# awslabs/crowd-coachable-recommendations

Hardware: AMD Instinct MI355X
Metric: queries/sec, exhaustive inner-product top-100 retrieval (NQ-shaped 2,681,468 x 768 bf16 corpus) (higher is better)
Workload: dtype bf16

## Files before the change

### crowd-coachable-recommendations_amd/ccrec_amd/_lib.py

```python
import ctypes
import os

_HERE = os.path.dirname(os.path.abspath(__file__))
LIB_PATH = os.path.join(os.path.dirname(_HERE), "lib", "libccr_hip.so")

CCR_OK = 0
CCR_ERR_INVALID, CCR_ERR_HIP, CCR_ERR_WORKSPACE, CCR_ERR_BLOCK_ID = -1, -2, -3, -4
DTYPE_F32, DTYPE_F16, DTYPE_BF16 = 0, 1, 2
SEARCH_DEFAULT, SEARCH_FORCE_DENSE, SEARCH_FORCE_FUSED, SEARCH_ASYNC = 0, 1, 2, 4
SCORES_CANONICAL, SCORES_MFMA = 0, 1

EXPORTS = [
    "ccr_last_error", "ccr_version", "ccr_pack_bf16", "ccr_pack_bf16_ex", "ccr_meanpool_pack_bf16", "ccr_meanpool_pack_bf16_ex", "ccr_index_create",
    "ccr_index_create_with_norms", "ccr_index_destroy",
    "ccr_index_rows", "ccr_index_dim", "ccr_search_workspace_bytes", "ccr_search", "ccr_search_last_stats",
    "ccr_merge_topk", "ccr_merge_topk_strided", "ccr_apply_block", "ccr_inbatch_ce_workspace_bytes", "ccr_inbatch_ce_fwd", "ccr_inbatch_ce_bwd", "ccr_inbatch_ce_bwd_dev", "ccr_rank_metrics",
    "ccr_search_finish", "ccr_scores", "ccr_search_blocked_workspace_bytes", "ccr_search_blocked",
    "ccr_search_sparse_prior_workspace_bytes", "ccr_search_sparse_prior", "ccr_colsum_bf16", "ccr_meanpool_bwd", "ccr_bm25_index_create", "ccr_bm25_index_destroy", "ccr_bm25_search_workspace_bytes",
    "ccr_bm25_search", "ccr_pack_bf16_padded", "ccr_shard_message_bytes", "ccr_search_shard", "ccr_shard_message_fill", "ccr_merge_shard_messages",
    "ccr_attention_bf16", "ccr_add_layernorm", "ccr_meanpool_pack_bf16_packed", "ccr_embed_layernorm", "ccr_gelu_bf16",
    "ccr_attention_half", "ccr_add_layernorm_half", "ccr_embed_layernorm_half", "ccr_gelu_half", "ccr_merge_short_lists",
    "ccr_bm25_search_workspace_bytes_k", "ccr_bm25_search_last_stats", "ccr_bm25_index_set_idf", "ccr_inbatch_pack3_bf16", "ccr_inbatch_ce_fwd_f32",
    "ccr_search_stream_wait_main_pass", "ccr_pool_ce_workspace_bytes", "ccr_pool_ce_fwd", "ccr_pool_ce_fwd_f32", "ccr_pool_ce_bwd_dev",
    "ccr_bpr_sample", "ccr_bpr_frozen_workspace_bytes", "ccr_bpr_frozen_fwd", "ccr_bpr_frozen_bwd_dev",
    "ccr_attention_fwd_train_half", "ccr_attention_bwd_workspace_bytes", "ccr_attention_bwd_half", "ccr_add_layernorm_bwd_half", "ccr_gelu_bwd_half",
    "ccr_dropout_bits_rows", "ccr_dropout_bits_attention", "ccr_dropout_apply", "ccr_attention_fwd_train_drop_half", "ccr_attention_bwd_drop_half",
    "ccr_add_layernorm_drop_half", "ccr_add_layernorm_bwd_drop_half",
]

MIN_VERSION = 101
BPR_VERSION = 102
ENCODER_TRAIN_VERSION = 103
ENCODER_DROPOUT_VERSION = 104

SHARD_HEADER_BYTES = 32
SHARD_MAGIC = 0x4D524343


class ShardHeader(ctypes.Structure):
    _fields_ = [("magic", ctypes.c_uint32), ("n_flagged", ctypes.c_uint32), ("k_valid", ctypes.c_uint32),
                ("n_covered", ctypes.c_uint32), ("row_offset", ctypes.c_int64), ("n_rows", ctypes.c_int64)]


class SearchStats(ctypes.Structure):
    _fields_ = [("path", ctypes.c_int32), ("n_fallback", ctypes.c_int32), ("sample_tiles", ctypes.c_int32),
                ("ranges", ctypes.c_int32), ("cap", ctypes.c_int32), ("sublists", ctypes.c_int32),
                ("n_candidates", ctypes.c_int64), ("ms_sample", ctypes.c_float), ("ms_threshold", ctypes.c_float),
                ("ms_main", ctypes.c_float), ("ms_select", ctypes.c_float), ("ms_fallback", ctypes.c_float),
                ("ms_total", ctypes.c_float), ("n_retried", ctypes.c_int32), ("n_dense", ctypes.c_int32),
                ("main_launches", ctypes.c_int32), ("opt_rank", ctypes.c_int32), ("main_tile_queries", ctypes.c_int32),
                ("reserved0", ctypes.c_int32)]


class CcrError(RuntimeError):
    pass


_lib = None


def load():
    global _lib
    if _lib is not None:
        return _lib
    if not os.path.isfile(LIB_PATH):
        raise CcrError(f"{LIB_PATH} not built: run `python -c 'import __graft_entry__ as g; g.build()'` "
                       f"(or make -C crowd-coachable-recommendations_amd/csrc)")
    lib = ctypes.CDLL(LIB_PATH)
    lib.ccr_version.restype = ctypes.c_int
    have = int(lib.ccr_version())
    if have < MIN_VERSION:
        raise CcrError(f"{LIB_PATH} is version {have}, this binding needs {MIN_VERSION}: rebuild it "
                       f"(python -c 'import __graft_entry__ as g; g.build()')")
    missing = [name for name in EXPORTS if not hasattr(lib, name)]
    if missing:
        raise CcrError(f"{LIB_PATH} lacks {', '.join(missing)}: rebuild it (python -c 'import __graft_entry__ as g; g.build()')")
    vp, i32, i64, f32, sz = ctypes.c_void_p, ctypes.c_int, ctypes.c_int64, ctypes.c_float, ctypes.c_size_t
    lib.ccr_last_error.restype = ctypes.c_char_p
    lib.ccr_last_error.argtypes = []
    lib.ccr_version.restype = i32
    lib.ccr_pack_bf16.argtypes = [vp, vp, vp, i64, i32, i32, vp]
    lib.ccr_pack_bf16_ex.argtypes = [vp, vp, vp, vp, i64, i32, i32, vp]
    lib.ccr_index_create_with_norms.argtypes = [vp, i64, i32, i64, vp, vp, ctypes.POINTER(vp)]
    lib.ccr_meanpool_pack_bf16.argtypes = [vp, i32, vp, vp, vp, i32, i32, i32, i32, vp]
    lib.ccr_meanpool_pack_bf16_ex.argtypes = [vp, i32, vp, vp, vp, vp, vp, i32, i32, i32, i32, vp]
    lib.ccr_index_create.argtypes = [vp, i64, i32, i64, vp, ctypes.POINTER(vp)]
    lib.ccr_index_destroy.argtypes = [vp]
    lib.ccr_index_rows.argtypes = [vp]
    lib.ccr_index_rows.restype = i64
    lib.ccr_index_dim.argtypes = [vp]
    lib.ccr_search_workspace_bytes.argtypes = [vp, i32, i32]
    lib.ccr_search_workspace_bytes.restype = sz
    lib.ccr_search.argtypes = [vp, vp, i32, i32, vp, vp, vp, sz, i32, vp]
    lib.ccr_search_last_stats.argtypes = [vp, ctypes.POINTER(SearchStats)]
    lib.ccr_merge_topk.argtypes = [vp, vp, i32, i32, i32, vp, vp, vp]
    lib.ccr_merge_topk_strided.argtypes = [vp, vp, i64, i64, i32, i32, i32, vp, vp, vp]
    lib.ccr_apply_block.argtypes = [vp, vp, i32, i32, vp, vp, i64, vp, vp, i32, vp]
    lib.ccr_inbatch_ce_workspace_bytes.argtypes = [i32, i32]
    lib.ccr_inbatch_ce_workspace_bytes.restype = sz
    lib.ccr_inbatch_ce_fwd.argtypes = [vp, vp, vp, i32, i32, f32, vp, vp, vp, sz, vp]
    lib.ccr_inbatch_ce_bwd.argtypes = [vp, vp, vp, vp, i32, i32, f32, f32, vp, vp, vp, vp, sz, vp]
    lib.ccr_inbatch_ce_bwd_dev.argtypes = [vp, vp, vp, vp, i32, i32, f32, vp, vp, vp, vp, vp, sz, vp]
    lib.ccr_inbatch_pack3_bf16.argtypes = [vp, vp, vp, i32, i32, vp, vp]
    lib.ccr_inbatch_ce_fwd_f32.argtypes = [vp, vp, vp, i32, i32, f32, vp, vp, vp, vp, sz, vp]
    lib.ccr_pool_ce_workspace_bytes.argtypes = [i32, i32, i32]
    lib.ccr_pool_ce_workspace_bytes.restype = sz
    lib.ccr_pool_ce_fwd.argtypes = [vp, vp, vp, vp, i32, i32, i32, f32, vp, vp, vp, sz, vp]
    lib.ccr_pool_ce_fwd_f32.argtypes = [vp, vp, vp, vp, i32, i32, i32, f32, vp, vp, vp, vp, sz, vp]
    lib.ccr_pool_ce_bwd_dev.argtypes = [vp, vp, vp, vp, vp, i32, i32, i32, f32, vp, vp, vp, vp, vp, sz, vp]
    lib.ccr_bpr_sample.argtypes = [vp, i32, i32, i64, vp, vp, vp, f32, vp, vp, i32, vp, i32, vp, vp]
    lib.ccr_bpr_frozen_workspace_bytes.argtypes = [i32, i32, i32]
    lib.ccr_bpr_frozen_workspace_bytes.restype = sz
    lib.ccr_bpr_frozen_fwd.argtypes = [vp, i64, i32, vp, vp, f32, vp, vp, vp, vp, i32, i32, vp, vp, sz, vp]
    lib.ccr_bpr_frozen_bwd_dev.argtypes = [vp, i64, i32, vp, vp, f32, vp, vp, vp, vp, i32, i32, vp, vp, vp, vp, vp, sz, vp]
    lib.ccr_rank_metrics.argtypes = [vp, i32, i32, vp, vp, vp, i32, vp, vp, vp]
    lib.ccr_search_finish.argtypes = [vp]
    lib.ccr_search_stream_wait_main_pass.argtypes = [vp, vp]
    lib.ccr_scores.argtypes = [vp, vp, i32, i32, vp, vp]
    lib.ccr_search_blocked_workspace_bytes.argtypes = [vp, i32, i32, vp]
    lib.ccr_search_blocked_workspace_bytes.restype = sz
    lib.ccr_search_blocked.argtypes = [vp, vp, i32, i32, vp, vp, vp, vp, vp, sz, i32, vp]
    lib.ccr_search_sparse_prior_workspace_bytes.argtypes = [vp, i32, i32, vp]
    lib.ccr_search_sparse_prior_workspace_bytes.restype = sz
    lib.ccr_search_sparse_prior.argtypes = [vp, vp, i32, i32, vp, vp, vp, vp, vp, vp, sz, i32, vp]
    lib.ccr_colsum_bf16.argtypes = [vp, i64, i32, vp, vp]
    lib.ccr_meanpool_bwd.argtypes = [vp, vp, vp, i32, i32, i32, i32, vp]
    lib.ccr_bm25_index_create.argtypes = [vp, vp, vp, vp, i64, i64, ctypes.c_double, ctypes.POINTER(vp)]
    lib.ccr_bm25_index_destroy.argtypes = [vp]
    lib.ccr_bm25_search_workspace_bytes.argtypes = [vp, i32, i32]
    lib.ccr_bm25_search_workspace_bytes.restype = sz
    lib.ccr_bm25_search_workspace_bytes_k.argtypes = [vp, i32, i32, i32]
    lib.ccr_bm25_search_workspace_bytes_k.restype = sz
    lib.ccr_bm25_search_last_stats.argtypes = [vp, vp]
    lib.ccr_bm25_index_set_idf.argtypes = [vp, vp, vp, vp]
    lib.ccr_bm25_search.argtypes = [vp, vp, vp, vp, i32, i32, vp, vp, vp, sz, vp]
    lib.ccr_pack_bf16_padded.argtypes = [vp, i64, i32, vp, i32, vp, vp, i32, vp]
    lib.ccr_attention_bf16.argtypes = [vp, vp, vp, vp, i32, i32, i32, i32, ctypes.c_float, vp]
    lib.ccr_add_layernorm.argtypes = [vp, vp, vp, vp, ctypes.c_float, vp, vp, i64, i32, vp]
    lib.ccr_embed_layernorm.argtypes = [vp, i64, vp, i64, vp, i64, vp, vp, vp, vp, vp, ctypes.c_float, vp, vp, i64, i32, vp]
    lib.ccr_gelu_bf16.argtypes = [vp, vp, i64, vp]
    lib.ccr_attention_half.argtypes = [vp, vp, vp, vp, i32, i32, i32, i32, ctypes.c_float, i32, vp]
    lib.ccr_add_layernorm_half.argtypes = [vp, vp, vp, vp, ctypes.c_float, vp, vp, i64, i32, i32, vp]
    lib.ccr_embed_layernorm_half.argtypes = [vp, i64, vp, i64, vp, i64, vp, vp, vp, vp, vp, ctypes.c_float, vp, vp, i64, i32, i32, vp]
    lib.ccr_gelu_half.argtypes = [vp, vp, i64, i32, vp]
    lib.ccr_attention_fwd_train_half.argtypes = [vp, vp, vp, vp, vp, i32, i32, i32, i32, ctypes.c_float, i32, vp]
    lib.ccr_attention_bwd_workspace_bytes.argtypes = [i32, i32, i32]
    lib.ccr_attention_bwd_workspace_bytes.restype = sz
    lib.ccr_attention_bwd_half.argtypes = [vp, vp, vp, vp, vp, vp, vp, i32, i32, i32, i32, ctypes.c_float, i32, vp, sz, vp]
    lib.ccr_add_layernorm_bwd_half.argtypes = [vp, vp, vp, ctypes.c_float, vp, vp, vp, vp, vp, i64, i32, i32, vp, sz, vp]
    lib.ccr_gelu_bwd_half.argtypes = [vp, vp, vp, i64, i32, vp]
    u64, u32, f64 = ctypes.c_uint64, ctypes.c_uint32, ctypes.c_double
    lib.ccr_dropout_bits_rows.argtypes = [vp, i64, i32, u64, u32, f64, vp]
    lib.ccr_dropout_bits_attention.argtypes = [vp, vp, vp, vp, i64, i32, i32, i32, u64, u32, f64, vp]
    lib.ccr_dropout_apply.argtypes = [vp, vp, f32, vp, vp, i64, i32, i32, vp]
    lib.ccr_attention_fwd_train_drop_half.argtypes = [vp, vp, vp, vp, vp, vp, f32, i32, i32, i32, i32, f32, i32, vp]
    lib.ccr_attention_bwd_drop_half.argtypes = [vp, vp, vp, vp, vp, vp, vp, vp, f32, vp, i32, i32, i32, i32, f32, i32, vp, sz, vp]
    lib.ccr_add_layernorm_drop_half.argtypes = [vp, vp, f32, vp, vp, vp, f32, vp, vp, i64, i32, i32, vp]
    lib.ccr_add_layernorm_bwd_drop_half.argtypes = [vp, vp, f32, vp, vp, f32, vp, vp, vp, vp, vp, i64, i32, i32, vp, sz, vp]
    lib.ccr_meanpool_pack_bf16_packed.argtypes = [vp, i32, vp, vp, vp, vp, vp, vp, i32, i32, i32, vp]
    lib.ccr_shard_message_bytes.argtypes = [i32, i32]
    lib.ccr_shard_message_bytes.restype = sz
    lib.ccr_search_shard.argtypes = [vp, vp, i32, i32, vp, vp, sz, i32, vp]
    lib.ccr_shard_message_fill.argtypes = [vp, i32, i32, i32, vp, vp, i64, i64, vp]
    lib.ccr_merge_shard_messages.argtypes = [vp, i64, i32, i32, i32, vp, vp, vp]
    lib.ccr_merge_short_lists.argtypes = [vp, i64, i32, i32, i32, i32, vp, vp, vp, vp, vp]
    for name in EXPORTS:
        fn = getattr(lib, name)
        if fn.restype is ctypes.c_int and name not in ("ccr_version", "ccr_index_dim"):
            fn.restype = i32
    _lib = lib
    return lib


def check(rc, what=""):
    if rc != CCR_OK:
        msg = load().ccr_last_error().decode("utf-8", "replace")
        if rc == CCR_ERR_BLOCK_ID:
            raise AssertionError("block id not found")
        raise CcrError(f"{what} failed ({rc}): {msg}")
```

### crowd-coachable-recommendations_amd/csrc/ccr_api.hip

```cpp
#include <stdarg.h>
#include <stdlib.h>
#include <string.h>

#include <math.h>

#include <algorithm>
#include <mutex>
#include <vector>

#include "ccr_index.h"
#include "ccr_narrow.h"
#include "ccr_topk_device.h"

namespace ccr {

static thread_local char g_err[512] = "";
void set_error(const char *fmt, ...) {
    va_list ap;
    va_start(ap, fmt);
    vsnprintf(g_err, sizeof(g_err), fmt, ap);
    va_end(ap);
}

static int env_int(const char *name, int dflt) {
    const char *e = getenv(name);
    return e ? atoi(e) : dflt;
}

Knobs read_knobs() {
    Knobs kn;
    kn.qgroups = env_int("CCR_QGROUPS", 0);
    kn.progressive = env_int("CCR_PROGRESSIVE", 1);
    kn.max_phases = env_int("CCR_PHASES", 3);
    kn.mfma16 = env_int("CCR_MFMA16", -1);
    kn.sample_div = env_int("CCR_SAMPLE_DIV", 0);
    kn.max_lists = env_int("CCR_MAX_LISTS", 0);
    kn.ranges = env_int("CCR_RANGES", 0);
    kn.optimistic = env_int("CCR_OPTIMISTIC", -1);
    kn.opt_rank = env_int("CCR_OPT_RANK", 0);
    kn.narrow = env_int("CCR_NARROW", -1);
    kn.wide = env_int("CCR_WIDE", -1);
    kn.narrow_grid = env_int("CCR_NARROW_GRID", 0);
    kn.narrow_groups = env_int("CCR_NARROW_GROUPS", NARROW_MAX_GROUPS);
    return kn;
}

static int pick_qgroups(int qblocks, int dim, const Knobs &kn, int tile_q = TILE_Q) {
    {
        const int v = kn.qgroups;
        if ((v == 1 || v == 2 || v == 4 || v == 8) && qblocks % v == 0) return v;
    }
    const size_t block_bytes = (size_t)tile_q * dim * 2;
    int best = 1;
    for (int gq = 1; gq <= NUM_XCD; gq *= 2) {
        if (qblocks % gq) continue;
        best = gq;
        if ((size_t)(qblocks / gq) * block_bytes <= (size_t)3 << 20) break;
    }
    return best;
}

static inline int64_t round_up(int64_t v, int64_t m) { return (v + m - 1) / m * m; }

static int best_sample_ranges(int64_t n_vt, int qblocks, int qgroups, int grid) {
    const int nrc = NUM_XCD / qgroups, qb_per = qblocks / qgroups, per_x = std::max(1, grid / NUM_XCD);
    int best_r = NUM_XCD;
    double best = 1e300;
    const int64_t r_max = round_up(std::min<int64_t>(n_vt, 1024), NUM_XCD);
    std::vector<double> load((size_t)per_x);
    for (int64_t R = NUM_XCD; R <= r_max; R += NUM_XCD) {
        double worst = 0.0;
        for (int rc = 0; rc < nrc; ++rc) {
            std::fill(load.begin(), load.end(), 0.0);
            const int64_t items = R / nrc * qb_per;
            for (int64_t item = 0; item < items; ++item) {
                const int64_t r = rc + nrc * (item / qb_per);
                const int64_t ntile = (n_vt - r + R - 1) / R;
                if (ntile > 0) load[(size_t)(item % per_x)] += (double)ntile + 0.15;
            }
            worst = std::max(worst, *std::max_element(load.begin(), load.end()));
        }
        if (worst < best - 1e-9) {
            best = worst;
            best_r = (int)R;
        }
    }
    return best_r;
}

constexpr size_t DENSE_SCRATCH_TARGET = (size_t)1 << 30;

struct MainPassChoice {
    int64_t sample, ranges;
    int item_a, item_b;
    int opt_rank;
};

static int optimistic_rank(int k, int64_t sample, int64_t tiles, const Knobs &kn) {
    if (kn.opt_rank > 0) return kn.opt_rank;
    const double need = (double)k * (double)sample / (double)tiles;
    int r = 40;
    for (; r < 1 << 20; ++r) {
        const double a = 1.0 / (9.0 * r), t = 1.0 - a - 5.2 * sqrt(a);
        if (t > 0.0 && (double)r * t * t * t >= need) break;
    }
    return r;
}

static MainPassChoice choose_main_pass(const Plan &p, int k, int64_t sample_a, int64_t sample_b, int64_t sample_c, const Knobs &kn,
                                       bool single_only = false) {
    const int nrc = NUM_XCD / p.main_qgroups, qb_per = p.main_qblocks / p.main_qgroups, per_x = p.grid / NUM_XCD;
    const double tile_cost = p.tile_q == WIDE_Q ? 1.37 : 1.0;
    int64_t max_lists = p.rescore_cap > 512 ? 2048 : 1024;
    if ((max_lists / p.sublists) * p.main_qblocks < p.grid) max_lists = 2048;
    if (kn.max_lists >= 64 && kn.max_lists < max_lists) max_lists = kn.max_lists;
    const int64_t r_hi = std::min<int64_t>(max_lists / p.sublists, round_up(std::max<int64_t>(1, p.tiles / 8), NUM_XCD));
    const int64_t target = std::min<int64_t>(r_hi, round_up(std::max<int64_t>(NUM_XCD, (int64_t)p.grid * 6 / p.main_qblocks), NUM_XCD));
    const bool prog_on = kn.progressive != 0 && !single_only;
    const int max_phases = kn.max_phases;
    const double qscale = (double)p.nq_pad / 3584.0;
    const double select_per_range = 0.1 * qscale, hit_w = 0.014 * qscale, phase_w = 3.0;
    auto sample_cost = [&](int64_t smp) -> double {
        return (double)((smp * p.qblocks + p.grid - 1) / p.grid) + 0.015 * (double)smp * std::max(1.0, qscale);
    };

    MainPassChoice best_choice = {sample_a, target, 0, 0, 0};
    double best = 1e300;
    for (int pass = 0; pass < 3; ++pass) {
        const int64_t smp = pass == 0 ? sample_a : (pass == 1 ? sample_b : sample_c);
        if ((pass >= 1 && smp == sample_a) || (pass == 2 && smp == sample_b)) continue;
        const double fs = (double)smp / (double)p.tiles;
        const double smp_cost = sample_cost(smp);
        auto survivors = [&](double fa, double fb) -> double {
            if (fa <= 0.0) return (double)k / fs;
            if (fb <= 0.0) return (double)k * (fa / fs + (1.0 - fa) / fa);
            return (double)k * (fa / fs + fb / fa + (1.0 - fa - fb) / (fa + fb));
        };
        const int64_t r_lo = std::max<int64_t>(NUM_XCD, target / 2 / NUM_XCD * NUM_XCD);
        for (int64_t R = r_lo; R <= std::min(r_hi, target * 2); R += NUM_XCD) {
            if (kn.ranges > 0 && R != std::min<int64_t>(r_hi, std::max<int64_t>(r_lo, round_up(kn.ranges, NUM_XCD)))) continue;
            const int64_t items = R / nrc * qb_per;
            const double item_cost = ((double)((p.tiles + R - 1) / R) + 0.15) * tile_cost;
            auto rounds = [&](int64_t n) { return (double)((n + per_x - 1) / per_x); };
            const double common = smp_cost + select_per_range * (double)R + 1e-3 * std::abs((double)(R - target));
            const double single = rounds(items) * item_cost + hit_w * survivors(0.0, 0.0) + common;
            if (single < best && kn.optimistic != 1) {
                best = single;
                best_choice = {smp, R, 0, 0, 0};
            }
            if (kn.optimistic != 0 && smp * GROUPS_PER_TILE >= 4 * 40) {
                const int rank = optimistic_rank(k, smp, p.tiles, kn);
                if ((int64_t)rank * 4 <= smp * GROUPS_PER_TILE) {
                    const double pass = std::max((double)rank / fs, (double)k);
                    const double opt = rounds(items) * item_cost + hit_w * pass + common - (kn.optimistic == 1 ? 1e9 : 0.0);
                    if (opt < best) {
                        best = opt;
                        best_choice = {smp, R, 0, 0, rank};
                    }
                }
            }
            if (!(prog_on && items > per_x && (double)p.tiles / (double)R >= 8.0)) continue;
            const double fa = (double)per_x / (double)items;
            const double two = (1.0 + rounds(items - per_x)) * item_cost + phase_w + hit_w * survivors(fa, 0.0) + common;
            if (two < best) {
                best = two;
                best_choice = {smp, R, per_x, 0, 0};
            }
            if (max_phases < 3) continue;
            for (int m = 1; m <= 3; ++m) {
                const int64_t ib = (int64_t)per_x * (1 + m);
                if (ib >= items) break;
                const double fb = (double)m * per_x / (double)items;
                const double three = (1.0 + m + rounds(items - ib)) * item_cost + 2.0 * phase_w + hit_w * survivors(fa, fb) + common;
                if (three < best) {
                    best = three;
                    best_choice = {smp, R, per_x, (int)ib, 0};
                }
            }
        }
    }
    return best_choice;
}

static CandLayout one_segment(int cap) {
    CandLayout L;
    memset(&L, 0, sizeof(L));
    L.nseg = 1;
    L.seg_end[0] = L.seg_end[1] = L.seg_end[2] = INT32_MAX;
    L.cap[0] = L.cap[1] = L.cap[2] = cap;
    return L;
}

static Plan make_plan_for(int64_t n_rows, int dim, int n_q, int k, int flags, int num_cu, const Knobs &kn, int mfma16) {
    Plan p;
    memset(&p, 0, sizeof(p));
    p.nq_pad = (int)round_up(n_q, TILE_Q);
    p.qblocks = p.nq_pad / TILE_Q;
    p.tile_q = TILE_Q;
    p.main_qblocks = p.qblocks;
    p.main_qgroups = 1;
    p.tiles = (n_rows + TILE_DOCS - 1) / TILE_DOCS;
    p.full_tiles = n_rows / TILE_DOCS;
    p.grid = std::max(NUM_XCD, num_cu / NUM_XCD * NUM_XCD);
    {
        p.mfma16 = mfma16;
        p.sublists = p.mfma16 ? 8 : 4;
    }
    p.rescore_cap = std::min(8192, std::max(256, 2 * pow2_ceil(k)));

    const int64_t min_sample = (2 * (int64_t)k + GROUPS_PER_TILE - 1) / GROUPS_PER_TILE;
    int64_t sample_div = 32;
    bool sample_div_forced = false;
    {
        if (kn.sample_div >= 4 && kn.sample_div <= 256) {
            sample_div = kn.sample_div;
            sample_div_forced = true;
        }
    }
    auto sample_for = [&](int64_t div) { return std::max<int64_t>({(p.tiles + div - 1) / div, min_sample, 4}); };
    int64_t sample = sample_for(sample_div);
    bool fused = (dim % 8 == 0) && dim >= 8 && (sample * 4 <= p.full_tiles) && k <= MAX_K;
    if ((flags & CCR_SEARCH_FORCE_FUSED) && (dim % 8 == 0) && p.full_tiles >= 1) {
        if (!fused) sample = std::min<int64_t>(std::max<int64_t>(sample, 1), p.full_tiles);
        fused = sample * GROUPS_PER_TILE >= k;
    }
    if (flags & CCR_SEARCH_FORCE_DENSE) fused = false;
    p.fused = fused ? 1 : 0;

    if (p.fused) {
        p.qgroups = pick_qgroups(p.qblocks, dim, kn);
        const bool pinned = sample_div_forced || (flags & CCR_SEARCH_FORCE_FUSED);
        const int64_t sample_alt = pinned ? sample : sample_for(2 * sample_div);
        int64_t sample_big = pinned ? sample : sample_for(sample_div / 2);
        if (sample_big * 4 > p.full_tiles) sample_big = sample;
        int nqt = n_q <= 16 ? 1 : (n_q <= 32 ? 2 : 4);
        int ngroups = n_q <= NARROW_MAX_Q ? 1 : 2;
        if (n_q > NARROW_MAX_Q && n_q <= 96 && kn.narrow_groups >= 2 && dim % TILE_K == 0 && narrow_lds_bytes(6, dim) <= (size_t)160 * 1024)
            nqt = 6, ngroups = 1;
        const bool narrow = kn.narrow != 0 && n_q <= NARROW_MAX_Q * std::min(std::max(kn.narrow_groups, 1), NARROW_MAX_GROUPS) && dim % TILE_K == 0 &&
                            narrow_lds_bytes(nqt, dim) <= (size_t)160 * 1024 && (ngroups == 1 || num_cu >= 16);
        p.narrow = narrow ? nqt : 0;
        p.narrow_groups = narrow ? ngroups : 1;
        p.tile_q = TILE_Q;
        p.main_qblocks = p.qblocks;
        if (!narrow && p.mfma16 && dim % 32 == 0 && kn.wide != 0) {
            const int wb = (n_q + WIDE_Q - 1) / WIDE_Q;
            const double per_xcd = (double)(wb / pick_qgroups(wb, dim, kn, WIDE_Q)) * WIDE_Q * dim * 2.0;
            const double per_flop = per_xcd <= 3.2 * 1048576.0 ? 0.95 : (per_xcd <= 5.5 * 1048576.0 ? 0.97 : 1.04);
            if (kn.wide == 1 || (double)wb * WIDE_Q * per_flop < (double)p.qblocks * TILE_Q) {
                p.tile_q = WIDE_Q;
                p.main_qblocks = wb;
                p.nq_pad = (int)round_up(std::max<int64_t>(n_q, (int64_t)wb * WIDE_Q), TILE_Q);
                p.qblocks = p.nq_pad / TILE_Q;
                p.qgroups = pick_qgroups(p.qblocks, dim, kn);
            }
        }
        p.main_qgroups = pick_qgroups(p.main_qblocks, dim, kn, p.tile_q);
        const MainPassChoice choice = choose_main_pass(p, k, sample, sample_alt, sample_big, kn, narrow);
        sample = choice.sample;
        const int64_t R = choice.ranges;
        p.sample_tiles = (int)sample;
        p.sample_stride = std::max<int64_t>(1, p.full_tiles / sample);
        p.sample_ranges = best_sample_ranges(sample, p.qblocks, p.qgroups, p.grid);
        p.ranges = (int)R;
        p.item_a = choice.item_a;
        p.item_b = choice.item_b;
        p.opt_rank = choice.opt_rank;
        const int nrc_p = NUM_XCD / p.main_qgroups, qb_per_p = p.main_qblocks / p.main_qgroups;
        const int64_t RA = p.item_a ? std::min<int64_t>(R, (int64_t)nrc_p * ((p.item_a + qb_per_p - 1) / qb_per_p)) : 0;
        const int64_t RB = p.item_b ? std::min<int64_t>(R, (int64_t)nrc_p * ((p.item_b + qb_per_p - 1) / qb_per_p)) : 0;
        const double ratio = (double)p.tiles / (double)sample;
        const double expect = (double)k * ratio * 1.3 + 64.0;
        const double fs = 1.0 / ratio, nlists = (double)R * p.sublists;
        const double xk = 1.25 * ((double)k + 4.75 * sqrt((double)k) + 8.0) / (double)k;
        const int64_t tile_rows = TILE_DOCS / p.sublists;
        const double xr = p.opt_rank ? 1.25 * ((double)p.opt_rank + 4.75 * sqrt((double)p.opt_rank) + 8.0) / (double)p.opt_rank : 0.0;
        auto cap_for = [&](double g) -> int {
            const double mean = p.opt_rank ? xr * std::max((double)p.opt_rank / fs, (double)k) / nlists : xk * (double)k / (g * nlists);
            const int64_t c = (int64_t)(mean + 6.0 * sqrt(mean)) + 16 + tile_rows;
            return (int)round_up(std::min<int64_t>(std::max<int64_t>(c, 16), 8192), 4);
        };
        const double fa = p.item_a ? (double)(p.item_a / qb_per_p) * nrc_p / (double)R : 0.0;
        const double fb = p.item_b ? std::max(0.0, (double)(p.item_b / qb_per_p) * nrc_p / (double)R - fa) : 0.0;
        const double upd_compact = std::min(32768.0, std::max(4096.0, 8.0 * pow2_ceil(k)));
        auto seen = [&](double g, double found) { return found > upd_compact ? g * upd_compact / found : g; };
        const double found_a = (double)k * fa / fs;
        CandLayout &L = p.cand;
        memset(&L, 0, sizeof(L));
        const int seg_end_v[3] = {RA ? (int)RA : (int)R, RB > RA ? (int)RB : (int)R, (int)R};
        int64_t recs = 0;
        L.nseg = 0;
        int prev_end = 0;
        for (int g = 0; g < 3; ++g) {
            L.seg_end[g] = INT32_MAX;
            L.cap[g] = 16;
            L.base[g] = recs;
        }
        for (int g = 0; g < 3; ++g) {
            if (seg_end_v[g] <= prev_end) continue;
            const int sg = L.nseg++;
            double frac_seen = fs;
            if (sg == 1) frac_seen = fa >= 2.0 * fs ? seen(fa, found_a) : fs;
            if (sg == 2) frac_seen = fa >= 2.0 * fs ? seen(fa + fb, found_a + (double)k * fb / fa) : fs;
            L.seg_end[sg] = seg_end_v[g];
            L.cap[sg] = cap_for(std::min(1.0, std::max(frac_seen, fs)));
            L.base[sg] = recs;
            recs += (int64_t)(seg_end_v[g] - prev_end) * p.nq_pad * p.sublists * L.cap[sg];
            recs = round_up(recs, 32);
            prev_end = seg_end_v[g];
        }
        L.seg_end[L.nseg - 1] = INT32_MAX;
        p.cap = L.cap[0];
        const double want_opt = std::max(xr * std::max((double)p.opt_rank / fs, (double)k) + 512.0, k > 256 ? 18.0 * k : 0.0);
        p.select_compact = select_compact_entries(dim, p.ranges * p.sublists, p.rescore_cap,
                                                  (int64_t)((p.opt_rank ? want_opt : (RA ? 16.0 * k + 512.0 : expect)) * 1.25));
        p.first_nsub = p.ranges * p.sublists;
        p.first_sp = p.sublists;
        p.first_lay = p.cand;
        if (p.narrow) {
            const double pass = p.opt_rank ? xr * std::max((double)p.opt_rank / fs, (double)k) : expect;
            int64_t capn = std::max<int64_t>(recs / ((int64_t)NARROW_SUBLISTS * std::max(1, n_q)), (int64_t)(8.0 * pass) + 4096);
            capn = std::min<int64_t>(capn, (int64_t)1 << 22) / 4 * 4;
            recs = std::max<int64_t>(recs, capn * NARROW_SUBLISTS * n_q);
            p.first_lay = one_segment((int)capn);
            p.first_nsub = NARROW_SUBLISTS;
            p.first_sp = NARROW_SUBLISTS;
        }
        p.cand_recs = recs;
        p.dense_rows_per_chunk = FALLBACK_ROWS;
    } else {
        int64_t rows = (int64_t)(DENSE_SCRATCH_TARGET / ((size_t)n_rows * 4));
        rows = std::min<int64_t>(std::max<int64_t>(rows, 1), n_q);
        if (rows >= 64) rows = rows / 64 * 64;
        p.dense_rows_per_chunk = rows;
    }
    const SearchWs w = search_ws(p, n_rows, dim, n_q, k, nullptr);
    p.off_qnorm = (size_t)w.qnorm, p.off_thr = (size_t)w.thr, p.off_gmax = (size_t)w.gmax, p.off_cnt = (size_t)w.cnt, p.off_cand = (size_t)w.cand;
    p.off_flag = (size_t)w.flag_count, p.off_dense = (size_t)w.dense, p.off_retry = (size_t)w.Q2, p.off_top = (size_t)w.top, p.off_safe = (size_t)w.thr_safe;
    p.total = w.total;
    return p;
}

SearchWs search_ws(const Plan &p, int64_t n_rows, int dim, int n_q, int k, char *base) {
    SearchWs w;
    memset(&w, 0, sizeof(w));
    Bump b = {0};
    auto at = [&](size_t off) { return (char *)((uintptr_t)base + off); };
    auto take = [&](size_t bytes) { return at(b.take(bytes)); };
    if (!p.fused) {
        w.flag_count = (uint32_t *)take(64 + (size_t)n_q * 4);
        w.flag_list = w.flag_count + 16;
        w.dense_bytes = (size_t)p.dense_rows_per_chunk * (n_rows + 3) * 4;
        w.dense = (float *)take(w.dense_bytes);
        w.total = b.off;
        return w;
    }
    const size_t nq_pad = p.nq_pad;
    w.qnorm = (float *)take(nq_pad * 4);
    w.thr = (float *)take(nq_pad * 8);
    w.cq = w.thr + nq_pad;
    w.gmax = (float *)take((size_t)p.sample_tiles * GROUPS_PER_TILE * nq_pad * 4);
    w.cnt = (uint32_t *)take((size_t)p.ranges * nq_pad * p.sublists * 4);
    w.cand = (uint2 *)take((size_t)p.cand_recs * 8);
    w.flag_count = (uint32_t *)take(64 + (size_t)n_q * 4);
    w.stat_cand = (unsigned long long *)(w.flag_count + 2);
    w.flag_list = w.flag_count + 16;
    w.cand_bytes = (char *)w.flag_count - (char *)w.cand;
    w.top = (uint32_t *)take(p.item_b ? (nq_pad + (size_t)n_q * k) * 4 : 0);
    w.thr_safe = (float *)take(p.opt_rank ? nq_pad * 8 : 0);
    w.cq_safe = w.thr_safe + nq_pad;
    w.dense_bytes = (size_t)p.dense_rows_per_chunk * n_rows * 4;
    w.dense = (float *)take(w.dense_bytes);
    w.retry_bytes = nq_pad * dim * 2 + nq_pad * 8 + (size_t)n_q * 16 + 64 + 64 + (size_t)n_q * 4 + 256 * 10;
    Bump r = {b.take(w.retry_bytes)};
    w.Q2 = (uint16_t *)at(r.take(nq_pad * dim * 2));
    w.thr2 = (float *)at(r.take(nq_pad * 4));
    w.cq2 = (float *)at(r.take(nq_pad * 4));
    w.retry_list = (uint32_t *)at(r.take((size_t)n_q * 4));
    w.dense_list = (uint32_t *)at(r.take((size_t)n_q * 4));
    w.counts = (uint32_t *)at(r.take(64));
    w.flag2 = (uint32_t *)at(r.take(64 + (size_t)n_q * 4));
    w.list_b = (uint32_t *)at(r.take((size_t)n_q * 4));
    w.list_c = (uint32_t *)at(r.take((size_t)n_q * 4));
    w.total = b.off;
    return w;
}

Plan make_plan(int64_t n_rows, int dim, int n_q, int k, int flags, int num_cu, const Knobs &kn) {
    if (kn.mfma16 >= 0) return make_plan_for(n_rows, dim, n_q, k, flags, num_cu, kn, kn.mfma16 ? 1 : 0);
    if (k <= 512) return make_plan_for(n_rows, dim, n_q, k, flags, num_cu, kn, 1);
    const Plan p32 = make_plan_for(n_rows, dim, n_q, k, flags, num_cu, kn, 0);
    if (p32.fused && p32.ranges * 8 <= 2048) return make_plan_for(n_rows, dim, n_q, k, flags, num_cu, kn, 1);
    return p32;
}

}

using namespace ccr;

namespace {
constexpr int SLAB_SLOTS = 1024, SLAB_SLOT_BYTES = 256, MAX_DEVICES = 64;
struct Slab {
    char *base = nullptr;
    char *host = nullptr;
    std::vector<int> free_slots;
};
constexpr int SLAB_HOST_BYTES = 64;
std::mutex g_slab_mutex;
Slab g_slabs[MAX_DEVICES];

int slab_take(int device, uint32_t **out, volatile uint32_t **host_out) {
    std::lock_guard<std::mutex> lock(g_slab_mutex);
    CCR_REQUIRE(device >= 0 && device < MAX_DEVICES, "device ordinal %d out of range", device);
    Slab &sl = g_slabs[device];
    if (!sl.base) {
        CCR_HIP_CHECK(hipMalloc((void **)&sl.base, (size_t)SLAB_SLOTS * SLAB_SLOT_BYTES));
        if (hipHostMalloc((void **)&sl.host, (size_t)SLAB_SLOTS * SLAB_HOST_BYTES, hipHostMallocDefault) != hipSuccess) {
            (void)hipFree(sl.base);
            sl.base = nullptr;
            set_error("ccr_index_create: hipHostMalloc of the pinned flag lines failed");
            return CCR_ERR_HIP;
        }
        for (int i = SLAB_SLOTS - 1; i >= 0; --i) sl.free_slots.push_back(i);
    }
    if (sl.free_slots.empty()) {
        set_error("ccr_index_create: more than %d live indices on device %d", SLAB_SLOTS, device);
        return CCR_ERR_INVALID;
    }
    *out = reinterpret_cast<uint32_t *>(sl.base + (size_t)sl.free_slots.back() * SLAB_SLOT_BYTES);
    *host_out = reinterpret_cast<volatile uint32_t *>(sl.host + (size_t)sl.free_slots.back() * SLAB_HOST_BYTES);
    sl.free_slots.pop_back();
    return CCR_OK;
}

void slab_give(int device, uint32_t *p) {
    if (!p || device < 0 || device >= MAX_DEVICES) return;
    std::lock_guard<std::mutex> lock(g_slab_mutex);
    Slab &sl = g_slabs[device];
    sl.free_slots.push_back((int)((reinterpret_cast<char *>(p) - sl.base) / SLAB_SLOT_BYTES));
}
}

extern "C" const char *ccr_last_error(void) { return g_err; }
extern "C" int ccr_version(void) { return 104; }

extern "C" int ccr_index_destroy(ccr_index *ix);

namespace {
struct CachedBlock {
    void *p;
    size_t bytes;
};
std::vector<CachedBlock> g_blocks[MAX_DEVICES];
constexpr size_t BLOCK_CACHE_ENTRIES = 8;

int block_take(int device, size_t bytes, void **out, size_t *got) {
    CCR_REQUIRE(device >= 0 && device < MAX_DEVICES, "device ordinal %d out of range", device);
    bytes = (bytes + 4095) / 4096 * 4096;
    {
        std::lock_guard<std::mutex> lock(g_slab_mutex);
        auto &v = g_blocks[device];
        for (size_t i = 0; i < v.size(); ++i)
            if (v[i].bytes >= bytes && v[i].bytes <= 2 * bytes) {
                *out = v[i].p;
                *got = v[i].bytes;
                v.erase(v.begin() + i);
                return CCR_OK;
            }
    }
    CCR_HIP_CHECK(hipMalloc(out, bytes));
    *got = bytes;
    return CCR_OK;
}

void block_give(int device, void *p, size_t bytes) {
    if (!p) return;
    void *drop = nullptr;
    if (device >= 0 && device < MAX_DEVICES && bytes <= ((size_t)64 << 20)) {
        std::lock_guard<std::mutex> lock(g_slab_mutex);
        auto &v = g_blocks[device];
        v.push_back({p, bytes});
        if (v.size() > BLOCK_CACHE_ENTRIES) {
            drop = v.front().p;
            v.erase(v.begin());
        }
    } else {
        drop = p;
    }
    if (drop) (void)hipFree(drop);
}
}

static int index_create_impl(const uint16_t *D_bf16, int64_t n_rows, int dim, int64_t global_row_offset, const float *row_bounds,
                             void *stream, ccr_index **out) {
    CCR_REQUIRE(D_bf16 && out, "ccr_index_create: null pointer");
    CCR_REQUIRE(n_rows >= 1 && n_rows < ((int64_t)1 << 32), "ccr_index_create: n_rows=%lld out of range [1, 2^32)",
                (long long)n_rows);
    CCR_REQUIRE(dim >= 8 && dim % 8 == 0 && dim <= 4096, "ccr_index_create: dim=%d must be a multiple of 8 in [8, 4096]", dim);
    CCR_REQUIRE((uintptr_t)D_bf16 % 16 == 0, "ccr_index_create: corpus pointer must be 16-byte aligned");
    hipStream_t s = (hipStream_t)stream;
    ccr_index *ix = new ccr_index();
    memset(ix, 0, sizeof(*ix));
    ix->D = D_bf16;
    ix->n_rows = n_rows;
    ix->dim = dim;
    ix->offset = ix->id_out = global_row_offset;
    ix->knobs = read_knobs();
    auto build = [&]() -> int {
        CCR_HIP_CHECK(hipGetDevice(&ix->device));
        CCR_HIP_CHECK(hipDeviceGetAttribute(&ix->num_cu, hipDeviceAttributeMultiprocessorCount, ix->device));
        int rc = slab_take(ix->device, &ix->dmax_bits, &ix->host_flags);
        if (rc != CCR_OK) return rc;
        const int64_t tiles = (n_rows + TILE_DOCS - 1) / TILE_DOCS;
        void *tn = nullptr;
        rc = block_take(ix->device, (size_t)tiles * 4, &tn, &ix->tile_bytes);
        if (rc != CCR_OK) return rc;
        ix->tile_norm = (float *)tn;
        uint32_t *tile_bits = reinterpret_cast<uint32_t *>(ix->tile_norm);
        if (row_bounds) {
            ix->row_norm = row_bounds;
            rc = launch_tile_norms(row_bounds, n_rows, tile_bits, ix->dmax_bits, s);
            if (rc != CCR_OK) return rc;
        } else {
            void *rn = nullptr;
            rc = block_take(ix->device, (size_t)n_rows * 4, &rn, &ix->row_bytes);
            if (rc != CCR_OK) return rc;
            ix->row_norm = ix->row_norm_own = (float *)rn;
            CCR_HIP_CHECK(hipMemsetAsync(ix->dmax_bits, 0, 4, s));
            CCR_HIP_CHECK(hipMemsetAsync(tile_bits, 0, (size_t)tiles * 4, s));
            rc = launch_row_norms_bf16(D_bf16, n_rows, dim, ix->row_norm_own, ix->dmax_bits, tile_bits, s);
            if (rc != CCR_OK) return rc;
            CCR_HIP_CHECK(hipStreamSynchronize(s));
        }
        return CCR_OK;
    };
    const int rc = build();
    if (rc != CCR_OK) {
        ccr_index_destroy(ix);
        return rc;
    }
    *out = ix;
    return CCR_OK;
}

extern "C" int ccr_index_create(const uint16_t *D_bf16, int64_t n_rows, int dim, int64_t global_row_offset, void *stream,
                                ccr_index **out) {
    return index_create_impl(D_bf16, n_rows, dim, global_row_offset, nullptr, stream, out);
}

extern "C" int ccr_index_create_with_norms(const uint16_t *D_bf16, int64_t n_rows, int dim, int64_t global_row_offset,
                                           const float *row_norm_bounds, void *stream, ccr_index **out) {
    CCR_REQUIRE(row_norm_bounds, "ccr_index_create_with_norms: null row_norm_bounds");
    return index_create_impl(D_bf16, n_rows, dim, global_row_offset, row_norm_bounds, stream, out);
}

extern "C" int ccr_index_destroy(ccr_index *ix) {
    if (!ix) return CCR_OK;
    if (ix->pending.active && ix->have_events) (void)hipEventSynchronize(ix->ev[EV_ASYNC_END]);
    ix->pending.active = false;
    slab_give(ix->device, ix->dmax_bits);
    block_give(ix->device, ix->tile_norm, ix->tile_bytes);
    block_give(ix->device, ix->row_norm_own, ix->row_bytes);
    if (ix->have_events)
        for (int i = 0; i < EV_COUNT; ++i)
            if (ix->ev[i]) (void)hipEventDestroy(ix->ev[i]);
    delete ix;
    return CCR_OK;
}

extern "C" int64_t ccr_index_rows(const ccr_index *ix) { return ix ? ix->n_rows : -1; }
extern "C" int ccr_index_dim(const ccr_index *ix) { return ix ? ix->dim : -1; }

extern "C" size_t ccr_search_workspace_bytes(const ccr_index *ix, int n_q, int k) {
    if (!ix || n_q <= 0 || k <= 0) return 0;
    Plan a = make_plan(ix->n_rows, ix->dim, n_q, k, CCR_SEARCH_DEFAULT, ix->num_cu, ix->knobs);
    Plan b = make_plan(ix->n_rows, ix->dim, n_q, k, CCR_SEARCH_FORCE_DENSE, ix->num_cu, ix->knobs);
    Plan c = make_plan(ix->n_rows, ix->dim, n_q, k, CCR_SEARCH_FORCE_FUSED, ix->num_cu, ix->knobs);
    return std::max({a.total, b.total, c.total}) + 256;
}

extern "C" int ccr_search_stream_wait_main_pass(const ccr_index *ix, void *stream) {
    CCR_REQUIRE(ix, "ccr_search_stream_wait_main_pass: null index");
    if (!ix->main_pass_recorded) return CCR_OK;
    CCR_HIP_CHECK(hipStreamWaitEvent((hipStream_t)stream, ix->ev[EV_MAIN_END], 0));
    return CCR_OK;
}

extern "C" int ccr_search_last_stats(const ccr_index *ix, ccr_search_stats *stats) {
    CCR_REQUIRE(ix && stats, "ccr_search_last_stats: null pointer");
    CCR_REQUIRE(!ix->pending.active, "ccr_search_last_stats: an asynchronous search is pending (call ccr_search_finish first)");
    *stats = ix->stats;
    return CCR_OK;
}

static int dense_for_list(const ccr_index *ix, const uint16_t *Q, const uint32_t *d_qlist, int n, int k, float *scratch, int64_t rows_per_chunk,
                          float *out_scores, int64_t *out_ids, hipStream_t s) {
    for (int lo = 0; lo < n; lo += (int)rows_per_chunk) {
        const int m = std::min<int64_t>(rows_per_chunk, n - lo);
        int rc = launch_dense_scores(ix->D, ix->n_rows, ix->dim, Q, d_qlist ? d_qlist + lo : nullptr, lo, m, nullptr, scratch, s);
        if (rc != CCR_OK) return rc;
        rc = launch_dense_select(scratch, ix->n_rows, k, d_qlist ? d_qlist + lo : nullptr, lo, m, nullptr, ix->id_out, out_scores, out_ids, s);
        if (rc != CCR_OK) return rc;
    }
    return CCR_OK;
}

static bool margin_path_ok(const ccr_index *ix, int k) { return ix->dim % 8 == 0 && k <= MAX_K; }
static int64_t tiles_of(const ccr_index *ix) { return (ix->n_rows + TILE_DOCS - 1) / TILE_DOCS; }

static GemmArgs gemm_args(const ccr_index *ix, const uint16_t *Q, int n_q, int nq_pad) {
    GemmArgs g;
    memset(&g, 0, sizeof(g));
    g.D = ix->D;
    g.n_rows = ix->n_rows;
    g.dim = ix->dim;
    g.Q = Q;
    g.n_q = n_q;
    g.nq_pad = nq_pad;
    g.qblocks = nq_pad / TILE_Q;
    g.item_end = INT32_MAX;
    return g;
}

static GemmArgs filter_args(const ccr_index *ix, const Plan &p, const SearchWs &w, const uint16_t *Q, int n_q, int nq_pad, int qblocks,
                            int qgroups, const float *thr, const float *cq, const CandLayout &lay) {
    GemmArgs g = gemm_args(ix, Q, n_q, nq_pad);
    g.qblocks = qblocks;
    g.qgroups = qgroups;
    g.n_vt = p.tiles;
    g.tile_stride = 1;
    g.ranges = p.ranges;
    g.thr = thr;
    g.cq = cq;
    g.tile_norm = ix->tile_norm;
    g.cnt = w.cnt;
    g.cand = w.cand;
    g.lay = lay;
    return g;
}

static int store_scores(const ccr_index *ix, const uint16_t *Q, int n_q, int ranges, float *out, int64_t pitch, hipStream_t s) {
    GemmArgs g = gemm_args(ix, Q, n_q, (int)round_up(n_q, TILE_Q));
    g.n_vt = tiles_of(ix);
    g.tile_stride = 1;
    g.ranges = ranges;
    g.qgroups = 1;
    g.store = out;
    g.store_pitch = pitch;
    return launch_gemm(g, ix->knobs.mfma16 != 0 ? MAIN_16X16 : MAIN_32X32, EPI_STORE, std::max(NUM_XCD, ix->num_cu / NUM_XCD * NUM_XCD), s);
}

static int margin_for_rows(const ccr_index *ix, const uint16_t *Qc, const float *hint, const uint32_t *out_rows, int n, int k, float *scratch,
                           size_t scratch_bytes, float *out_scores, int64_t *out_ids, uint32_t *flag_count, uint32_t *flag_list, hipStream_t s) {
    const int64_t pitch = round_up(ix->n_rows, 4);
    int64_t chunk = (int64_t)(scratch_bytes / ((size_t)pitch * 4));
    CCR_REQUIRE(chunk >= 1, "margin path: no room for one score row");
    if (chunk > TILE_Q) chunk = chunk / TILE_Q * TILE_Q;
    const int ranges = (int)round_up(std::min<int64_t>(std::max<int64_t>(1, tiles_of(ix) / 4), 1024), NUM_XCD);
    for (int lo = 0; lo < n; lo += (int)chunk) {
        const int m = std::min<int64_t>(chunk, n - lo);
        const uint16_t *Q = Qc + (int64_t)lo * ix->dim;
        int rc = store_scores(ix, Q, m, ranges, scratch, pitch, s);
        if (rc != CCR_OK) return rc;
        rc = launch_margin_select(scratch, pitch, ix->n_rows, k, ix->dim, Q, ix->D, ix->tile_norm, ix->row_norm, ix->dmax_bits,
                                  hint ? hint + lo : nullptr, out_rows ? out_rows + lo : nullptr, lo, m, ix->id_out, out_scores, out_ids, flag_count, flag_list, s);
        if (rc != CCR_OK) return rc;
    }
    return CCR_OK;
}

static int run_main_pass(const ccr_index *ix, const Plan &p, const SearchWs &w, const uint16_t *Q, int n_q, int k, hipStream_t s) {
    GemmArgs gm = filter_args(ix, p, w, Q, n_q, p.nq_pad, p.main_qblocks, p.main_qgroups, w.thr, w.cq, p.cand);
    const int nrc = NUM_XCD / gm.qgroups, qb_per = gm.qblocks / gm.qgroups, items = p.ranges / nrc * qb_per;
    const int bounds[4] = {0, p.item_a, p.item_b, items};
    int done = 0, updates = 0, prev_full = 0, prev_part = 0, prev_blocks = 0;
    for (int ph = 1; ph < 4; ++ph) {
        if (bounds[ph] <= done) continue;
        if (done > 0) {
            const int rl_full = done / qb_per, part = done % qb_per;
            const int full = rl_full * nrc * p.sublists, partial = part ? (rl_full + 1) * nrc * p.sublists : 0;
            const bool more = bounds[ph] < items && ph < 3;
            const int rc = launch_threshold_update(w.cand, w.cnt, full, partial, part, prev_full, prev_part, prev_blocks, qb_per, p.sublists, n_q,
                                                   p.nq_pad, p.cand, k, w.cq, ix->tile_norm, p.item_b ? w.top : nullptr, updates > 0, more, w.thr, s, p.tile_q);
            if (rc != CCR_OK) return rc;
            prev_full = full;
            prev_part = partial;
            prev_blocks = part;
            ++updates;
        }
        gm.item_begin = done;
        gm.item_end = bounds[ph];
        const MainKernel kind = p.tile_q == WIDE_Q ? MAIN_WIDE : p.mfma16 ? MAIN_16X16 : MAIN_32X32;
        const int rc = launch_gemm(gm, kind, EPI_FILTER, p.grid, s);
        if (rc != CCR_OK) return rc;
        done = bounds[ph];
    }
    return CCR_OK;
}

static int run_narrow_pass(const ccr_index *ix, const Plan &p, const SearchWs &w, const uint16_t *Q, int n_q, hipStream_t s) {
    NarrowArgs na;
    memset(&na, 0, sizeof(na));
    na.D = ix->D;
    na.n_rows = ix->n_rows;
    na.dim = ix->dim;
    na.Q = Q;
    na.n_q = n_q;
    na.q_stride = narrow_query_stride(ix->dim);
    na.thr = w.thr;
    na.cq = w.cq;
    na.tile_norm = ix->tile_norm;
    na.cand = w.cand;
    na.cnt = w.cnt;
    na.cap = p.first_lay.cap[0];
    na.groups = p.narrow_groups;
    int ngrid = ix->knobs.narrow_grid > 0 ? ix->knobs.narrow_grid : ix->num_cu;
    const int64_t blocks = (ix->n_rows + 16 * NARROW_WAVES - 1) / (16 * NARROW_WAVES);
    if ((int64_t)ngrid > blocks) ngrid = (int)std::max<int64_t>(1, blocks);
    if (p.narrow_groups == 2) ngrid = std::max(16, ngrid / 16 * 16);
    return launch_narrow_filter(na, p.narrow, ngrid, s);
}

static int read_words(void *host, const void *dev, int n, hipStream_t s) {
    CCR_HIP_CHECK(hipMemcpyAsync(host, dev, (size_t)n * 4, hipMemcpyDeviceToHost, s));
    CCR_HIP_CHECK(hipStreamSynchronize(s));
    return CCR_OK;
}


static int fused_stats(ccr_index *ix, uint32_t nflag, unsigned long long ncand) {
    const Plan &p = ix->plan;
    ccr_search_stats &st = ix->stats;
    float a = 0, b = 0;
    CCR_HIP_CHECK(hipEventElapsedTime(&st.ms_sample, ix->ev[EV_SAMPLE_BEGIN], ix->ev[EV_SAMPLE_END]));
    CCR_HIP_CHECK(hipEventElapsedTime(&a, ix->ev[EV_BEGIN], ix->ev[EV_SAMPLE_BEGIN]));
    CCR_HIP_CHECK(hipEventElapsedTime(&b, ix->ev[EV_SAMPLE_END], ix->ev[EV_MAIN_BEGIN]));
    st.ms_threshold = a + b;
    CCR_HIP_CHECK(hipEventElapsedTime(&st.ms_main, ix->ev[EV_MAIN_BEGIN], ix->ev[EV_MAIN_END]));
    CCR_HIP_CHECK(hipEventElapsedTime(&st.ms_select, ix->ev[EV_MAIN_END], ix->ev[EV_SELECT_END]));
    CCR_HIP_CHECK(hipEventElapsedTime(&st.ms_total, ix->ev[EV_BEGIN], ix->ev[EV_SELECT_END]));
    st.path = 1;
    st.n_fallback = (int32_t)nflag;
    st.sample_tiles = p.sample_tiles;
    st.ranges = p.narrow ? 1 : p.ranges;
    st.cap = p.narrow ? p.first_lay.cap[0] : p.cap;
    st.sublists = p.narrow ? p.first_sp : p.sublists;
    st.main_launches = 1 + (p.item_a ? 1 : 0) + (p.item_b ? 1 : 0);
    st.opt_rank = p.opt_rank;
    st.main_tile_queries = p.narrow ? 0 : p.tile_q;
    st.n_candidates = (int64_t)ncand;
    return CCR_OK;
}

static int recover_thresholds(const ccr_index *ix, const SearchWs &w, int nflag) {
    const auto &pd = ix->pending;
    const int rc = launch_threshold(w.gmax, (int64_t)ix->plan.sample_tiles * GROUPS_PER_TILE, pd.n_q, ix->plan.nq_pad, pd.k, w.qnorm, ix->dmax_bits,
                                    ix->dim, ix->tile_norm, ix->plan.sample_stride, w.thr_safe, w.cq_safe, pd.stream);
    if (rc != CCR_OK) return rc;
    return launch_underfilled_to_retry(w.flag_list, 0, nflag, w.thr_safe, w.thr, pd.stream);
}

static int to_dense(const SearchWs &w, const uint32_t *list, int n, int &n_dense, hipStream_t s) {
    CCR_HIP_CHECK(hipMemcpyAsync(w.dense_list + n_dense, list, (size_t)n * 4, hipMemcpyDeviceToDevice, s));
    n_dense += n;
    return CCR_OK;
}

static int retry_group(ccr_index *ix, const SearchWs &w, const uint32_t *cur, int n_cur, int &n_dense) {
    const Plan &p = ix->plan;
    const auto &pd = ix->pending;
    hipStream_t s = pd.stream;
    const int nsub_all = p.ranges * p.sublists;
    for (int round = 0;; ++round) {
        int rc = launch_gather_queries(pd.Q, ix->dim, cur, n_cur, w.thr, w.cq, w.Q2, w.thr2, w.cq2, s);
        if (rc != CCR_OK) return rc;
        const int pad2 = (int)round_up(n_cur, TILE_Q);
        const int64_t cap2 = std::min<int64_t>(8192, (int64_t)(w.cand_bytes / 8) / ((int64_t)nsub_all * pad2) / 4 * 4);
        if (cap2 < 16) break;
        const CandLayout lay2 = one_segment((int)cap2);
        CCR_HIP_CHECK(hipMemsetAsync(w.cnt, 0, (size_t)nsub_all * pad2 * 4, s));
        CCR_HIP_CHECK(hipMemsetAsync(w.flag2, 0, 64, s));
        const GemmArgs g = filter_args(ix, p, w, w.Q2, n_cur, pad2, pad2 / TILE_Q, pick_qgroups(pad2 / TILE_Q, ix->dim, ix->knobs), w.thr2, w.cq2, lay2);
        rc = launch_gemm(g, p.mfma16 ? MAIN_16X16 : MAIN_32X32, EPI_FILTER, p.grid, s);
        if (rc != CCR_OK) return rc;
        rc = launch_select_rescore(w.cand, w.cnt, nsub_all, p.sublists, n_cur, pad2, lay2, pd.k, p.rescore_cap, p.select_compact, ix->n_rows,
                                   w.thr2, w.cq2, ix->tile_norm, ix->row_norm, ix->dmax_bits, w.Q2, ix->D, ix->dim, ix->id_out, pd.out_scores, pd.out_ids,
                                   w.flag2, w.flag2 + 16, nullptr, cur, s);
        if (rc != CCR_OK) return rc;
        ix->stats.n_retried += n_cur;
        uint32_t again = 0;
        rc = read_words(&again, w.flag2, 1, s);
        if (rc != CCR_OK || again == 0) return rc;
        uint32_t *next = (cur == w.list_b) ? w.list_c : w.list_b;
        rc = launch_partition_flags(w.flag2 + 16, 0, (int)again, next, w.dense_list + n_dense, w.counts, s);
        if (rc != CCR_OK) return rc;
        uint32_t hc[2] = {0, 0};
        rc = read_words(hc, w.counts, 2, s);
        if (rc != CCR_OK) return rc;
        n_dense += (int)hc[1];
        const uint32_t *list = cur;
        const int n = n_cur;
        cur = next;
        n_cur = (int)hc[0];
        if (n_cur == 0 || round == 2 || n_cur >= n) break;
        rc = launch_threshold_update(w.cand, w.cnt, nsub_all, 0, 0, 0, 0, 0, 1, p.sublists, n, pad2, lay2, pd.k, w.cq2, ix->tile_norm, nullptr,
                                     false, false, w.thr2, s);
        if (rc != CCR_OK) return rc;
        rc = launch_scatter_thresholds(list, n, w.thr2, w.thr, s);
        if (rc != CCR_OK) return rc;
    }
    return n_cur > 0 ? to_dense(w, cur, n_cur, n_dense, s) : CCR_OK;
}

static int retry_flagged(ccr_index *ix, const SearchWs &w, int n_retry, int &n_dense) {
    const Plan &p = ix->plan;
    const auto &pd = ix->pending;
    const int nsub_all = p.ranges * p.sublists;
    if (nsub_all > 2048) return to_dense(w, w.retry_list, n_retry, n_dense, pd.stream);
    int rc = launch_threshold_update(w.cand, w.cnt, p.first_nsub, 0, 0, 0, 0, 0, 1, p.first_sp, pd.n_q, p.nq_pad, p.first_lay, pd.k, w.cq,
                                     ix->tile_norm, nullptr, false, false, w.thr, pd.stream);
    if (rc != CCR_OK) return rc;
    const int64_t want_cap = std::min<int64_t>(8192, 4 * (int64_t)p.cap);
    int64_t group = (int64_t)(w.cand_bytes / 8) / ((int64_t)nsub_all * want_cap) / TILE_Q * TILE_Q;
    group = std::max<int64_t>(TILE_Q, std::min<int64_t>(group, round_up(n_retry, TILE_Q)));
    for (int g0 = 0; g0 < n_retry && rc == CCR_OK; g0 += (int)group)
        rc = retry_group(ix, w, w.retry_list + g0, std::min<int>((int)group, n_retry - g0), n_dense);
    return rc;
}

static int complete_dense(ccr_index *ix, const SearchWs &w, int n_dense) {
    const Plan &p = ix->plan;
    const auto &pd = ix->pending;
    hipStream_t s = pd.stream;
    const bool margin_in_cand = w.cand_bytes > w.dense_bytes;
    const int64_t fit = (int64_t)(w.cand_bytes / ((size_t)ix->n_rows * 4)) / 64 * 64;
    const bool fp64_in_cand = n_dense > p.dense_rows_per_chunk && fit >= 64;
    const int64_t chunk = fp64_in_cand ? std::min<int64_t>(fit, 256) : p.dense_rows_per_chunk;
    float *fp64_scr = fp64_in_cand ? (float *)w.cand : w.dense;
    if (!margin_path_ok(ix, pd.k))
        return dense_for_list(ix, pd.Q, w.dense_list, n_dense, pd.k, fp64_scr, chunk, pd.out_scores, pd.out_ids, s);
    CCR_HIP_CHECK(hipMemsetAsync(w.flag2, 0, 64, s));
    for (int lo = 0; lo < n_dense; lo += p.nq_pad) {
        const int m = std::min(p.nq_pad, n_dense - lo);
        int rc = launch_gather_queries(pd.Q, ix->dim, w.dense_list + lo, m, w.thr, w.cq, w.Q2, w.thr2, w.cq2, s);
        if (rc != CCR_OK) return rc;
        rc = margin_for_rows(ix, w.Q2, w.thr2, w.dense_list + lo, m, pd.k, margin_in_cand ? (float *)w.cand : w.dense,
                             margin_in_cand ? w.cand_bytes : w.dense_bytes, pd.out_scores, pd.out_ids, w.flag2, w.flag2 + 16, s);
        if (rc != CCR_OK) return rc;
    }
    uint32_t left = 0;
    const int rc = read_words(&left, w.flag2, 1, s);
    if (rc != CCR_OK || left == 0) return rc;
    return dense_for_list(ix, pd.Q, w.flag2 + 16, (int)left, pd.k, fp64_scr, chunk, pd.out_scores, pd.out_ids, s);
}

static int search_complete(ccr_index *ix) {
    auto &pd = ix->pending;
    hipStream_t s = pd.stream;
    const bool was_async = pd.active;
    pd.active = false;
    const SearchWs w = search_ws(ix->plan, ix->n_rows, ix->dim, pd.n_q, pd.k, pd.ws);
    struct { uint32_t nflag, pad; unsigned long long ncand; } host;
    int rc = CCR_OK;
    if (was_async) {
        CCR_HIP_CHECK(hipEventSynchronize(ix->ev[EV_ASYNC_END]));
        host.nflag = ix->host_flags[0];
        host.ncand = *reinterpret_cast<volatile unsigned long long *>(ix->host_flags + 2);
    } else {
        rc = read_words(&host, w.flag_count, 4, s);
        if (rc != CCR_OK) return rc;
    }
    rc = fused_stats(ix, host.nflag, host.ncand);
    if (rc != CCR_OK || host.nflag == 0) return rc;
    rc = ix->plan.opt_rank ? recover_thresholds(ix, w, (int)host.nflag) : CCR_OK;
    if (rc != CCR_OK) return rc;
    rc = launch_partition_flags(w.flag_list, 0, (int)host.nflag, w.retry_list, w.dense_list, w.counts, s);
    if (rc != CCR_OK) return rc;
    uint32_t hc[2] = {0, 0};
    rc = read_words(hc, w.counts, 2, s);
    if (rc != CCR_OK) return rc;
    int n_dense = (int)hc[1];
    if (hc[0] > 0) rc = retry_flagged(ix, w, (int)hc[0], n_dense);
    if (rc == CCR_OK && n_dense > 0) rc = complete_dense(ix, w, n_dense);
    if (rc != CCR_OK) return rc;
    ix->stats.n_dense += n_dense;
    CCR_HIP_CHECK(hipEventRecord(ix->ev[EV_DONE], s));
    CCR_HIP_CHECK(hipStreamSynchronize(s));
    CCR_HIP_CHECK(hipEventElapsedTime(&ix->stats.ms_fallback, ix->ev[EV_SELECT_END], ix->ev[EV_DONE]));
    ix->stats.ms_total += ix->stats.ms_fallback;
    return CCR_OK;
}

extern "C" int ccr_search_finish(ccr_index *ix) {
    CCR_REQUIRE(ix, "ccr_search_finish: null index");
    return ix->pending.active ? search_complete(ix) : CCR_OK;
}

static int search_dense(ccr_index *ix, const SearchWs &w, const uint16_t *Q, int n_q, int k, float *out_scores, int64_t *out_ids,
                        int flags, hipStream_t s) {
    const bool async = (flags & CCR_SEARCH_ASYNC) != 0;
    const int64_t chunk = ix->plan.dense_rows_per_chunk;
    int rc;
    if (!async && !(flags & CCR_SEARCH_FORCE_DENSE) && margin_path_ok(ix, k)) {
        CCR_HIP_CHECK(hipMemsetAsync(w.flag_count, 0, 64, s));
        rc = margin_for_rows(ix, Q, nullptr, nullptr, n_q, k, w.dense, w.dense_bytes, out_scores, out_ids, w.flag_count, w.flag_list, s);
        if (rc != CCR_OK) return rc;
        uint32_t nf = 0;
        rc = read_words(&nf, w.flag_count, 1, s);
        if (rc != CCR_OK) return rc;
        ix->stats.n_fallback = ix->stats.n_dense = (int32_t)nf;
        if (nf > 0) rc = dense_for_list(ix, Q, w.flag_list, (int)nf, k, w.dense, chunk, out_scores, out_ids, s);
    } else {
        rc = dense_for_list(ix, Q, nullptr, n_q, k, w.dense, chunk, out_scores, out_ids, s);
    }
    if (rc != CCR_OK) return rc;
    CCR_HIP_CHECK(hipEventRecord(ix->ev[EV_DONE], s));
    if (async) return CCR_OK;
    CCR_HIP_CHECK(hipStreamSynchronize(s));
    CCR_HIP_CHECK(hipEventElapsedTime(&ix->stats.ms_total, ix->ev[EV_BEGIN], ix->ev[EV_DONE]));
    ix->stats.ms_fallback = ix->stats.ms_total;
    return CCR_OK;
}

static int search_impl(ccr_index *ix, const uint16_t *Q_bf16, int n_q, int k, float *out_scores, int64_t *out_ids, int64_t id_out,
                       uint32_t *flagged_out, void *workspace, size_t ws_bytes, int flags, void *stream) {
    CCR_REQUIRE(ix && Q_bf16 && out_scores && out_ids, "ccr_search: null pointer");
    CCR_REQUIRE(n_q >= 0, "ccr_search: n_q=%d", n_q);
    CCR_REQUIRE(k >= 1 && k <= MAX_K && (int64_t)k <= ix->n_rows, "ccr_search: k=%d must be in [1, min(n_rows=%lld, %d)]", k,
                (long long)ix->n_rows, MAX_K);
    CCR_REQUIRE((uintptr_t)Q_bf16 % 16 == 0, "ccr_search: query pointer must be 16-byte aligned");
    CCR_REQUIRE(!ix->pending.active, "ccr_search: an asynchronous search is pending on this index (call ccr_search_finish first)");
    memset(&ix->stats, 0, sizeof(ix->stats));
    ix->main_pass_recorded = false;
    if (n_q == 0) return CCR_OK;
    hipStream_t s = (hipStream_t)stream;
    ix->id_out = id_out;
    const bool async = (flags & CCR_SEARCH_ASYNC) != 0;
    const int plan_flags = flags & ~CCR_SEARCH_ASYNC;
    if (!(ix->plan_nq == n_q && ix->plan_k == k && ix->plan_flags == plan_flags)) {
        ix->plan = make_plan(ix->n_rows, ix->dim, n_q, k, plan_flags, ix->num_cu, ix->knobs);
        ix->plan_nq = n_q;
        ix->plan_k = k;
        ix->plan_flags = plan_flags;
    }
    const Plan p = ix->plan;
    if (!workspace || ws_bytes < p.total || (uintptr_t)workspace % 256 != 0) {
        set_error("ccr_search: workspace %zu bytes (256-byte aligned) required, got %zu at %p", p.total, ws_bytes, workspace);
        return CCR_ERR_WORKSPACE;
    }
    const SearchWs w = search_ws(p, ix->n_rows, ix->dim, n_q, k, (char *)workspace);

    if (!ix->have_events) {
        for (int i = 0; i < EV_COUNT; ++i) CCR_HIP_CHECK(hipEventCreate(&ix->ev[i]));
        ix->have_events = true;
    }
    CCR_HIP_CHECK(hipEventRecord(ix->ev[EV_BEGIN], s));
    if (!p.fused) return search_dense(ix, w, Q_bf16, n_q, k, out_scores, out_ids, flags, s);

    CCR_HIP_CHECK(hipMemsetAsync(w.flag_count, 0, 64, s));
    if ((int64_t)p.ranges > p.tiles) CCR_HIP_CHECK(hipMemsetAsync(w.cnt, 0, (size_t)p.ranges * p.nq_pad * p.sublists * 4, s));
    int rc = launch_row_norms_bf16(Q_bf16, n_q, ix->dim, w.qnorm, nullptr, nullptr, s);
    if (rc != CCR_OK) return rc;

    GemmArgs gs = gemm_args(ix, Q_bf16, n_q, p.nq_pad);
    gs.qgroups = p.qgroups;
    gs.n_vt = p.sample_tiles;
    gs.tile_stride = p.sample_stride;
    gs.ranges = p.sample_ranges;
    gs.gmax = w.gmax;
    CCR_HIP_CHECK(hipEventRecord(ix->ev[EV_SAMPLE_BEGIN], s));
    rc = launch_gemm(gs, MAIN_32X32, EPI_GMAX, p.grid, s);
    if (rc != CCR_OK) return rc;
    CCR_HIP_CHECK(hipEventRecord(ix->ev[EV_SAMPLE_END], s));
    rc = launch_threshold(w.gmax, (int64_t)p.sample_tiles * GROUPS_PER_TILE, n_q, p.nq_pad, p.opt_rank ? p.opt_rank : k, w.qnorm, ix->dmax_bits,
                          ix->dim, ix->tile_norm, p.sample_stride, w.thr, w.cq, s, p.narrow ? w.cnt : nullptr, p.narrow ? NARROW_SUBLISTS : 0);
    if (rc != CCR_OK) return rc;

    CCR_HIP_CHECK(hipEventRecord(ix->ev[EV_MAIN_BEGIN], s));
    rc = p.narrow ? run_narrow_pass(ix, p, w, Q_bf16, n_q, s) : run_main_pass(ix, p, w, Q_bf16, n_q, k, s);
    if (rc != CCR_OK) return rc;
    CCR_HIP_CHECK(hipEventRecord(ix->ev[EV_MAIN_END], s));
    ix->main_pass_recorded = true;
    rc = launch_select_rescore(w.cand, w.cnt, p.first_nsub, p.first_sp, n_q, p.nq_pad, p.first_lay, k, p.rescore_cap, p.select_compact, ix->n_rows, w.thr,
                               w.cq, ix->tile_norm, ix->row_norm, ix->dmax_bits, Q_bf16, ix->D, ix->dim, ix->id_out, out_scores, out_ids,
                               w.flag_count, w.flag_list, w.stat_cand, nullptr, s);
    if (rc != CCR_OK) return rc;
    CCR_HIP_CHECK(hipEventRecord(ix->ev[EV_SELECT_END], s));

    ix->pending = {false, Q_bf16, n_q, k, out_scores, out_ids, (char *)workspace, s};
    if (!async) return search_complete(ix);
    if (flagged_out) CCR_HIP_CHECK(hipMemcpyAsync(flagged_out, w.flag_count, 4, hipMemcpyDeviceToDevice, s));
    CCR_HIP_CHECK(hipMemcpyAsync((void *)ix->host_flags, w.flag_count, 16, hipMemcpyDeviceToHost, s));
    CCR_HIP_CHECK(hipEventRecord(ix->ev[EV_ASYNC_END], s));
    ix->pending.active = true;
    return CCR_OK;
}

extern "C" int ccr_search(ccr_index *ix, const uint16_t *Q_bf16, int n_q, int k, float *out_scores, int64_t *out_ids,
                          void *workspace, size_t ws_bytes, int flags, void *stream) {
    CCR_REQUIRE(ix, "ccr_search: null index");
    return search_impl(ix, Q_bf16, n_q, k, out_scores, out_ids, ix->offset, nullptr, workspace, ws_bytes, flags, stream);
}

static inline size_t shard_rows_at(int n_q, int k) { return (sizeof(ccr_shard_header) + (size_t)n_q * k * 4 + 15) / 16 * 16; }

extern "C" size_t ccr_shard_message_bytes(int n_q, int k) {
    if (n_q < 0 || k < 1) return 0;
    return (shard_rows_at(n_q, k) + (size_t)n_q * k * 4 + 15) / 16 * 16;
}

extern "C" int ccr_search_shard(ccr_index *ix, const uint16_t *Q_bf16, int n_q, int k, void *message, void *workspace, size_t ws_bytes,
                                int flags, void *stream) {
    CCR_REQUIRE(ix && message, "ccr_search_shard: null pointer");
    CCR_REQUIRE((uintptr_t)message % 16 == 0, "ccr_search_shard: message must be 16-byte aligned");
    CCR_REQUIRE(n_q >= 0 && k >= 1, "ccr_search_shard: bad shape n_q=%d k=%d", n_q, k);
    hipStream_t s = (hipStream_t)stream;
    ccr_shard_header h;
    memset(&h, 0, sizeof(h));
    h.magic = CCR_SHARD_MAGIC;
    h.k_valid = (uint32_t)k;
    h.n_covered = 0u;
    h.row_offset = ix->offset;
    h.n_rows = ix->n_rows;
    int rc = launch_shard_header(h, message, s);
    if (rc != CCR_OK) return rc;
    if (n_q == 0) return CCR_OK;
    char *m = (char *)message;
    uint32_t *flagged = reinterpret_cast<uint32_t *>(m + offsetof(ccr_shard_header, n_flagged));
    return search_impl(ix, Q_bf16, n_q, k, reinterpret_cast<float *>(m + sizeof(ccr_shard_header)),
                       reinterpret_cast<int64_t *>(m + shard_rows_at(n_q, k)), ID_LOCAL_U32, flagged, workspace, ws_bytes, flags, stream);
}

extern "C" int ccr_scores(const ccr_index *ix, const uint16_t *Q_bf16, int n_q, int mode, float *out, void *stream) {
    CCR_REQUIRE(ix && Q_bf16 && out && n_q > 0, "ccr_scores: bad argument");
    CCR_REQUIRE((uintptr_t)Q_bf16 % 16 == 0, "ccr_scores: query pointer must be 16-byte aligned");
    if (mode == CCR_SCORES_CANONICAL)
        return launch_dense_scores(ix->D, ix->n_rows, ix->dim, Q_bf16, nullptr, 0, n_q, nullptr, out, (hipStream_t)stream);
    CCR_REQUIRE(mode == CCR_SCORES_MFMA, "ccr_scores: unknown mode %d", mode);
    CCR_REQUIRE(ix->dim % 8 == 0, "ccr_scores: CCR_SCORES_MFMA needs dim %% 8 == 0 (dim=%d)", ix->dim);
    return store_scores(ix, Q_bf16, n_q, (int)round_up(std::min<int64_t>(64, tiles_of(ix)), NUM_XCD), out, 0, (hipStream_t)stream);
}
```

### crowd-coachable-recommendations_amd/csrc/ccr_common.h

```cpp
#pragma once
#include <hip/hip_runtime.h>
#include <stdint.h>
#include <stdio.h>

#include "ccr_retrieval.h"

namespace ccr {

void set_error(const char *fmt, ...);

#define CCR_HIP_CHECK(expr)                                                                   \
    do {                                                                                      \
        hipError_t _e = (expr);                                                               \
        if (_e != hipSuccess) {                                                               \
            ccr::set_error("%s failed: %s (%s:%d)", #expr, hipGetErrorString(_e), __FILE__, __LINE__); \
            return CCR_ERR_HIP;                                                               \
        }                                                                                     \
    } while (0)

#define CCR_REQUIRE(cond, ...)            \
    do {                                  \
        if (!(cond)) {                    \
            ccr::set_error(__VA_ARGS__);  \
            return CCR_ERR_INVALID;       \
        }                                 \
    } while (0)

#define CCR_LAUNCH_CHECK()                                                              \
    do {                                                                                \
        hipError_t _e = hipGetLastError();                                              \
        if (_e != hipSuccess) {                                                         \
            ccr::set_error("kernel launch failed: %s (%s:%d)", hipGetErrorString(_e), __FILE__, __LINE__); \
            return CCR_ERR_HIP;                                                         \
        }                                                                               \
    } while (0)

constexpr int TILE_DOCS = 256;
constexpr int TILE_Q = 256;
constexpr int WIDE_Q = 384;
constexpr int TILE_K = 32;
constexpr int GEMM_THREADS = 512;
constexpr int GROUPS_PER_TILE = 16;
constexpr int MAX_K = 4096;
constexpr uint32_t FLAG_DENSE = 0x80000000u;
constexpr int NUM_XCD = 8;

struct CandLayout {
    int nseg;
    int seg_end[3];
    int cap[3];
    long long base[3];
};
__host__ __device__ __forceinline__ void cand_segment(const CandLayout &L, int r, int &cap, int &r0, long long &base) {
    const int g = (r >= L.seg_end[0] ? 1 : 0) + (r >= L.seg_end[1] ? 1 : 0);
    r0 = g ? L.seg_end[g - 1] : 0;
    cap = L.cap[g];
    base = L.base[g];
}
__host__ __device__ __forceinline__ long long cand_sublist(const CandLayout &L, int r, int q, int s, int nq_pad, int sp, int &cap) {
    const int g = (r >= L.seg_end[0] ? 1 : 0) + (r >= L.seg_end[1] ? 1 : 0);
    const int r0 = g ? L.seg_end[g - 1] : 0;
    cap = L.cap[g];
    return L.base[g] + (((long long)(r - r0) * nq_pad + q) * sp) * (long long)cap + s;
}

struct Plan {
    int fused;
    int nq_pad;
    int qblocks;
    int tile_q;
    int main_qblocks;
    int main_qgroups;
    int64_t tiles;
    int64_t full_tiles;
    int sample_tiles;
    int64_t sample_stride;
    int sample_ranges;
    int ranges;
    int item_a;
    int item_b;
    int opt_rank;
    int qgroups;
    int cap;
    CandLayout cand;
    int grid;
    int rescore_cap;
    int select_compact;
    int mfma16;
    int sublists;
    int narrow;
    int narrow_groups;
    int first_nsub;
    int first_sp;
    CandLayout first_lay;
    int64_t cand_recs;
    size_t off_qnorm, off_thr, off_gmax, off_cnt, off_cand, off_flag, off_dense, off_retry, off_top, off_safe, total;
    int64_t dense_rows_per_chunk;
};

enum { EPI_FILTER = 0, EPI_GMAX = 1, EPI_STORE = 2 };

struct GemmArgs {
    const uint16_t *D;
    int64_t n_rows;
    int dim;
    const uint16_t *Q;
    int n_q;
    int nq_pad;
    int qblocks;
    int64_t n_vt;
    int64_t tile_stride;
    int ranges;
    int qgroups;
    int item_begin, item_end;
    const float *thr;
    const float *cq;
    const float *tile_norm;
    uint2 *cand;
    uint32_t *cnt;
    CandLayout lay;
    float *gmax;
    float *store;
    int64_t store_pitch;
};


__device__ __forceinline__ float bf16_bits_to_f32(uint16_t h) { return __uint_as_float(((uint32_t)h) << 16); }

__device__ __forceinline__ uint32_t f32_orderable(float f) {
    uint32_t u = __float_as_uint(f);
    return (u & 0x80000000u) ? ~u : (u | 0x80000000u);
}
__device__ __forceinline__ float orderable_to_f32(uint32_t u) {
    return __uint_as_float((u & 0x80000000u) ? (u & 0x7fffffffu) : ~u);
}

constexpr int64_t ID_LOCAL_U32 = INT64_MIN;
__device__ __forceinline__ void store_id(int64_t *out_ids, int64_t pos, int64_t id_offset, uint32_t row) {
    if (id_offset == ID_LOCAL_U32)
        reinterpret_cast<uint32_t *>(out_ids)[pos] = row;
    else
        out_ids[pos] = id_offset + (int64_t)row;
}

__host__ __device__ __forceinline__ float mfma_gamma(int dim) { return (float)dim * 1.1920929e-7f * 1.02f; }

}
```

### crowd-coachable-recommendations_amd/csrc/ccr_fused.hip

```cpp
#include <stdlib.h>

#include <mutex>
#include <set>
#include <type_traits>
#include <utility>

#include "ccr_gemm_common.h"
#include "ccr_index.h"
#include "ccr_topk_device.h"

namespace ccr {

__device__ __attribute__((aligned(16))) uint32_t g_zero_chunk[4];

__device__ __forceinline__ float load_uniform_f32(const float *p) {
    float v;
    asm volatile("s_load_dword %0, %1, 0x0\n\ts_waitcnt lgkmcnt(0)" : "=s"(v) : "s"(p) : "memory");
    return v;
}

template <int N>
__device__ __forceinline__ void wait_vm() {
    asm volatile("s_waitcnt vmcnt(%0)" ::"n"(N) : "memory");
}

typedef float f32x4v __attribute__((ext_vector_type(4)));

__device__ __forceinline__ float max4_asm(const f32x4v &c) {
    float m;
    asm("v_max3_f32 %0, %1, %2, %3\n\tv_max_f32 %0, %0, %4" : "=&v"(m) : "v"(c[0]), "v"(c[1]), "v"(c[2]), "v"(c[3]));
    return m;
}
__device__ __forceinline__ float max3_asm(float a, float b, float c) {
    float m;
    asm("v_max3_f32 %0, %1, %2, %3" : "=v"(m) : "v"(a), "v"(b), "v"(c));
    return m;
}

struct ItemWalk {
    int jx, step, qg, rc, nrc, qb_per, end;
    __device__ __forceinline__ explicit ItemWalk(const GemmArgs &a) {
        const int xcd = blockIdx.x & (NUM_XCD - 1);
        jx = blockIdx.x >> 3;
        step = gridDim.x >> 3;
        qg = xcd % a.qgroups;
        rc = xcd / a.qgroups;
        nrc = NUM_XCD / a.qgroups;
        qb_per = a.qblocks / a.qgroups;
        const int count_x = (a.ranges / nrc) * qb_per;
        end = a.item_end < count_x ? a.item_end : count_x;
    }
    __device__ __forceinline__ int first(const GemmArgs &a) const { return a.item_begin + jx; }
    __device__ __forceinline__ int64_t item(const GemmArgs &a, int i, int &r, int &qb) const {
        const int rl = i / qb_per;
        const int b = qg * qb_per + i % qb_per;
        const int ri = rc + nrc * rl;
        const int64_t ntile = (a.n_vt - ri + a.ranges - 1) / a.ranges;
        r = ri;
        qb = b;
        return ntile;
    }
};


struct Mfma32 {
    typedef f32x16 Acc;
    static constexpr int TILE = 32, REGS = 16, DT = 4, QT = 2, SUBLISTS = 4;
    struct Frags { bf16x8 a[2][4], b[2][2]; };

    static __device__ __forceinline__ int src_swizzle(int row) { return (row >> 2) & 3; }

    int a_base, b_base, cofs[2];
    __device__ __forceinline__ Mfma32(int lane, int wd, int wq) {
        const int swz = (lane >> 2) & 3;
#pragma unroll
        for (int ks = 0; ks < 2; ++ks) cofs[ks] = (((2 * ks + (lane >> 5)) ^ swz) << 4);
        a_base = (wd * 128 + (lane & 31)) * 64;
        b_base = SUB_Q_REGION + (wq * 64 + (lane & 31)) * 64;
    }
    __device__ __forceinline__ void read(const char *buf, Frags &f) const {
#pragma unroll
        for (int ks = 0; ks < 2; ++ks) {
#pragma unroll
            for (int dt = 0; dt < 4; ++dt) f.a[ks][dt] = *reinterpret_cast<const bf16x8 *>(buf + a_base + dt * 2048 + cofs[ks]);
#pragma unroll
            for (int qt = 0; qt < 2; ++qt) f.b[ks][qt] = *reinterpret_cast<const bf16x8 *>(buf + b_base + qt * 2048 + cofs[ks]);
        }
    }
    static __device__ __forceinline__ void mma(Acc (&acc)[4][2], const Frags &f, bool first) {
        if (first) {
            const f32x16 z = {0.f, 0.f, 0.f, 0.f, 0.f, 0.f, 0.f, 0.f, 0.f, 0.f, 0.f, 0.f, 0.f, 0.f, 0.f, 0.f};
#pragma unroll
            for (int dt = 0; dt < 4; ++dt)
#pragma unroll
                for (int qt = 0; qt < 2; ++qt) acc[dt][qt] = __builtin_amdgcn_mfma_f32_32x32x16_bf16(f.a[0][dt], f.b[0][qt], z, 0, 0, 0);
        } else {
#pragma unroll
            for (int dt = 0; dt < 4; ++dt)
#pragma unroll
                for (int qt = 0; qt < 2; ++qt) acc[dt][qt] = __builtin_amdgcn_mfma_f32_32x32x16_bf16(f.a[0][dt], f.b[0][qt], acc[dt][qt], 0, 0, 0);
        }
#pragma unroll
        for (int dt = 0; dt < 4; ++dt)
#pragma unroll
            for (int qt = 0; qt < 2; ++qt) acc[dt][qt] = __builtin_amdgcn_mfma_f32_32x32x16_bf16(f.a[1][dt], f.b[1][qt], acc[dt][qt], 0, 0, 0);
    }

    static __device__ __forceinline__ void tile_max(const Acc (&acc)[4][2], int qt, float (&sub)[4][4], float (&mdt)[4]) {
#pragma unroll
        for (int dt = 0; dt < 4; ++dt) {
#pragma unroll
            for (int g = 0; g < 4; ++g)
                sub[dt][g] = fmaxf(fmaxf(acc[dt][qt][4 * g], acc[dt][qt][4 * g + 1]), fmaxf(acc[dt][qt][4 * g + 2], acc[dt][qt][4 * g + 3]));
            mdt[dt] = fmaxf(fmaxf(sub[dt][0], sub[dt][1]), fmaxf(sub[dt][2], sub[dt][3]));
        }
    }
    static __device__ __forceinline__ void gmax(const Acc (&acc)[4][2], const GemmArgs &a, int64_t vt, int q0, int wd, int wq, int lane) {
        const int h = lane >> 5;
#pragma unroll
        for (int qt = 0; qt < 2; ++qt) {
            float sub[4][4], mdt[4];
            tile_max(acc, qt, sub, mdt);
            const int ql = wq * 64 + qt * 32 + (lane & 31);
#pragma unroll
            for (int dt = 0; dt < 4; ++dt) a.gmax[(vt * GROUPS_PER_TILE + wd * 8 + dt * 2 + h) * a.nq_pad + q0 + ql] = mdt[dt];
        }
    }
    static __device__ __forceinline__ void filter(const Acc (&acc)[4][2], const float (&thr)[2], const float (&cqv)[2], float nt,
                                                  int64_t row_base, const GemmArgs &a, uint2 *const (&clist)[2], uint32_t (&ncand)[2],
                                                  int cap) {
        const uint32_t row32 = (uint32_t)row_base;
        const int64_t left = a.n_rows - row_base;
        const uint32_t rows_left = left <= 0 ? 0u : (left > 128 ? 128u : (uint32_t)left);
#pragma unroll
        for (int qt = 0; qt < 2; ++qt) {
            float sub[4][4], mdt[4];
            tile_max(acc, qt, sub, mdt);
            const float t = fmaf(-cqv[qt], nt, thr[qt]);
            const float mall = fmaxf(fmaxf(mdt[0], mdt[1]), fmaxf(mdt[2], mdt[3]));
            if (__ballot(mall >= t) == 0ull) continue;
#pragma unroll
            for (int dt = 0; dt < 4; ++dt) {
                if (__ballot(mdt[dt] >= t) == 0ull) continue;
#pragma unroll
                for (int g = 0; g < 4; ++g) {
                    if (sub[dt][g] >= t) {
#pragma unroll
                        for (int e2 = 0; e2 < 4; ++e2) {
                            const float v = acc[dt][qt][4 * g + e2];
                            const uint32_t off = (uint32_t)(dt * 32 + 8 * g + e2);
                            if (v >= t && off < rows_left) {
                                if (ncand[qt] < (uint32_t)cap) clist[qt][ncand[qt] * 4] = make_uint2(__float_as_uint(v), row32 + off);
                                ++ncand[qt];
                            }
                        }
                    }
                }
            }
        }
    }
};

struct Mfma16 {
    typedef f32x4v Acc;
    static constexpr int TILE = 16, REGS = 4, DT = 8, QT = 4, SUBLISTS = 8;
    struct Frags { bf16x8 a[8], b[4]; };

    static __device__ __forceinline__ int src_swizzle(int row) { return ((row >> 2) & 1) << 1; }

    int a_base, b_base;
    __device__ __forceinline__ Mfma16(int lane, int wd, int wq) {
        const int cofs = (((lane >> 4) ^ (((lane >> 2) & 1) << 1)) << 4);
        a_base = (wd * 128 + (lane & 15)) * 64 + cofs;
        b_base = SUB_Q_REGION + (wq * 64 + (lane & 15)) * 64 + cofs;
    }
    __device__ __forceinline__ void read(const char *buf, Frags &f) const {
#pragma unroll
        for (int dt = 0; dt < 8; ++dt) f.a[dt] = *reinterpret_cast<const bf16x8 *>(buf + a_base + dt * 1024);
#pragma unroll
        for (int qt = 0; qt < 4; ++qt) f.b[qt] = *reinterpret_cast<const bf16x8 *>(buf + b_base + qt * 1024);
    }
    static __device__ __forceinline__ void mma(Acc (&acc)[8][4], const Frags &f, bool first) {
        if (first) {
            const f32x4v z = {0.f, 0.f, 0.f, 0.f};
#pragma unroll
            for (int dt = 0; dt < 8; ++dt)
#pragma unroll
                for (int qt = 0; qt < 4; ++qt) acc[dt][qt] = __builtin_amdgcn_mfma_f32_16x16x32_bf16(f.a[dt], f.b[qt], z, 0, 0, 0);
            return;
        }
#pragma unroll
        for (int dt = 0; dt < 8; ++dt)
#pragma unroll
            for (int qt = 0; qt < 4; ++qt) acc[dt][qt] = __builtin_amdgcn_mfma_f32_16x16x32_bf16(f.a[dt], f.b[qt], acc[dt][qt], 0, 0, 0);
    }

    static __device__ __forceinline__ void filter(const Acc (&acc)[8][4], const float (&thr)[4], const float (&cqv)[4], float nt,
                                                  int64_t row_base, const GemmArgs &a, uint2 *const (&clist)[4], uint32_t (&ncand)[4],
                                                  int cap) {
#pragma unroll
        for (int qt = 0; qt < 4; ++qt) {
            float sub[8];
#pragma unroll
            for (int dt = 0; dt < 8; ++dt) sub[dt] = max4_asm(acc[dt][qt]);
            const float t = fmaf(-cqv[qt], nt, thr[qt]);
            float mall = max3_asm(sub[0], sub[1], sub[2]);
            mall = max3_asm(mall, sub[3], sub[4]);
            mall = max3_asm(mall, sub[5], sub[6]);
            mall = fmaxf(mall, sub[7]);
            if (__ballot(mall >= t) == 0ull) continue;
#pragma unroll
            for (int dt = 0; dt < 8; ++dt) {
                if (sub[dt] >= t) {
#pragma unroll
                    for (int e = 0; e < 4; ++e) {
                        const float v = acc[dt][qt][e];
                        const int64_t doc = row_base + dt * 16 + e;
                        if (v >= t && doc < a.n_rows) {
                            if (ncand[qt] < (uint32_t)cap) clist[qt][ncand[qt] * 8] = make_uint2(__float_as_uint(v), (uint32_t)doc);
                            ++ncand[qt];
                        }
                    }
                }
            }
        }
    }
};

template <class S, int EPI, bool TAIL>
__device__ __forceinline__ void main_pass_256(const GemmArgs &a) {
    static_assert(EPI != EPI_GMAX || std::is_same<S, Mfma32>::value, "EPI_GMAX exists on the 32x32 shape only");
    extern __shared__ __attribute__((aligned(16))) char smem[];

    const int tid = threadIdx.x & (GEMM_THREADS - 1);
    const int lane = tid & 63;
    const int wv = __builtin_amdgcn_readfirstlane(tid >> 6);
    const int wd = wv >> 2;
    const int wq = wv & 3;
    const int lc = lane & (S::TILE - 1);
    const int lh = lane / S::TILE;
    const int cell = wd * (S::SUBLISTS / 2) + lh;
    const bool g1 = (wv >= 4);
    const int KS2 = TAIL ? (a.dim + SUB_K - 1) / SUB_K : a.dim / SUB_K;

    const int srow = wv * 16 + (lane >> 2);
    const int schunk = (lane & 3) ^ S::src_swizzle(srow);
    const S mfma(lane, wd, wq);

    const ItemWalk walk(a);
    for (int item = walk.first(a); item < walk.end; item += walk.step) {
        int r, qb;
        const int64_t ntile = walk.item(a, item, r, qb);
        if (ntile <= 0) continue;
        const int q0 = qb * TILE_Q;

        float thr[S::QT] = {}, cqv[S::QT] = {};
        uint32_t ncand[S::QT] = {};
        uint2 *clist[S::QT] = {};
        int cap = 0;
        if (EPI == EPI_FILTER) {
            int seg_r0;
            long long seg_base;
            cand_segment(a.lay, r, cap, seg_r0, seg_base);
#pragma unroll
            for (int qt = 0; qt < S::QT; ++qt) {
                const int q = q0 + wq * 64 + qt * S::TILE + lc;
                thr[qt] = (q < a.n_q) ? a.thr[q] : __builtin_nanf("");
                cqv[qt] = (q < a.n_q) ? a.cq[q] : 0.f;
                clist[qt] = a.cand + seg_base + ((int64_t)(r - seg_r0) * a.nq_pad + q) * S::SUBLISTS * cap + cell;
            }
#pragma unroll
            for (int qt = 0; qt < S::QT; ++qt) asm volatile("" : "+v"(thr[qt]), "+v"(cqv[qt]));
        }
        float *dst[S::QT] = {};
        if (EPI == EPI_STORE) {
            const int64_t pitch = a.store_pitch ? a.store_pitch : a.n_rows;
#pragma unroll
            for (int qt = 0; qt < S::QT; ++qt) {
                const int q = q0 + wq * 64 + qt * S::TILE + lc;
                if (q < a.n_q) dst[qt] = a.store + (int64_t)q * pitch;
            }
        }
        const uint16_t *qsrc[2];
#pragma unroll
        for (int i = 0; i < 2; ++i) {
            int qrow = q0 + i * 128 + srow;
            if (qrow > a.n_q - 1) qrow = a.n_q - 1;
            qsrc[i] = a.Q + (int64_t)qrow * a.dim + schunk * 8;
        }

        typename S::Acc acc[S::DT][S::QT];
        const int64_t U = ntile * KS2;

        int64_t iu = 0, it = 0;
        int iks = 0;
        const uint16_t *dsrc[2];
        auto tile_ptrs = [&]() {
            const int64_t row0 = (r + it * a.ranges) * a.tile_stride * TILE_DOCS;
#pragma unroll
            for (int i = 0; i < 2; ++i) {
                int64_t drow = row0 + (i * 128 + srow);
                if (drow > a.n_rows - 1) drow = a.n_rows - 1;
                dsrc[i] = a.D + drow * a.dim + schunk * 8;
            }
        };
        tile_ptrs();
        auto issue = [&]() {
            char *buf = smem + (int)(iu & (RING - 1)) * SUB_BYTES;
            const int k0 = iks * SUB_K;
            if (TAIL && iks == KS2 - 1) {
                const bool in = k0 + schunk * 8 < a.dim;
#pragma unroll
                for (int i = 0; i < 2; ++i)
                    glds16(in ? (const void *)(dsrc[i] + k0) : (const void *)g_zero_chunk, buf + (i * 512 + wv * 64) * 16);
#pragma unroll
                for (int i = 0; i < 2; ++i)
                    glds16(in ? (const void *)(qsrc[i] + k0) : (const void *)g_zero_chunk, buf + SUB_Q_REGION + (i * 512 + wv * 64) * 16);
            } else {
#pragma unroll
                for (int i = 0; i < 2; ++i) glds16(dsrc[i] + k0, buf + (i * 512 + wv * 64) * 16);
#pragma unroll
                for (int i = 0; i < 2; ++i) glds16(qsrc[i] + k0, buf + SUB_Q_REGION + (i * 512 + wv * 64) * 16);
            }
            ++iu;
            if (++iks == KS2) {
                iks = 0;
                ++it;
                tile_ptrs();
            }
        };

        auto epilogue = [&](int64_t vt, float nt) {
            const int64_t row_base = vt * a.tile_stride * TILE_DOCS + wd * 128 + 4 * lh;
            if constexpr (EPI == EPI_GMAX) {
                S::gmax(acc, a, vt, q0, wd, wq, lane);
            } else if constexpr (EPI == EPI_FILTER) {
                S::filter(acc, thr, cqv, nt, row_base, a, clist, ncand, cap);
            } else {
                const int64_t pitch = a.store_pitch ? a.store_pitch : a.n_rows;
#pragma unroll
                for (int qt = 0; qt < S::QT; ++qt) {
                    if (!dst[qt]) continue;
#pragma unroll
                    for (int dt = 0; dt < S::DT; ++dt)
#pragma unroll
                        for (int g = 0; g < S::REGS / 4; ++g) {
                            const int64_t doc = row_base + dt * S::TILE + 8 * g;
                            if ((pitch & 3) == 0 && doc + 3 < a.n_rows) {
                                *reinterpret_cast<float4 *>(dst[qt] + doc) = make_float4(acc[dt][qt][4 * g], acc[dt][qt][4 * g + 1],
                                                                                             acc[dt][qt][4 * g + 2], acc[dt][qt][4 * g + 3]);
                            } else {
#pragma unroll
                                for (int e2 = 0; e2 < 4; ++e2)
                                    if (doc + e2 < a.n_rows) dst[qt][doc + e2] = acc[dt][qt][4 * g + e2];
                            }
                        }
                }
            }
        };

        const int npro = U < 3 ? (int)U : 3;
        for (int i = 0; i < npro; ++i) issue();
        if (npro == 3)
            CCR_WAIT_VM(8);
        else if (npro == 2)
            CCR_WAIT_VM(4);
        else
            CCR_WAIT_VM(0);
        CCR_BARRIER();
        if (g1) CCR_BARRIER();

        int cks = 0;
        int64_t ct = 0;
        bool pending = false;
        int64_t pending_vt = 0;
        float pending_nt = 0.f;
        for (int64_t u = 0; u < U; ++u) {
            if (pending) {
                epilogue(pending_vt, pending_nt);
                pending = false;
            }
            if (u + 1 < U) {
                if (u + 2 < U)
                    CCR_WAIT_VM(4);
                else
                    CCR_WAIT_VM(0);
            }
            typename S::Frags f;
            mfma.read(smem + (int)(u & (RING - 1)) * SUB_BYTES, f);
            if (u + 3 < U) issue();
            CCR_WAIT_LGKM0();
            CCR_BARRIER();
            S::mma(acc, f, cks == 0);
            if (++cks == KS2) {
                cks = 0;
                const int64_t vt_done = r + ct * a.ranges;
                const float nt_done = EPI == EPI_FILTER ? load_uniform_f32(a.tile_norm + vt_done * a.tile_stride) : 0.f;
                if (g1) {
                    epilogue(vt_done, nt_done);
                } else {
                    pending = true;
                    pending_vt = vt_done;
                    pending_nt = nt_done;
                }
                ++ct;
            }
            CCR_BARRIER();
        }
        if (pending) epilogue(pending_vt, pending_nt);
        if (!g1) CCR_BARRIER();

        if (EPI == EPI_FILTER) {
#pragma unroll
            for (int qt = 0; qt < S::QT; ++qt)
                a.cnt[((int64_t)r * a.nq_pad + q0 + wq * 64 + qt * S::TILE + lc) * S::SUBLISTS + cell] = ncand[qt];
        }
        __syncthreads();
    }
}

template <int EPI, bool TAIL = false>
__global__ __launch_bounds__(GEMM_THREADS, 2) void gemm_topk_kernel(const GemmArgs a) { main_pass_256<Mfma32, EPI, TAIL>(a); }
template <int EPI, bool TAIL = false>
__global__ __launch_bounds__(GEMM_THREADS, 2) void gemm_topk16_kernel(const GemmArgs a) { main_pass_256<Mfma16, EPI, TAIL>(a); }


__device__ __forceinline__ int fresh_lane() {
    int l;
    asm volatile("v_mbcnt_lo_u32_b32 %0, -1, 0\n\tv_mbcnt_hi_u32_b32 %0, -1, %0" : "=v"(l));
    return l;
}
__device__ __forceinline__ uint32_t lds_offset(const void *p) {
    return (uint32_t)(uintptr_t)(const __attribute__((address_space(3))) void *)p;
}
__device__ __forceinline__ float2 lds_read_f2(uint32_t addr) {
    uint64_t v;
    asm volatile("ds_read_b64 %0, %1\n\ts_waitcnt lgkmcnt(0)" : "=v"(v) : "v"(addr) : "memory");
    return make_float2(__uint_as_float((uint32_t)v), __uint_as_float((uint32_t)(v >> 32)));
}
__device__ __forceinline__ uint32_t lds_add_rtn(uint32_t addr, uint32_t x) {
    uint32_t r;
    asm volatile("ds_add_rtn_u32 %0, %1, %2\n\ts_waitcnt lgkmcnt(0)" : "=v"(r) : "v"(addr), "v"(x) : "memory");
    return r;
}
constexpr int WIDE_SUB_BYTES = (TILE_DOCS + WIDE_Q) * SUB_K * 2;
constexpr int WIDE_Q_REGION = TILE_DOCS * SUB_K * 2;
constexpr int WIDE_RING = 3;
constexpr int WIDE_PIECES = 5;
constexpr int WIDE_QT = 6;
#ifndef WIDE_BFR
#define WIDE_BFR 6
#endif
constexpr int WIDE_RING_BYTES = WIDE_RING * WIDE_SUB_BYTES;
constexpr size_t WIDE_LDS = (size_t)WIDE_RING_BYTES + WIDE_Q * 8 + (size_t)(GEMM_THREADS / 64) * WIDE_QT * 64 * 4;

__global__ __launch_bounds__(GEMM_THREADS, 2) void gemm_topk16w_kernel(const GemmArgs a) {
    extern __shared__ __attribute__((aligned(16))) char smem[];
    float2 *s_tc = reinterpret_cast<float2 *>(smem + WIDE_RING_BYTES);
    uint32_t *s_cnt = reinterpret_cast<uint32_t *>(smem + WIDE_RING_BYTES + WIDE_Q * 8);
    const int wv = __builtin_amdgcn_readfirstlane((int)threadIdx.x >> 6);
    const int wd = wv >> 2;
    const int wq = wv & 3;
    const bool g1 = (wv >= 4);
    const int KS2 = a.dim / SUB_K;
    const uint32_t pitch = (uint32_t)a.dim * 2u;
    uint32_t lane_src, lane_lds;
    {
        const int ln = fresh_lane();
        const int pr = ln >> 2;
        lane_src = (uint32_t)pr * pitch + (uint32_t)(((ln & 3) ^ (((pr >> 2) & 1) << 1)) << 4);
        lane_lds = (uint32_t)((ln & 15) * 64 + (((ln >> 4) ^ (((ln >> 2) & 1) << 1)) << 4));
    }

    const ItemWalk walk(a);
    for (int item = walk.first(a); item < walk.end; item += walk.step) {
        int r, qb;
        const int64_t ntile = walk.item(a, item, r, qb);
        if (ntile <= 0) continue;
        const int q0 = qb * WIDE_Q;

        int cap, seg_r0;
        long long seg_base;
        cand_segment(a.lay, r, cap, seg_r0, seg_base);
        {
            const int ln = fresh_lane();
            const int tid = wv * 64 + ln;
            if (tid < WIDE_Q) {
                const int q = q0 + tid;
                s_tc[tid] = make_float2((q < a.n_q) ? a.thr[q] : __builtin_nanf(""), (q < a.n_q) ? a.cq[q] : 0.f);
            }
#pragma unroll
            for (int qt = 0; qt < WIDE_QT; ++qt) s_cnt[(wv * WIDE_QT + qt) * 64 + ln] = 0u;
        }
        CCR_WAIT_VM(0);

        const int qlimit = (a.n_q - 1 - q0 < WIDE_Q - 1) ? a.n_q - 1 - q0 : WIDE_Q - 1;
        const char *qblk = reinterpret_cast<const char *>(a.Q) + (int64_t)q0 * pitch;

        f32x4v acc[8][WIDE_QT];
        const int U = (int)(ntile * KS2);
        int islot = 0, iks = 0;
        int64_t it = 0;
        const char *dtile = nullptr;
        int dlimit = 0;
        auto tile_base = [&]() __attribute__((always_inline)) {
            const int64_t row0 = (r + it * a.ranges) * a.tile_stride * TILE_DOCS;
            dlimit = (a.n_rows - 1 - row0 < TILE_DOCS - 1) ? (int)(a.n_rows - 1 - row0) : TILE_DOCS - 1;
            dtile = reinterpret_cast<const char *>(a.D) + row0 * pitch;
        };
        tile_base();
        const bool q_whole = g1 ? ((wv - 4) * 96 + 95 <= qlimit) : (wv * 96 + 15 <= qlimit);
        auto issue = [&]() __attribute__((always_inline)) {
            char *buf = smem + islot * WIDE_SUB_BYTES;
            const uint32_t kb = (uint32_t)iks * (SUB_K * 2);
            if (q_whole && (g1 || dlimit == TILE_DOCS - 1)) {
                const uint32_t voff = lane_src + kb;
                if (!g1) {
                    const char *rows = dtile + (size_t)(wv * 64) * pitch;
#pragma unroll
                    for (int i = 0; i < 4; ++i) glds16(rows + (size_t)(i * 16) * pitch + voff, buf + (wv * 4 + i) * 1024);
                    glds16(qblk + (size_t)(wv * 96) * pitch + voff, buf + WIDE_Q_REGION + wv * 96 * 64);
                } else {
                    const char *rows = qblk + (size_t)((wv - 4) * 96 + 16) * pitch;
                    char *dst = buf + WIDE_Q_REGION + ((wv - 4) * 96 + 16) * 64;
#pragma unroll
                    for (int i = 0; i < WIDE_PIECES; ++i) glds16(rows + (size_t)(i * 16) * pitch + voff, dst + i * 1024);
                }
            } else {
                const int iln = fresh_lane();
                const int pr = iln >> 2;
                const uint32_t co = (uint32_t)(((iln & 3) ^ (((pr >> 2) & 1) << 1)) << 4) + kb;
                auto piece = [&](const char *rows, int row0, int limit, char *dst) __attribute__((always_inline)) {
                    int row = row0 + pr;
                    row = row < limit ? row : limit;
                    glds16(rows + ((uint32_t)row * pitch + co), dst);
                };
                if (!g1) {
#pragma unroll
                    for (int i = 0; i < 4; ++i) piece(dtile, (wv * 4 + i) * 16, dlimit, buf + (wv * 4 + i) * 1024);
                    piece(qblk, wv * 96, qlimit, buf + WIDE_Q_REGION + wv * 96 * 64);
                } else {
#pragma unroll
                    for (int i = 0; i < WIDE_PIECES; ++i)
                        piece(qblk, (wv - 4) * 96 + 16 * (1 + i), qlimit, buf + WIDE_Q_REGION + ((wv - 4) * 96 + 16 * (1 + i)) * 64);
                }
            }
            islot = islot == WIDE_RING - 1 ? 0 : islot + 1;
            if (++iks == KS2) {
                iks = 0;
                ++it;
                if (!g1) tile_base();
            }
        };

        auto epilogue = [&](int64_t vt, float nt) __attribute__((always_inline)) {
            const int eln = fresh_lane();
            const int l15o = eln & 15, lqo = eln >> 4;
            char *const cbase = reinterpret_cast<char *>(a.cand + seg_base + ((int64_t)(r - seg_r0) * a.nq_pad + q0) * 8 * cap + wd * 4);
            const uint32_t row_lo = (uint32_t)(wd * 128 + 4 * lqo);
            const uint32_t tc_addr = lds_offset(s_tc) + (uint32_t)l15o * 8u;
            const uint32_t cnt_addr = lds_offset(s_cnt) + (uint32_t)(lqo * 16 + l15o) * 4u;
            const int64_t tile_row0 = vt * a.tile_stride * TILE_DOCS;
            const uint32_t rows_left = a.n_rows - tile_row0 < TILE_DOCS ? (uint32_t)(a.n_rows - tile_row0) : (uint32_t)TILE_DOCS;
#pragma unroll
            for (int qt = 0; qt < WIDE_QT; ++qt) {
                float sub[8];
#pragma unroll
                for (int dt = 0; dt < 8; ++dt) sub[dt] = max4_asm(acc[dt][qt]);
                const float2 tc = lds_read_f2(tc_addr + (uint32_t)(wq * 96 + qt * 16) * 8u);
                const float t = fmaf(-tc.y, nt, tc.x);
                float mall = max3_asm(sub[0], sub[1], sub[2]);
                mall = max3_asm(mall, sub[3], sub[4]);
                mall = max3_asm(mall, sub[5], sub[6]);
                mall = fmaxf(mall, sub[7]);
                if (__ballot(mall >= t) != 0ull) {
                    const uint32_t ql = (uint32_t)(wq * 96 + qt * 16 + l15o);
                    const uint32_t cell = (ql * 8u * (uint32_t)cap + (uint32_t)lqo) * 8u;
                    const uint32_t cn = cnt_addr + (uint32_t)((wv * WIDE_QT + qt) * 64) * 4u;
#pragma unroll
                    for (int dt = 0; dt < 8; ++dt) {
                        if (sub[dt] >= t) {
#pragma unroll
                            for (int e = 0; e < 4; ++e) {
                                const float v = acc[dt][qt][e];
                                const uint32_t row = row_lo + dt * 16 + e;
                                if (v >= t && row < rows_left) {
                                    const uint32_t n = lds_add_rtn(cn, 1u);
                                    if (n < (uint32_t)cap)
                                        *reinterpret_cast<uint2 *>(cbase + (cell + n * 64u)) = make_uint2(__float_as_uint(v), (uint32_t)tile_row0 + row);
                                }
                            }
                        }
                    }
                }
            }
        };

        const int npro = U < 2 ? U : 2;
        for (int i = 0; i < npro; ++i) issue();
        if (npro == 2)
            wait_vm<WIDE_PIECES>();
        else
            CCR_WAIT_VM(0);
        CCR_BARRIER();
        if (g1) CCR_BARRIER();

        int cks = 0;
        int64_t ct = 0;
        bool pending = false;
        int64_t pending_vt = 0;
        float pending_nt = 0.f;
        int uslot = 0;
        for (int u = 0; u < U; ++u) {
            if (u + 2 < U) issue();
            __builtin_amdgcn_sched_barrier(0);
            if (pending) {
                epilogue(pending_vt, pending_nt);
                pending = false;
            }
            const char *abuf = smem + uslot * WIDE_SUB_BYTES;
            const char *bbuf = abuf + WIDE_Q_REGION;
            uslot = uslot == WIDE_RING - 1 ? 0 : uslot + 1;
            const int a_base = wd * 128 * 64 + (int)lane_lds;
            const int b_base = wq * 96 * 64 + (int)lane_lds;
            bf16x8 af[8], bfr[WIDE_BFR];
#pragma unroll
            for (int dt = 0; dt < 8; ++dt) af[dt] = *reinterpret_cast<const bf16x8 *>(abuf + a_base + dt * 1024);
#pragma unroll
            for (int qt = 0; qt < WIDE_BFR; ++qt) bfr[qt] = *reinterpret_cast<const bf16x8 *>(bbuf + b_base + qt * 1024);
            if (u + 2 < U)
                wait_vm<WIDE_PIECES>();
            else
                CCR_WAIT_VM(0);
            CCR_WAIT_LGKM0();
            CCR_BARRIER();
            if (cks == 0) {
                const f32x4v z = {0.f, 0.f, 0.f, 0.f};
#pragma unroll
                for (int qt = 0; qt < WIDE_QT; ++qt) {
#pragma unroll
                    for (int dt = 0; dt < 8; ++dt) acc[dt][qt] = __builtin_amdgcn_mfma_f32_16x16x32_bf16(af[dt], bfr[qt % WIDE_BFR], z, 0, 0, 0);
                    if (WIDE_BFR == 3 && qt < 3) {
                        __builtin_amdgcn_sched_barrier(0);
                        bfr[qt] = *reinterpret_cast<const bf16x8 *>(bbuf + b_base + (qt + 3) * 1024);
                        __builtin_amdgcn_sched_barrier(0);
                    }
                }
            } else {
#pragma unroll
                for (int qt = 0; qt < WIDE_QT; ++qt) {
#pragma unroll
                    for (int dt = 0; dt < 8; ++dt)
                        acc[dt][qt] = __builtin_amdgcn_mfma_f32_16x16x32_bf16(af[dt], bfr[qt % WIDE_BFR], acc[dt][qt], 0, 0, 0);
                    if (WIDE_BFR == 3 && qt < 3) {
                        __builtin_amdgcn_sched_barrier(0);
                        bfr[qt] = *reinterpret_cast<const bf16x8 *>(bbuf + b_base + (qt + 3) * 1024);
                        __builtin_amdgcn_sched_barrier(0);
                    }
                }
            }
            if (++cks == KS2) {
                cks = 0;
                const int64_t vt_done = r + ct * a.ranges;
                const float nt_done = load_uniform_f32(a.tile_norm + vt_done * a.tile_stride);
                if (g1) {
                    epilogue(vt_done, nt_done);
                } else {
                    pending = true;
                    pending_vt = vt_done;
                    pending_nt = nt_done;
                }
                ++ct;
            }
            CCR_WAIT_LGKM0();
            CCR_BARRIER();
        }
        if (pending) epilogue(pending_vt, pending_nt);
        if (!g1) CCR_BARRIER();

        {
            const int ln = fresh_lane();
#pragma unroll
            for (int qt = 0; qt < WIDE_QT; ++qt)
                a.cnt[((int64_t)r * a.nq_pad + q0 + wq * 96 + qt * 16 + (ln & 15)) * 8 + wd * 4 + (ln >> 4)] = s_cnt[(wv * WIDE_QT + qt) * 64 + ln];
        }
        __syncthreads();
    }
}

__global__ __launch_bounds__(256) void row_norms_bf16_kernel(const uint16_t *__restrict__ X, int64_t rows, int dim,
                                                            float *__restrict__ norms, uint32_t *__restrict__ max_bits,
                                                            uint32_t *__restrict__ tile_bits) {
    const int lane = threadIdx.x & 63;
    const int64_t wave = ((int64_t)blockIdx.x * blockDim.x + threadIdx.x) >> 6;
    const int64_t nwaves = ((int64_t)gridDim.x * blockDim.x) >> 6;
    const int chunk = tile_bits ? 64 : 1;
    uint32_t wbits = 0u;
    for (int64_t r0 = wave * chunk; r0 < rows; r0 += nwaves * chunk) {
        uint32_t cbits = 0u;
        const int64_t r1 = r0 + chunk < rows ? r0 + chunk : rows;
        for (int64_t r = r0; r < r1; ++r) {
            const uint16_t *x = X + r * dim;
            float s = 0.f;
            for (int c = lane * 8; c < dim; c += 64 * 8) {
                const uint4 v = *reinterpret_cast<const uint4 *>(x + c);
                const uint32_t w[4] = {v.x, v.y, v.z, v.w};
#pragma unroll
                for (int e = 0; e < 4; ++e) {
                    const float lo = __uint_as_float(w[e] << 16), hi = __uint_as_float(w[e] & 0xffff0000u);
                    s = fmaf(lo, lo, s);
                    s = fmaf(hi, hi, s);
                }
            }
#pragma unroll
            for (int off = 32; off >= 1; off >>= 1) s += __shfl_xor(s, off, 64);
            const float n = sqrtf(s);
            if (norms && lane == 0) norms[r] = n;
            const uint32_t nb = __float_as_uint(n) & 0x7fffffffu;
            cbits = nb > cbits ? nb : cbits;
        }
        if (tile_bits && lane == 0) atomicMax(tile_bits + r0 / TILE_DOCS, cbits);
        wbits = cbits > wbits ? cbits : wbits;
    }
    if (max_bits && lane == 0 && wbits > __hip_atomic_load(max_bits, __ATOMIC_RELAXED, __HIP_MEMORY_SCOPE_AGENT)) atomicMax(max_bits, wbits);
}

__global__ __launch_bounds__(256) void tile_norms_kernel(const float *__restrict__ row_bounds, int64_t rows,
                                                        uint32_t *__restrict__ tile_bits) {
    __shared__ uint32_t s_w[4];
    const int64_t r = (int64_t)blockIdx.x * TILE_DOCS + threadIdx.x;
    uint32_t b = r < rows ? (__float_as_uint(row_bounds[r]) & 0x7fffffffu) : 0u;
#pragma unroll
    for (int off = 32; off >= 1; off >>= 1) {
        const uint32_t o = __shfl_xor(b, off, 64);
        b = o > b ? o : b;
    }
    if ((threadIdx.x & 63) == 0) s_w[threadIdx.x >> 6] = b;
    __syncthreads();
    if (threadIdx.x == 0) {
        const uint32_t m01 = s_w[0] > s_w[1] ? s_w[0] : s_w[1], m23 = s_w[2] > s_w[3] ? s_w[2] : s_w[3];
        tile_bits[blockIdx.x] = m01 > m23 ? m01 : m23;
    }
}

__global__ __launch_bounds__(1024) void max_tile_norm_kernel(const uint32_t *__restrict__ tile_bits, int64_t tiles,
                                                            uint32_t *__restrict__ max_bits) {
    __shared__ uint32_t s_w[16];
    uint32_t b = 0u;
    for (int64_t t = threadIdx.x; t < tiles; t += 1024) {
        const uint32_t v = tile_bits[t];
        b = v > b ? v : b;
    }
#pragma unroll
    for (int off = 32; off >= 1; off >>= 1) {
        const uint32_t o = __shfl_xor(b, off, 64);
        b = o > b ? o : b;
    }
    if ((threadIdx.x & 63) == 0) s_w[threadIdx.x >> 6] = b;
    __syncthreads();
    if (threadIdx.x == 0) {
        uint32_t m = 0u;
        for (int w = 0; w < 16; ++w) m = s_w[w] > m ? s_w[w] : m;
        *max_bits = m;
    }
}

__global__ __launch_bounds__(256) void threshold_kernel(const float *__restrict__ gmax, int64_t n_groups, int n_q, int nq_pad,
                                                       int k, const float *__restrict__ qnorm,
                                                       const uint32_t *__restrict__ dmax_bits, float gamma,
                                                       const float *__restrict__ tile_norm, int64_t sample_stride,
                                                       float *__restrict__ thr, float *__restrict__ cq) {
    __shared__ uint32_t s_hist[16][256];
    __shared__ uint32_t s_prefix[16], s_remaining[16];
    const int tid = threadIdx.x;
    const int ql = tid & 15, ph = tid >> 4;
    const int q = blockIdx.x * 16 + ql;
    if (tid < 16) {
        s_prefix[tid] = 0;
        s_remaining[tid] = (uint32_t)k;
    }
    const float dmax = __uint_as_float(*dmax_bits);
    const float c = (q < n_q) ? ((dmax < INFINITY) ? gamma * (qnorm[q] * 1.001f) * 1.001f : __builtin_nanf("")) : 0.f;
    auto tile_of = [&](int64_t g) { return tile_norm[(g / GROUPS_PER_TILE) * sample_stride]; };
    uint32_t mask = 0;
    for (int shift = 24; shift >= 0; shift -= 8) {
        for (int b = tid; b < 16 * 256; b += 256) (&s_hist[0][0])[b] = 0;
        __syncthreads();
        const uint32_t prefix = s_prefix[ql];
        int64_t i = ph;
        for (; i + 240 < n_groups; i += 256) {
            float v[16], tn[16];
#pragma unroll
            for (int j = 0; j < 16; ++j) {
                v[j] = gmax[(i + 16 * j) * nq_pad + q];
                tn[j] = tile_of(i + 16 * j);
            }
#pragma unroll
            for (int j = 0; j < 16; ++j) {
                const uint32_t o = f32_orderable(fmaf(-c, tn[j], v[j]));
                if ((o & mask) == prefix) atomicAdd(&s_hist[ql][(o >> shift) & 255u], 1u);
            }
        }
        for (; i < n_groups; i += 16) {
            const uint32_t o = f32_orderable(fmaf(-c, tile_of(i), gmax[i * nq_pad + q]));
            if ((o & mask) == prefix) atomicAdd(&s_hist[ql][(o >> shift) & 255u], 1u);
        }
        __syncthreads();
        {
            const int qi = tid >> 4, part = tid & 15;
            const uint32_t remaining = s_remaining[qi];
            uint32_t hb[16];
            uint32_t own = 0;
#pragma unroll
            for (int j = 0; j < 16; ++j) {
                hb[j] = s_hist[qi][16 * part + j];
                own += hb[j];
            }
            uint32_t incl = own;
#pragma unroll
            for (int off = 1; off < 16; off <<= 1) {
                const uint32_t t = __shfl_down(incl, off, 16);
                if (part + off < 16) incl += t;
            }
            const uint32_t above = incl - own;
            const uint32_t total = __shfl(incl, 0, 16);
            __syncthreads();
            if (above < remaining && remaining <= incl) {
                uint32_t cum = above;
                int d = 16 * part;
#pragma unroll
                for (int j = 15; j >= 1; --j) {
                    if (cum + hb[j] >= remaining) {
                        d = 16 * part + j;
                        break;
                    }
                    cum += hb[j];
                }
                s_prefix[qi] |= (uint32_t)d << shift;
                s_remaining[qi] = remaining - cum;
            } else if (part == 0 && total < remaining) {
                s_remaining[qi] = remaining - (total - hb[0]);
            }
        }
        mask |= 0xffu << shift;
        __syncthreads();
    }
    if (tid < 16) {
        const int qq = blockIdx.x * 16 + tid;
        if (qq < n_q) {
            const float tau = orderable_to_f32(s_prefix[tid]);
            cq[qq] = c;
            thr[qq] = (c < INFINITY) ? tau : __builtin_nanf("");
        }
    }
}


template <int THREADS, int BATCH, class At, class Want, class Put>
__device__ __forceinline__ void sweep_sublists(int tid, int n_lists, int first, int longest, const uint32_t *s_cnt, At at,
                                               Want want, Put put) {
    if (longest <= first) return;
    int lw = 0;
    while ((1 << lw) < longest - first) ++lw;
    const int sweep = n_lists << lw;
    for (int i0 = tid; i0 < sweep; i0 += THREADS * BATCH) {
        uint2 e[BATCH];
        int jj[BATCH], ss[BATCH];
#pragma unroll
        for (int u = 0; u < BATCH; ++u) {
            const int i = i0 + u * THREADS;
            const int j = i >> lw, sl = first + (i & ((1 << lw) - 1));
            jj[u] = -1;
            ss[u] = sl;
            if (i < sweep && (uint32_t)sl < s_cnt[j] && want(j, sl)) {
                jj[u] = j;
                e[u] = at(j, sl);
            }
        }
#pragma unroll
        for (int u = 0; u < BATCH; ++u)
            if (jj[u] >= 0) put(jj[u], ss[u], e[u]);
    }
}

__global__ __launch_bounds__(256) void threshold_update_kernel(const uint2 *__restrict__ cand, const uint32_t *__restrict__ cnt,
                                                              int nsub_full, int nsub_part, int part_blocks, int prev_full,
                                                              int prev_part, int prev_blocks, int qb_per, int sp, int nq_pad,
                                                              const CandLayout lay, int k, int compact,
                                                              const float *__restrict__ cq, const float *__restrict__ tile_norm,
                                                              uint32_t *__restrict__ top, int top_in, int top_out,
                                                              float *__restrict__ thr, int tile_q) {
    extern __shared__ __attribute__((aligned(16))) uint32_t s_val[];
    __shared__ uint32_t s_hist[256];
    __shared__ uint32_t s_ctl[4];
    __shared__ uint32_t s_cnt[2048];
    __shared__ uint32_t s_total, s_maxc, s_fill, s_eq;
    const int tid = threadIdx.x;
    const int q = blockIdx.x;
    const int qpos = (q / tile_q) % qb_per;
    const int nsub = qpos < part_blocks ? nsub_part : nsub_full;
    uint32_t *top_n = top;
    uint32_t *top_v = top ? top + nq_pad + (int64_t)q * k : nullptr;
    const bool have_prev = top_in && top_n[q] == (uint32_t)k;
    const int j0 = have_prev ? (qpos < prev_blocks ? prev_part : prev_full) : 0;
    if (tid == 0) {
        s_total = have_prev ? (uint32_t)k : 0u;
        s_maxc = 0;
        s_fill = 0;
    }
    __syncthreads();
    uint32_t my = 0, mymax = 0;
    for (int j = j0 + tid; j < nsub; j += blockDim.x) {
        uint32_t c = cnt[((int64_t)(j / sp) * nq_pad + q) * sp + (j % sp)];
        int cap;
        (void)cand_sublist(lay, j / sp, q, j % sp, nq_pad, sp, cap);
        if (c > (uint32_t)cap) c = (uint32_t)cap;
        s_cnt[j - j0] = c;
        my += c;
        mymax = c > mymax ? c : mymax;
    }
    if (my) {
        atomicAdd(&s_total, my);
        atomicMax(&s_maxc, mymax);
    }
    __syncthreads();
    if (s_total < (uint32_t)k) {
        if (top_out && tid == 0) top_n[q] = 0u;
        return;
    }
    auto sub_base = [&](int j) -> int64_t {
        int cap;
        return cand_sublist(lay, (j0 + j) / sp, q, (j0 + j) % sp, nq_pad, sp, cap);
    };
    uint32_t kth = 0;
    int need_eq = 0, M = 0;
    bool selected = false;
    {
        const int maxc = (int)s_maxc;
        const float c = cq[q];
        uint32_t keep = 0u;
        auto append = [&](uint32_t o) {
            if (o >= keep) {
                const uint32_t p = atomicAdd(&s_fill, 1u);
                if (p < (uint32_t)compact) s_val[p] = o;
            }
        };
        for (int round = 0; round < 4; ++round) {
            __syncthreads();
            if (tid == 0) s_fill = 0;
            __syncthreads();
            selected = false;
            if (have_prev)
                for (int i = tid; i < k; i += blockDim.x) append(top_v[i]);
            sweep_sublists<256, 8>(
                tid, nsub - j0, 0, maxc, s_cnt, [&](int j, int sl) -> uint2 { return cand[sub_base(j) + (int64_t)sl * sp]; },
                [](int, int) { return true; },
                [&](int, int, uint2 e) { append(f32_orderable(fmaf(-c, tile_norm[e.y / TILE_DOCS], __uint_as_float(e.x)))); });
            __syncthreads();
            const uint32_t filled = s_fill;
            M = (int)(filled < (uint32_t)compact ? filled : (uint32_t)compact);
            if (M < k) break;
            block_radix_select(
                [&](int64_t i, bool &skip) -> uint32_t {
                    (void)skip;
                    return s_val[i];
                },
                (int64_t)M, k, s_hist, s_ctl, kth, need_eq);
            selected = true;
            if (filled <= (uint32_t)compact || kth <= keep) break;
            keep = kth;
        }
    }
    if (top_out) {
        if (!selected) {
            if (tid == 0) top_n[q] = 0u;
        } else {
            __syncthreads();
            if (tid == 0) s_fill = s_eq = 0u;
            __syncthreads();
            for (int i = tid; i < M; i += blockDim.x) {
                const uint32_t v = s_val[i];
                bool take = v > kth;
                if (v == kth) take = atomicAdd(&s_eq, 1u) < (uint32_t)need_eq;
                if (take) top_v[atomicAdd(&s_fill, 1u)] = v;
            }
            if (tid == 0) top_n[q] = (uint32_t)k;
        }
    }
    if (tid == 0) {
        const float t1 = orderable_to_f32(kth);
        if (t1 > thr[q]) thr[q] = t1;
    }
}

template <int THREADS>
__global__ __launch_bounds__(THREADS) void select_rescore_kernel(const uint2 *__restrict__ cand, const uint32_t *__restrict__ cnt,
                                                            int ranges, int sp, int nq_pad, const CandLayout lay, int k, int rescore_cap, int compact,
                                                            int64_t n_rows, float *__restrict__ thr, const float *__restrict__ cq,
                                                            const float *__restrict__ tile_norm, const float *__restrict__ row_norm,
                                                            const uint32_t *__restrict__ dmax_bits,
                                                            const uint16_t *__restrict__ Q, const uint16_t *__restrict__ D,
                                                            int dim, int64_t id_offset, float *__restrict__ out_scores,
                                                            int64_t *__restrict__ out_ids, uint32_t *__restrict__ flag_count,
                                                            uint32_t *__restrict__ flag_list,
                                                            unsigned long long *__restrict__ stat_cand,
                                                            const uint32_t *__restrict__ out_rows) {
    extern __shared__ __attribute__((aligned(16))) char sm[];
    const size_t cnt_bytes = ((size_t)(ranges + 1) * 4 + 15) & ~(size_t)15;
    uint16_t *s_q = reinterpret_cast<uint16_t *>(sm);
    uint32_t *s_cnt = reinterpret_cast<uint32_t *>(sm + (((size_t)dim * 2 + 15) & ~(size_t)15));
    uint32_t *s_off = reinterpret_cast<uint32_t *>(reinterpret_cast<char *>(s_cnt) + cnt_bytes);
    unsigned long long *s_keys = reinterpret_cast<unsigned long long *>(reinterpret_cast<char *>(s_off) + cnt_bytes);
    uint2 *s_comp = reinterpret_cast<uint2 *>(s_keys + rescore_cap);
    __shared__ uint32_t s_hist[256];
    __shared__ uint32_t s_ctl[4];
    __shared__ uint32_t s_wsum[THREADS / 64];
    __shared__ int s_flag;
    __shared__ uint32_t s_total, s_maxc, s_fill;
    __shared__ uint32_t s_ncoll;

    const int tid = threadIdx.x;
    const int q = blockIdx.x;
    if (tid == 0) {
        s_flag = 0;
        s_total = 0;
        s_ncoll = 0;
        s_maxc = 0;
        s_fill = 0;
    }
    __syncthreads();
    const int per = (ranges + THREADS - 1) / THREADS;
    uint32_t my = 0, mymax = 0;
    for (int j = tid * per; j < min(ranges, tid * per + per); ++j) {
        uint32_t c = cnt[((int64_t)(j / sp) * nq_pad + q) * sp + (j % sp)];
        int cap;
        (void)cand_sublist(lay, j / sp, q, j % sp, nq_pad, sp, cap);
        if (c > (uint32_t)cap) {
            s_flag = 1;
            c = (uint32_t)cap;
        }
        s_cnt[j] = c;
        my += c;
        mymax = c > mymax ? c : mymax;
    }
    {
        const int lane = tid & 63, wid = tid >> 6;
        uint32_t incl = my;
#pragma unroll
        for (int off = 1; off < 64; off <<= 1) {
            const uint32_t t = __shfl_up(incl, off, 64);
            if (lane >= off) incl += t;
        }
        if (lane == 63) s_wsum[wid] = incl;
        if (my) atomicMax(&s_maxc, mymax);
        for (int c = tid; c < dim / 8; c += THREADS)
            reinterpret_cast<uint4 *>(s_q)[c] = reinterpret_cast<const uint4 *>(Q + (int64_t)q * dim)[c];
        __syncthreads();
        uint32_t base = incl - my;
        for (int w = 0; w < wid; ++w) base += s_wsum[w];
        for (int j = tid * per; j < min(ranges, tid * per + per); ++j) {
            s_off[j] = base;
            base += s_cnt[j];
        }
        if (tid == THREADS - 1) s_total = base;
        __syncthreads();
    }
    if (tid == 0 && stat_cand) atomicAdd(stat_cand, (unsigned long long)s_total);
    bool bad = (s_flag != 0) || (s_total < (uint32_t)k);
    bool dense_only = (s_flag == 0) && bad;
    if (dense_only && thr && tid == 0) thr[q] = -INFINITY;

    auto sub_base = [&](int j) -> int64_t {
        int cap;
        return cand_sublist(lay, j / sp, q, j % sp, nq_pad, sp, cap);
    };
    auto at = [&](int j, int sl) -> uint2 { return cand[sub_base(j) + (int64_t)sl * sp]; };
    const int coll_cap = rescore_cap;
    uint32_t kth = 0;
    int need_eq = 0;
    int n_lds = 0;
    const float c = cq[q];
    bool row_lb = false;

    if (!bad && s_total <= (uint32_t)compact) {
        constexpr int FIRST = THREADS >= 1024 ? 8 : 4, MAXL = 8;
        {
            const int per_cell = FIRST * sp / 2;
            const int nload = (ranges / sp) * per_cell;
            uint4 v[MAXL];
#pragma unroll
            for (int t = 0; t < MAXL; ++t) {
                const int x = tid + t * THREADS;
                if (x < nload) {
                    const int cell = x / per_cell, w = x - cell * per_cell;
                    int cap;
                    v[t] = *reinterpret_cast<const uint4 *>(cand + cand_sublist(lay, cell, q, 0, nq_pad, sp, cap) + 2 * w);
                }
            }
#pragma unroll
            for (int t = 0; t < MAXL; ++t) {
                const int x = tid + t * THREADS;
                if (x < nload) {
                    const int cell = x / per_cell, w = x - cell * per_cell;
                    const int slot = (2 * w) / sp, part = (2 * w) % sp;
                    const int j = cell * sp + part;
                    if ((uint32_t)slot < s_cnt[j]) s_comp[s_off[j] + slot] = make_uint2(v[t].x, v[t].y);
                    if ((uint32_t)slot < s_cnt[j + 1]) s_comp[s_off[j + 1] + slot] = make_uint2(v[t].z, v[t].w);
                }
            }
        }
        sweep_sublists<THREADS, 8>(tid, ranges, FIRST, (int)s_maxc, s_cnt, at, [](int, int) { return true; },
                                   [&](int j, int sl, uint2 e) { s_comp[s_off[j] + sl] = e; });
        __syncthreads();
        n_lds = (int)s_total;
        for (int i0 = tid; i0 < n_lds; i0 += 4 * THREADS) {
            uint2 e[4];
            float rn[4];
#pragma unroll
            for (int u = 0; u < 4; ++u) {
                const int i = i0 + u * THREADS;
                e[u] = s_comp[i < n_lds ? i : i0];
                rn[u] = tile_norm[e[u].y / TILE_DOCS];
            }
#pragma unroll
            for (int u = 0; u < 4; ++u) {
                const int i = i0 + u * THREADS;
                if (i < n_lds) s_comp[i] = make_uint2(__float_as_uint(fmaf(-c, rn[u], __uint_as_float(e[u].x))), e[u].y);
            }
        }
        __syncthreads();
    } else if (!bad && compact < k) {
        bad = dense_only = true;
    } else if (!bad) {
        float keep = -INFINITY;
        bool fits = false;
        row_lb = true;
        for (int round = 0; round < 4 && !fits; ++round) {
            __syncthreads();
            if (tid == 0) s_fill = 0u;
            __syncthreads();
            sweep_sublists<THREADS, 8>(tid, ranges, 0, (int)s_maxc, s_cnt, at, [](int, int) { return true; },
                                       [&](int, int, uint2 e) {
                                           const float cn = c * row_norm[e.y];
                                           if (__uint_as_float(e.x) + cn >= keep) {
                                               const uint32_t p = atomicAdd(&s_fill, 1u);
                                               if (p < (uint32_t)compact) s_comp[p] = make_uint2(__float_as_uint(__uint_as_float(e.x) - cn), e.y);
                                           }
                                       });
            __syncthreads();
            if (s_fill <= (uint32_t)compact) {
                fits = true;
            } else {
                uint32_t kth0 = 0;
                int eq0 = 0;
                block_radix_select(
                    [&](int64_t i, bool &skip) -> uint32_t {
                        (void)skip;
                        return f32_orderable(__uint_as_float(s_comp[i].x));
                    },
                    compact, k, s_hist, s_ctl, kth0, eq0);
                keep = orderable_to_f32(kth0);
            }
        }
        if (fits)
            n_lds = (int)s_fill;
        else
            bad = dense_only = true;
    }
    if (!bad) {
        const int M = n_lds;
        block_radix_select(
            [&](int64_t i, bool &skip) -> uint32_t {
                (void)skip;
                return f32_orderable(__uint_as_float(s_comp[i].x));
            },
            M, k, s_hist, s_ctl, kth, need_eq);
        const float low = orderable_to_f32(kth);
        if (thr && low < thr[q]) {
            __syncthreads();
            if (tid == 0) {
                thr[q] = low;
                const uint32_t p = atomicAdd(flag_count, 1u);
                flag_list[p] = (out_rows ? out_rows[q] : (uint32_t)q);
            }
            return;
        }
        const float loose = fmaf(-2.f * c, __uint_as_float(*dmax_bits), low);
        for (int i = tid; i < M; i += THREADS) {
            const uint2 e = s_comp[i];
            const float lb = __uint_as_float(e.x);
            if (lb >= loose && fmaf(c, row_norm[e.y], fmaf(c, row_lb ? row_norm[e.y] : tile_norm[e.y / TILE_DOCS], lb)) >= low) {
                const uint32_t p = atomicAdd(&s_ncoll, 1u);
                if (p < (uint32_t)coll_cap) s_keys[p] = (unsigned long long)e.y;
            }
        }
        __syncthreads();
        if (s_ncoll > (uint32_t)coll_cap) bad = dense_only = true;
    }
    if (bad) {
        if (tid == 0) {
            const uint32_t p = atomicAdd(flag_count, 1u);
            flag_list[p] = (out_rows ? out_rows[q] : (uint32_t)q) | (dense_only ? FLAG_DENSE : 0u);
        }
        return;
    }
    const int ncoll = (int)s_ncoll;
    const int np2 = pow2_ceil(ncoll);
    const size_t stage_bytes = (size_t)compact * 8;
    int SB = (size_t)ncoll * 144 <= stage_bytes ? 128 : ((size_t)ncoll * 80 <= stage_bytes ? 64 : 0);
    constexpr int PRE = 8;
    if (SB == 128 && ncoll * 8 > PRE * THREADS) SB = 64;
    if (SB != 0 && ncoll <= 2 * THREADS && ncoll * (SB / 16) <= PRE * THREADS) {
        char *stage = reinterpret_cast<char *>(s_comp);
        const int stride = SB + 16;
        const int lpr = SB / 16;
        const int row_bytes = dim * 2;
        const char *Dbytes = reinterpret_cast<const char *>(D);
        const int col = (tid % lpr) * 16;
#define CCR_PIECES(X) X(0) X(1) X(2) X(3) X(4) X(5) X(6) X(7)
        const int acol = col < row_bytes ? col : 0;
        const char *Dcol = Dbytes + acol;
        const int npiece = ncoll * lpr;
#define CCR_DECL(j)                                                                                              \
    const int idx##j = tid + j * THREADS;                                                                        \
    const char *src##j = Dcol + (int64_t)(uint32_t)s_keys[idx##j < npiece ? idx##j / lpr : 0] * row_bytes;      \
    uint4 pre##j = *reinterpret_cast<const uint4 *>(src##j);
        CCR_PIECES(CCR_DECL)
#undef CCR_DECL
        double acc[2] = {0.0, 0.0};
        for (int k0 = 0; k0 < row_bytes; k0 += SB) {
            __syncthreads();
            const bool col_in = k0 + col < row_bytes;
#define CCR_PUT(j) \
    if (col_in && idx##j < npiece) *reinterpret_cast<uint4 *>(stage + (idx##j / lpr) * stride + col) = pre##j;
            CCR_PIECES(CCR_PUT)
#undef CCR_PUT
            __syncthreads();
            {
                const int kn = (k0 + SB + col < row_bytes) ? k0 + SB : -acol;
#define CCR_GET(j) pre##j = *reinterpret_cast<const uint4 *>(src##j + kn);
                CCR_PIECES(CCR_GET)
#undef CCR_GET
            }
#undef CCR_PIECES
#pragma unroll
            for (int j = 0; j < 2; ++j) {
                const int i = tid + j * THREADS;
                if (i < ncoll) {
                    double a = acc[j];
                    for (int c = 0; c < lpr && k0 + c * 16 < row_bytes; ++c) {
                        const uint4 dv = *reinterpret_cast<const uint4 *>(stage + (size_t)i * stride + c * 16);
                        const uint4 qv = *reinterpret_cast<const uint4 *>(reinterpret_cast<const char *>(s_q) + k0 + c * 16);
                        const uint32_t dw[4] = {dv.x, dv.y, dv.z, dv.w};
                        const uint32_t qw[4] = {qv.x, qv.y, qv.z, qv.w};
#pragma unroll
                        for (int e = 0; e < 4; ++e) {
                            a = fma((double)__uint_as_float(qw[e] << 16), (double)__uint_as_float(dw[e] << 16), a);
                            a = fma((double)__uint_as_float(qw[e] & 0xffff0000u), (double)__uint_as_float(dw[e] & 0xffff0000u), a);
                        }
                    }
                    acc[j] = a;
                }
            }
        }
        __syncthreads();
#pragma unroll
        for (int j = 0; j < 2; ++j) {
            const int i = tid + j * THREADS;
            if (i < np2) s_keys[i] = i < ncoll ? make_key((float)acc[j], (uint32_t)s_keys[i]) : 0ull;
        }
    } else {
        for (int i = tid; i < np2; i += blockDim.x) {
            unsigned long long key = 0ull;
            if (i < ncoll) {
                const uint32_t row = (uint32_t)s_keys[i];
                key = make_key(canonical_dot(s_q, D + (int64_t)row * dim, dim), row);
            }
            s_keys[i] = key;
        }
    }
    block_bitonic_sort_desc(s_keys, np2);
    const int64_t orow = out_rows ? (int64_t)out_rows[q] : (int64_t)q;
    for (int i = tid; i < k; i += blockDim.x) {
        const unsigned long long key = s_keys[i];
        out_scores[orow * k + i] = key_score(key);
        store_id(out_ids, orow * k + i, id_offset, key_idx(key));
    }
}

__global__ __launch_bounds__(256) void partition_flags_kernel(const uint32_t *__restrict__ flags, int begin, int n,
                                                             uint32_t *__restrict__ retry_list, uint32_t *__restrict__ dense_list,
                                                             uint32_t *__restrict__ counts) {
    __shared__ uint32_t s_n[2];
    if (threadIdx.x == 0) s_n[0] = s_n[1] = 0;
    __syncthreads();
    for (int i = begin + threadIdx.x; i < n; i += blockDim.x) {
        const uint32_t f = flags[i];
        if (f & FLAG_DENSE)
            dense_list[atomicAdd(&s_n[1], 1u)] = f & ~FLAG_DENSE;
        else
            retry_list[atomicAdd(&s_n[0], 1u)] = f;
    }
    __syncthreads();
    if (threadIdx.x < 2) counts[threadIdx.x] = s_n[threadIdx.x];
}

__global__ __launch_bounds__(256) void underfilled_to_retry_kernel(uint32_t *__restrict__ flags, int begin, int n,
                                                                  const float *__restrict__ thr_safe, float *__restrict__ thr) {
    const int i = begin + blockIdx.x * blockDim.x + threadIdx.x;
    if (i >= n) return;
    const uint32_t f = flags[i];
    const uint32_t q = f & ~FLAG_DENSE;
    if ((f & FLAG_DENSE) && thr[q] == -INFINITY && thr_safe[q] > -INFINITY) {
        thr[q] = thr_safe[q];
        flags[i] = q;
    }
}

__global__ __launch_bounds__(256) void scatter_thresholds_kernel(const uint32_t *__restrict__ list, int n, const float *__restrict__ thr2,
                                                                float *__restrict__ thr) {
    const int i = blockIdx.x * blockDim.x + threadIdx.x;
    if (i < n) thr[list[i]] = thr2[i];
}

__global__ __launch_bounds__(256) void gather_queries_kernel(const uint16_t *__restrict__ Q, int dim, const uint32_t *__restrict__ list,
                                                            int n, const float *__restrict__ thr, const float *__restrict__ delta,
                                                            uint16_t *__restrict__ Q2, float *__restrict__ thr2,
                                                            float *__restrict__ delta2) {
    const int i = blockIdx.x;
    if (i >= n) return;
    const uint32_t q = list[i];
    for (int c = threadIdx.x; c < dim / 8; c += blockDim.x)
        reinterpret_cast<uint4 *>(Q2 + (int64_t)i * dim)[c] = reinterpret_cast<const uint4 *>(Q + (int64_t)q * dim)[c];
    if (threadIdx.x == 0) {
        thr2[i] = thr[q];
        delta2[i] = delta[q];
    }
}

int ensure_dynamic_lds(const void *kernel, size_t lds) {
    static std::mutex mu;
    static std::set<std::pair<const void *, int>> done;
    int dev = 0;
    CCR_HIP_CHECK(hipGetDevice(&dev));
    std::lock_guard<std::mutex> lock(mu);
    if (done.count({kernel, dev})) return CCR_OK;
    CCR_HIP_CHECK(hipFuncSetAttribute(kernel, hipFuncAttributeMaxDynamicSharedMemorySize, (int)lds));
    done.insert({kernel, dev});
    return CCR_OK;
}

template <class K>
static int launch_kernel(K kernel, size_t lds, const GemmArgs &a, int grid, hipStream_t s) {
    const int rc = ensure_dynamic_lds(reinterpret_cast<const void *>(kernel), lds);
    if (rc != CCR_OK) return rc;
    hipLaunchKernelGGL(kernel, dim3(grid), dim3(GEMM_THREADS), lds, s, a);
    CCR_LAUNCH_CHECK();
    return CCR_OK;
}

int launch_gemm(const GemmArgs &a, MainKernel kind, int epi, int grid, hipStream_t s) {
    if (epi != EPI_FILTER && epi != EPI_GMAX && epi != EPI_STORE) {
        set_error("launch_gemm: unknown epilogue %d", epi);
        return CCR_ERR_INVALID;
    }
    if (kind == MAIN_WIDE) {
        if (epi != EPI_FILTER || a.dim % SUB_K != 0 || a.dim < SUB_K) {
            set_error("launch_gemm: the 256 x 384 kernel takes EPI_FILTER and dim %% %d == 0 only (epi %d, dim %d)", SUB_K, epi, a.dim);
            return CCR_ERR_INVALID;
        }
        return launch_kernel(&gemm_topk16w_kernel, WIDE_LDS, a, grid, s);
    }
    typedef void (*Kernel)(const GemmArgs);
    static const Kernel k256[2][3][2] = {
        {{gemm_topk_kernel<EPI_FILTER>, gemm_topk_kernel<EPI_FILTER, true>},
         {gemm_topk_kernel<EPI_GMAX>, gemm_topk_kernel<EPI_GMAX, true>},
         {gemm_topk_kernel<EPI_STORE>, gemm_topk_kernel<EPI_STORE, true>}},
        {{gemm_topk16_kernel<EPI_FILTER>, gemm_topk16_kernel<EPI_FILTER, true>},
         {nullptr, nullptr},
         {gemm_topk16_kernel<EPI_STORE>, gemm_topk16_kernel<EPI_STORE, true>}},
    };
    const Kernel k = k256[kind == MAIN_16X16][epi][a.dim % SUB_K != 0];
    if (!k) {
        set_error("launch_gemm: the 16x16x32 kernel has no EPI_GMAX");
        return CCR_ERR_INVALID;
    }
    return launch_kernel(k, RING * (size_t)SUB_BYTES, a, grid, s);
}

int launch_row_norms_bf16(const uint16_t *X, int64_t rows, int dim, float *norms, uint32_t *max_bits, uint32_t *tile_bits,
                          hipStream_t s) {
    if (rows <= 0) return CCR_OK;
    int64_t blocks = tile_bits ? (rows + 255) / 256 : (rows + 3) / 4;
    if (blocks > 2048) blocks = 2048;
    hipLaunchKernelGGL(row_norms_bf16_kernel, dim3((unsigned)blocks), dim3(256), 0, s, X, rows, dim, norms, max_bits, tile_bits);
    CCR_LAUNCH_CHECK();
    return CCR_OK;
}

int launch_tile_norms(const float *row_bounds, int64_t rows, uint32_t *tile_bits, uint32_t *max_bits, hipStream_t s) {
    if (rows <= 0) return CCR_OK;
    const int64_t tiles = (rows + TILE_DOCS - 1) / TILE_DOCS;
    hipLaunchKernelGGL(tile_norms_kernel, dim3((unsigned)tiles), dim3(256), 0, s, row_bounds, rows, tile_bits);
    hipLaunchKernelGGL(max_tile_norm_kernel, dim3(1), dim3(1024), 0, s, tile_bits, tiles, max_bits);
    CCR_LAUNCH_CHECK();
    return CCR_OK;
}

__global__ __launch_bounds__(256) void threshold_small_kernel(const float *__restrict__ gmax, int n_groups, int nq_pad, int k,
                                                             const float *__restrict__ qnorm, const uint32_t *__restrict__ dmax_bits,
                                                             float gamma, const float *__restrict__ tile_norm, int64_t sample_stride,
                                                             float *__restrict__ thr, float *__restrict__ cq, uint32_t *__restrict__ zero_cnt,
                                                             int zero_per_query) {
    extern __shared__ __attribute__((aligned(16))) uint32_t s_low[];
    __shared__ uint32_t s_hist[256];
    __shared__ uint32_t s_ctl[4];
    const int tid = threadIdx.x, q = blockIdx.x;
    const float dmax = __uint_as_float(*dmax_bits);
    const float c = (dmax < INFINITY) ? gamma * (qnorm[q] * 1.001f) * 1.001f : __builtin_nanf("");
    for (int g = tid; g < n_groups; g += 256)
        s_low[g] = f32_orderable(fmaf(-c, tile_norm[(int64_t)(g / GROUPS_PER_TILE) * sample_stride], gmax[(int64_t)g * nq_pad + q]));
    if (zero_cnt && tid < zero_per_query) zero_cnt[q * zero_per_query + tid] = 0u;
    __syncthreads();
    uint32_t kth = 0;
    int need_eq = 0;
    block_radix_select<true>(
        [&](int64_t i, bool &skip) -> uint32_t {
            (void)skip;
            return s_low[i];
        },
        n_groups, k, s_hist, s_ctl, kth, need_eq);
    if (tid == 0) {
        cq[q] = c;
        thr[q] = (c < INFINITY) ? orderable_to_f32(kth) : __builtin_nanf("");
    }
}

int launch_threshold(const float *gmax, int64_t n_groups, int n_q, int nq_pad, int k, const float *qnorm,
                     const uint32_t *dmax_bits, int dim, const float *tile_norm, int64_t sample_stride, float *thr, float *cq,
                     hipStream_t s, uint32_t *zero_cnt, int zero_per_query) {
    if (n_q <= 128 && n_groups >= k && n_groups <= 16384 && zero_per_query <= 256) {
        if (n_groups * 4 > 32 * 1024) {
            const int rc = ensure_dynamic_lds(reinterpret_cast<const void *>(&threshold_small_kernel), 72 * 1024);
            if (rc != CCR_OK) return rc;
        }
        hipLaunchKernelGGL(threshold_small_kernel, dim3(n_q), dim3(256), (size_t)n_groups * 4, s, gmax, (int)n_groups, nq_pad, k, qnorm, dmax_bits,
                           mfma_gamma(dim), tile_norm, sample_stride, thr, cq, zero_cnt, zero_per_query);
        CCR_LAUNCH_CHECK();
        return CCR_OK;
    }
    if (zero_cnt) CCR_HIP_CHECK(hipMemsetAsync(zero_cnt, 0, (size_t)n_q * zero_per_query * 4, s));
    hipLaunchKernelGGL(threshold_kernel, dim3(nq_pad / 16), dim3(256), 0, s, gmax, n_groups, n_q, nq_pad, k, qnorm, dmax_bits,
                       mfma_gamma(dim), tile_norm, sample_stride, thr, cq);
    CCR_LAUNCH_CHECK();
    return CCR_OK;
}

int launch_threshold_update(const uint2 *cand, const uint32_t *cnt, int nsub, int nsub_part, int part_blocks, int prev_nsub, int prev_part,
                            int prev_blocks, int qb_per, int sp, int n_q, int nq_pad, const CandLayout &lay, int k, const float *cq,
                            const float *tile_norm, uint32_t *top, bool top_in, bool top_out, float *thr, hipStream_t s, int tile_q) {
    if (nsub_part < nsub) nsub_part = nsub;
    if (prev_part < prev_nsub) prev_part = prev_nsub;
    if (nsub_part > 2048) {
        set_error("threshold_update: %d sub-lists exceed 2048", nsub_part);
        return CCR_ERR_INVALID;
    }
    if (!top) top_in = top_out = false;
    int compact = std::max(4096, 8 * pow2_ceil(k));
    if (compact > 32768) compact = 32768;
    const size_t lds = (size_t)compact * 4;
    if (lds > 48 * 1024) {
        const int rc = ensure_dynamic_lds(reinterpret_cast<const void *>(&threshold_update_kernel), 128 * 1024);
        if (rc != CCR_OK) return rc;
    }
    hipLaunchKernelGGL(threshold_update_kernel, dim3(n_q), dim3(256), lds, s, cand, cnt, nsub, nsub_part, part_blocks, prev_nsub, prev_part,
                       prev_blocks, qb_per > 0 ? qb_per : 1, sp, nq_pad, lay, k, compact, cq, tile_norm, top, top_in ? 1 : 0, top_out ? 1 : 0,
                       thr, tile_q > 0 ? tile_q : TILE_Q);
    CCR_LAUNCH_CHECK();
    return CCR_OK;
}

constexpr size_t SELECT_LDS_BUDGET = 150 * 1024;

static size_t select_fixed_lds(int dim, int ranges, int rescore_cap) {
    const size_t cnt_bytes = ((size_t)(ranges + 1) * 4 + 15) & ~(size_t)15;
    return (((size_t)dim * 2 + 15) & ~(size_t)15) + 2 * cnt_bytes + (size_t)rescore_cap * 8;
}

int select_compact_entries(int dim, int ranges, int rescore_cap, int64_t want) {
    const size_t fixed = select_fixed_lds(dim, ranges, rescore_cap);
    const int64_t fit = fixed + 2048 < SELECT_LDS_BUDGET ? (int64_t)((SELECT_LDS_BUDGET - fixed) / 8) : 256;
    return (int)std::min<int64_t>(std::max<int64_t>(want, 2048), fit) / 256 * 256;
}

int launch_partition_flags(const uint32_t *flags, int begin, int n, uint32_t *retry_list, uint32_t *dense_list, uint32_t *counts,
                           hipStream_t s) {
    hipLaunchKernelGGL(partition_flags_kernel, dim3(1), dim3(256), 0, s, flags, begin, n, retry_list, dense_list, counts);
    CCR_LAUNCH_CHECK();
    return CCR_OK;
}

int launch_underfilled_to_retry(uint32_t *flags, int begin, int n, const float *thr_safe, float *thr, hipStream_t s) {
    if (n <= begin) return CCR_OK;
    hipLaunchKernelGGL(underfilled_to_retry_kernel, dim3((n - begin + 255) / 256), dim3(256), 0, s, flags, begin, n, thr_safe, thr);
    CCR_LAUNCH_CHECK();
    return CCR_OK;
}

int launch_scatter_thresholds(const uint32_t *list, int n, const float *thr2, float *thr, hipStream_t s) {
    if (n <= 0) return CCR_OK;
    hipLaunchKernelGGL(scatter_thresholds_kernel, dim3((n + 255) / 256), dim3(256), 0, s, list, n, thr2, thr);
    CCR_LAUNCH_CHECK();
    return CCR_OK;
}

int launch_gather_queries(const uint16_t *Q, int dim, const uint32_t *list, int n, const float *thr, const float *delta, uint16_t *Q2,
                          float *thr2, float *delta2, hipStream_t s) {
    if (n <= 0) return CCR_OK;
    hipLaunchKernelGGL(gather_queries_kernel, dim3(n), dim3(256), 0, s, Q, dim, list, n, thr, delta, Q2, thr2, delta2);
    CCR_LAUNCH_CHECK();
    return CCR_OK;
}

int launch_select_rescore(const uint2 *cand, const uint32_t *cnt, int ranges, int sp, int n_q, int nq_pad, const CandLayout &lay, int k,
                          int rescore_cap, int compact, int64_t n_rows, float *thr, const float *cq, const float *tile_norm, const float *row_norm,
                          const uint32_t *dmax_bits, const uint16_t *Q,
                          const uint16_t *D, int dim, int64_t id_offset, float *out_scores, int64_t *out_ids,
                          uint32_t *flag_count, uint32_t *flag_list, unsigned long long *stat_cand, const uint32_t *out_rows,
                          hipStream_t s) {
    const size_t lds = select_fixed_lds(dim, ranges, rescore_cap) + (size_t)compact * 8;
    const bool wide = rescore_cap > 512 || compact > 8192 || ranges > 1024;
    auto go = [&](auto kernel, int threads) -> int {
        if (lds > 48 * 1024) {
            const int rc = ensure_dynamic_lds(reinterpret_cast<const void *>(kernel), SELECT_LDS_BUDGET + 8192);
            if (rc != CCR_OK) return rc;
        }
        hipLaunchKernelGGL(kernel, dim3(n_q), dim3(threads), lds, s, cand, cnt, ranges, sp, nq_pad, lay, k, rescore_cap, compact,
                           n_rows, thr, cq, tile_norm, row_norm, dmax_bits, Q, D, dim, id_offset, out_scores, out_ids, flag_count, flag_list, stat_cand,
                           out_rows);
        CCR_LAUNCH_CHECK();
        return CCR_OK;
    };
    if (wide) return go(&select_rescore_kernel<1024>, 1024);
    return go(&select_rescore_kernel<256>, 256);
}

}
```

### crowd-coachable-recommendations_amd/csrc/ccr_index.h

```cpp
#pragma once
#include "ccr_common.h"

namespace ccr {

struct Knobs {
    int qgroups;
    int progressive;
    int max_phases;
    int mfma16;
    int sample_div;
    int ranges;
    int optimistic;
    int opt_rank;
    int max_lists;
    int narrow;
    int narrow_grid;
    int wide;
    int narrow_groups;
};
Knobs read_knobs();

constexpr int FALLBACK_ROWS = 16;

Plan make_plan(int64_t n_rows, int dim, int n_q, int k, int flags, int num_cu, const Knobs &kn);

struct Bump {
    size_t off;
    size_t take(size_t bytes) { const size_t o = off; off = (off + bytes + 255) / 256 * 256; return o; }
};

struct SearchWs {
    float *qnorm, *thr, *cq, *gmax;
    uint32_t *cnt;
    uint2 *cand;
    uint32_t *flag_count, *flag_list;
    unsigned long long *stat_cand;
    uint32_t *top;
    float *thr_safe, *cq_safe, *dense;
    uint16_t *Q2;
    float *thr2, *cq2;
    uint32_t *retry_list, *dense_list, *counts, *flag2, *list_b, *list_c;
    size_t cand_bytes, dense_bytes, retry_bytes, total;
};
SearchWs search_ws(const Plan &p, int64_t n_rows, int dim, int n_q, int k, char *base);

enum MainKernel { MAIN_32X32, MAIN_16X16, MAIN_WIDE };
int launch_gemm(const GemmArgs &a, MainKernel kind, int epi, int grid, hipStream_t s);
int launch_shard_header(const ccr_shard_header &h, void *message, hipStream_t s);
int ensure_dynamic_lds(const void *kernel, size_t lds);
int launch_row_norms_bf16(const uint16_t *X, int64_t rows, int dim, float *norms, uint32_t *max_bits, uint32_t *tile_bits,
                          hipStream_t s);
int launch_tile_norms(const float *row_bounds, int64_t rows, uint32_t *tile_bits, uint32_t *max_bits, hipStream_t s);
int launch_threshold(const float *gmax, int64_t n_groups, int n_q, int nq_pad, int k, const float *qnorm,
                     const uint32_t *dmax_bits, int dim, const float *tile_norm, int64_t sample_stride, float *thr, float *cq,
                     hipStream_t s, uint32_t *zero_cnt = nullptr, int zero_per_query = 0);
int select_compact_entries(int dim, int ranges, int rescore_cap, int64_t want);
int launch_select_rescore(const uint2 *cand, const uint32_t *cnt, int ranges, int sp, int n_q, int nq_pad, const CandLayout &lay, int k,
                          int rescore_cap, int compact, int64_t n_rows, float *thr, const float *cq, const float *tile_norm, const float *row_norm,
                          const uint32_t *dmax_bits, const uint16_t *Q, const uint16_t *D, int dim, int64_t id_offset, float *out_scores, int64_t *out_ids,
                          uint32_t *flag_count, uint32_t *flag_list, unsigned long long *stat_cand, const uint32_t *out_rows,
                          hipStream_t s);
int launch_partition_flags(const uint32_t *flags, int begin, int n, uint32_t *retry_list, uint32_t *dense_list, uint32_t *counts,
                           hipStream_t s);
int launch_underfilled_to_retry(uint32_t *flags, int begin, int n, const float *thr_safe, float *thr, hipStream_t s);
int launch_scatter_thresholds(const uint32_t *list, int n, const float *thr2, float *thr, hipStream_t s);
int launch_gather_queries(const uint16_t *Q, int dim, const uint32_t *list, int n, const float *thr, const float *cq, uint16_t *Q2,
                          float *thr2, float *cq2, hipStream_t s);
int launch_threshold_update(const uint2 *cand, const uint32_t *cnt, int nsub, int nsub_part, int part_blocks, int prev_nsub, int prev_part,
                            int prev_blocks, int qb_per, int sp, int n_q, int nq_pad, const CandLayout &lay, int k, const float *cq,
                            const float *tile_norm, uint32_t *top, bool top_in, bool top_out, float *thr, hipStream_t s, int tile_q = TILE_Q);
int launch_dense_scores(const uint16_t *D, int64_t n_rows, int dim, const uint16_t *Q, const uint32_t *qlist,
                        int q_begin, int nq_chunk, const uint32_t *count_dev, float *out, hipStream_t s);
int launch_dense_select(const float *scores, int64_t n_rows, int k, const uint32_t *out_rows, int q_begin, int nq_chunk,
                        const uint32_t *count_dev, int64_t id_offset, float *out_scores, int64_t *out_ids, hipStream_t s,
                        bool aggregate = true, const uint32_t *in_rows = nullptr, bool in_rows_compact = false);

int launch_margin_select(const float *scores, int64_t pitch, int64_t n_rows, int k, int dim, const uint16_t *Q, const uint16_t *D,
                         const float *tile_norm, const float *row_norm, const uint32_t *dmax_bits, const float *hint, const uint32_t *out_rows,
                         int q_begin, int nq_chunk, int64_t id_offset, float *out_scores, int64_t *out_ids, uint32_t *flag_count, uint32_t *flag_list,
                         hipStream_t s);

enum SearchEvent { EV_BEGIN, EV_SAMPLE_BEGIN, EV_SAMPLE_END, EV_MAIN_BEGIN, EV_MAIN_END, EV_SELECT_END, EV_DONE, EV_ASYNC_END, EV_COUNT };

}

struct ccr_index {
    const uint16_t *D;
    int64_t n_rows;
    int dim;
    int64_t offset;
    int64_t id_out;
    uint32_t *dmax_bits;
    float *tile_norm;
    size_t tile_bytes;
    const float *row_norm;
    float *row_norm_own;
    size_t row_bytes;
    bool have_events;
    bool main_pass_recorded;
    int num_cu;
    int device;
    ccr::Knobs knobs;
    hipEvent_t ev[ccr::EV_COUNT];
    volatile uint32_t *host_flags;
    ccr::Plan plan;
    int plan_nq, plan_k, plan_flags;
    ccr_search_stats stats;
    struct {
        bool active;
        const uint16_t *Q;
        int n_q, k;
        float *out_scores;
        int64_t *out_ids;
        char *ws;
        hipStream_t stream;
    } pending;
};
```

### crowd-coachable-recommendations_amd/csrc/ccr_topk_device.h

```cpp
#pragma once
#include "ccr_common.h"

namespace ccr {

__device__ __forceinline__ void radix_pick_digit(const uint32_t *hist, int lane, uint32_t remaining, uint32_t *ctl) {
    uint32_t h[4];
#pragma unroll
    for (int j = 0; j < 4; ++j) h[j] = hist[4 * lane + j];
    const uint32_t own = h[0] + h[1] + h[2] + h[3];
    uint32_t incl = own;
#pragma unroll
    for (int off = 1; off < 64; off <<= 1) {
        const uint32_t t = __shfl_down(incl, off, 64);
        if (lane + off < 64) incl += t;
    }
    const uint32_t above = incl - own;
    const bool cross = above < remaining && remaining <= incl;
    if (cross) {
        uint32_t cum = above;
        int d = 4 * lane;
#pragma unroll
        for (int j = 3; j >= 1; --j) {
            if (cum + h[j] >= remaining) {
                d = 4 * lane + j;
                break;
            }
            cum += h[j];
        }
        ctl[0] = (uint32_t)d;
        ctl[1] = remaining - cum;
    }
    if (lane == 0 && incl < remaining) {
        ctl[0] = 0u;
        ctl[1] = remaining - (incl - h[0]);
    }
}

__device__ __forceinline__ void hist_add_aggregated(uint32_t *hist, uint32_t bin, bool active) {
    const int lane = threadIdx.x & 63;
    unsigned long long todo = __ballot(active);
#pragma unroll 1
    for (int r = 0; r < 3 && todo != 0ull; ++r) {
        const int leader = __ffsll((long long)todo) - 1;
        const uint32_t lb = (uint32_t)__shfl((int)bin, leader, 64);
        const bool mine = active && bin == lb;
        const unsigned long long same = __ballot(mine);
        if (lane == leader) atomicAdd(&hist[lb], (uint32_t)__popcll(same));
        if (mine) active = false;
        todo &= ~same;
    }
    if (active) atomicAdd(&hist[bin], 1u);
}

template <bool AGG = false, class Get>
__device__ __forceinline__ void block_radix_select(Get get, int64_t M, int k, uint32_t *s_hist, uint32_t *s_ctl,
                                                   uint32_t &kth, int &need_eq) {
    const int tid = threadIdx.x;
    const int nt = blockDim.x;
    uint32_t prefix = 0, mask = 0;
    int remaining = k;
    for (int shift = 24; shift >= 0; shift -= 8) {
        for (int b = tid; b < 256; b += nt) s_hist[b] = 0;
        __syncthreads();
        if (AGG) {
            for (int64_t base = 0; base < M; base += nt) {
                const int64_t i = base + tid;
                bool skip = false;
                uint32_t o = 0;
                if (i < M) o = get(i, skip);
                hist_add_aggregated(s_hist, (o >> shift) & 255u, i < M && !skip && (o & mask) == prefix);
            }
        } else {
            for (int64_t i = tid; i < M; i += nt) {
                bool skip = false;
                uint32_t o = get(i, skip);
                if (!skip && (o & mask) == prefix) atomicAdd(&s_hist[(o >> shift) & 255u], 1u);
            }
        }
        __syncthreads();
        if (tid < 64) radix_pick_digit(s_hist, tid, (uint32_t)remaining, s_ctl);
        __syncthreads();
        prefix |= s_ctl[0] << shift;
        mask |= 0xffu << shift;
        remaining = (int)s_ctl[1];
        __syncthreads();
    }
    kth = prefix;
    need_eq = remaining;
}

__device__ __forceinline__ void block_bitonic_sort_desc(unsigned long long *keys, int n) {
    const int tid = threadIdx.x;
    const int nt = blockDim.x;
    for (int size = 2; size <= n; size <<= 1) {
        for (int stride = size >> 1; stride > 0; stride >>= 1) {
            __syncthreads();
            for (int i = tid; i < (n >> 1); i += nt) {
                const int pos = 2 * i - (i & (stride - 1));
                const unsigned long long a = keys[pos], b = keys[pos + stride];
                const bool desc = ((pos & size) == 0);
                if ((a < b) == desc) {
                    keys[pos] = b;
                    keys[pos + stride] = a;
                }
            }
        }
    }
    __syncthreads();
}

__device__ __forceinline__ unsigned long long make_key(float score, uint32_t local_idx) {
    return ((unsigned long long)f32_orderable(score) << 32) | (unsigned long long)(~local_idx);
}
__device__ __forceinline__ float key_score(unsigned long long key) { return orderable_to_f32((uint32_t)(key >> 32)); }
__device__ __forceinline__ uint32_t key_idx(unsigned long long key) { return ~(uint32_t)key; }

__host__ __device__ __forceinline__ int pow2_ceil(int v) {
    int p = 1;
    while (p < v) p <<= 1;
    return p;
}

__device__ __forceinline__ float canonical_dot(const uint16_t *__restrict__ q, const uint16_t *__restrict__ d, int dim) {
    double acc = 0.0;
#pragma unroll 4
    for (int c = 0; c < dim; c += 8) {
        const uint4 dv = *reinterpret_cast<const uint4 *>(d + c);
        const uint4 qv = *reinterpret_cast<const uint4 *>(q + c);
        const uint32_t dw[4] = {dv.x, dv.y, dv.z, dv.w};
        const uint32_t qw[4] = {qv.x, qv.y, qv.z, qv.w};
#pragma unroll
        for (int e = 0; e < 4; ++e) {
            acc = fma((double)__uint_as_float(qw[e] << 16), (double)__uint_as_float(dw[e] << 16), acc);
            acc = fma((double)__uint_as_float(qw[e] & 0xffff0000u), (double)__uint_as_float(dw[e] & 0xffff0000u), acc);
        }
    }
    return (float)acc;
}


}
```

### include/ccr_retrieval.h

```cpp
#ifndef CCR_RETRIEVAL_H
#define CCR_RETRIEVAL_H

#include <stddef.h>
#include <stdint.h>

#ifdef __cplusplus
extern "C" {
#endif

#define CCR_OK 0
#define CCR_ERR_INVALID (-1)
#define CCR_ERR_HIP (-2)
#define CCR_ERR_WORKSPACE (-3)
#define CCR_ERR_BLOCK_ID (-4)

#define CCR_DTYPE_F32 0
#define CCR_DTYPE_F16 1
#define CCR_DTYPE_BF16 2

#define CCR_SEARCH_DEFAULT 0
#define CCR_SEARCH_FORCE_DENSE 1
#define CCR_SEARCH_FORCE_FUSED 2
#define CCR_SEARCH_ASYNC 4

#define CCR_SCORES_CANONICAL 0
#define CCR_SCORES_MFMA 1

typedef struct ccr_index ccr_index;

typedef struct ccr_search_stats {
    int32_t path;
    int32_t n_fallback;
    int32_t sample_tiles;
    int32_t ranges;
    int32_t cap;
    int32_t sublists;
    int64_t n_candidates;
    float ms_sample;
    float ms_threshold;
    float ms_main;
    float ms_select;
    float ms_fallback;
    float ms_total;
    int32_t n_retried;
    int32_t n_dense;
    int32_t main_launches;
    int32_t opt_rank;
    int32_t main_tile_queries;
    int32_t reserved0;
} ccr_search_stats;

const char *ccr_last_error(void);
int ccr_version(void);

int ccr_pack_bf16(const float *src, uint16_t *dst, float *norms, int64_t rows, int dim, int normalize, void *stream);
int ccr_pack_bf16_ex(const float *src, uint16_t *dst, float *norms, float *row_norm_bounds, int64_t rows, int dim, int normalize,
                     void *stream);

int ccr_pack_bf16_padded(const float *src, int64_t rows, int src_dim, uint16_t *dst, int dst_dim, float *norms,
                         float *row_norm_bounds, int normalize, void *stream);

int ccr_meanpool_pack_bf16(const void *hidden, int hidden_dtype, const int64_t *mask, uint16_t *dst_bf16,
                           float *dst_f32, int B, int L, int dim, int normalize, void *stream);
int ccr_meanpool_pack_bf16_ex(const void *hidden, int hidden_dtype, const int64_t *mask, uint16_t *dst_bf16,
                              float *dst_f32, const int64_t *dst_rows, float *row_norm_bounds, int B, int L, int dim,
                              int normalize, void *stream);

int ccr_meanpool_pack_bf16_packed(const void *hidden, int hidden_dtype, const int32_t *seq_start, const int32_t *seq_len,
                                  uint16_t *dst_bf16, float *dst_f32, const int64_t *dst_rows, float *row_norm_bounds, int n_seq,
                                  int dim, int normalize, void *stream);

int ccr_meanpool_bwd(const float *grad, const int64_t *mask, void *dhidden, int hidden_dtype, int B, int L, int dim,
                     void *stream);

int ccr_embed_layernorm(const float *word_table, int64_t vocab, const float *position_table, int64_t n_positions,
                        const float *type_table, int64_t n_types, const int64_t *token_ids, const int64_t *positions,
                        const int64_t *token_types, const float *gamma, const float *beta, float eps, float *out_f32,
                        uint16_t *out_bf16, int64_t rows, int dim, void *stream);
int ccr_gelu_bf16(const uint16_t *x, uint16_t *y, int64_t n, void *stream);
int ccr_attention_bf16(const uint16_t *qkv, const int32_t *seq_start, const int32_t *seq_len, uint16_t *out, int n_seq,
                       int n_heads, int max_len, int pad_len, float scale, void *stream);
int ccr_add_layernorm(const uint16_t *x_bf16, const float *residual, const float *gamma, const float *beta, float eps,
                      float *out_f32, uint16_t *out_bf16, int64_t rows, int dim, void *stream);
int ccr_attention_half(const uint16_t *qkv, const int32_t *seq_start, const int32_t *seq_len, uint16_t *out, int n_seq, int n_heads,
                       int max_len, int pad_len, float scale, int half_dtype, void *stream);
int ccr_add_layernorm_half(const uint16_t *x_half, const float *residual, const float *gamma, const float *beta, float eps,
                           float *out_f32, uint16_t *out_half, int64_t rows, int dim, int half_dtype, void *stream);
int ccr_embed_layernorm_half(const float *word_table, int64_t vocab, const float *position_table, int64_t n_positions,
                             const float *type_table, int64_t n_types, const int64_t *token_ids, const int64_t *positions,
                             const int64_t *token_types, const float *gamma, const float *beta, float eps, float *out_f32,
                             uint16_t *out_half, int64_t rows, int dim, int half_dtype, void *stream);
int ccr_gelu_half(const uint16_t *x, uint16_t *y, int64_t n, int half_dtype, void *stream);

int ccr_attention_fwd_train_half(const uint16_t *qkv, const int32_t *seq_start, const int32_t *seq_len, uint16_t *out, float *lse,
                                 int n_seq, int n_heads, int max_len, int pad_len, float scale, int half_dtype, void *stream);
size_t ccr_attention_bwd_workspace_bytes(int n_seq, int n_heads, int max_len);
int ccr_attention_bwd_half(const uint16_t *qkv, const uint16_t *out, const float *lse, const uint16_t *d_out, const int32_t *seq_start,
                           const int32_t *seq_len, uint16_t *d_qkv, int n_seq, int n_heads, int max_len, int pad_len, float scale,
                           int half_dtype, void *workspace, size_t workspace_bytes, void *stream);
int ccr_add_layernorm_bwd_half(const uint16_t *x_half, const float *residual, const float *gamma, float eps, const float *d_y,
                               float *d_res, uint16_t *d_x, float *d_gamma, float *d_beta, int64_t rows, int dim, int half_dtype,
                               void *workspace, size_t workspace_bytes, void *stream);
int ccr_gelu_bwd_half(const uint16_t *x, const uint16_t *d_y, uint16_t *d_x, int64_t n, int half_dtype, void *stream);

int ccr_dropout_bits_rows(uint32_t *bits, int64_t rows, int dim, uint64_t seed, uint32_t stream_id, double p, void *stream);
int ccr_dropout_bits_attention(uint32_t *keep_q, uint32_t *keep_k, const int32_t *seq_start, const int32_t *seq_len, int64_t n_tokens,
                               int n_seq, int n_heads, int max_len, uint64_t seed, uint32_t stream_id, double p, void *stream);
int ccr_dropout_apply(const float *x, const uint32_t *bits, float inv_keep, float *out_f32, uint16_t *out_half, int64_t rows, int dim,
                      int half_dtype, void *stream);
int ccr_attention_fwd_train_drop_half(const uint16_t *qkv, const int32_t *seq_start, const int32_t *seq_len, uint16_t *out, float *lse,
                                      const uint32_t *keep_q, float inv_keep, int n_seq, int n_heads, int max_len, int pad_len,
                                      float scale, int half_dtype, void *stream);
int ccr_attention_bwd_drop_half(const uint16_t *qkv, const uint16_t *out, const float *lse, const uint16_t *d_out,
                                const int32_t *seq_start, const int32_t *seq_len, const uint32_t *keep_q, const uint32_t *keep_k,
                                float inv_keep, uint16_t *d_qkv, int n_seq, int n_heads, int max_len, int pad_len, float scale,
                                int half_dtype, void *workspace, size_t workspace_bytes, void *stream);
int ccr_add_layernorm_drop_half(const uint16_t *x_half, const uint32_t *bits, float inv_keep, const float *residual, const float *gamma,
                                const float *beta, float eps, float *out_f32, uint16_t *out_half, int64_t rows, int dim, int half_dtype,
                                void *stream);
int ccr_add_layernorm_bwd_drop_half(const uint16_t *x_half, const uint32_t *bits, float inv_keep, const float *residual,
                                    const float *gamma, float eps, const float *d_y, float *d_res, uint16_t *d_x, float *d_gamma,
                                    float *d_beta, int64_t rows, int dim, int half_dtype, void *workspace, size_t workspace_bytes,
                                    void *stream);

int ccr_index_create(const uint16_t *D_bf16, int64_t n_rows, int dim, int64_t global_row_offset, void *stream,
                     ccr_index **out);
int ccr_index_create_with_norms(const uint16_t *D_bf16, int64_t n_rows, int dim, int64_t global_row_offset,
                                const float *row_norm_bounds, void *stream, ccr_index **out);
int ccr_index_destroy(ccr_index *index);
int64_t ccr_index_rows(const ccr_index *index);
int ccr_index_dim(const ccr_index *index);

size_t ccr_search_workspace_bytes(const ccr_index *index, int n_q, int k);
int ccr_search(ccr_index *index, const uint16_t *Q_bf16, int n_q, int k, float *out_scores, int64_t *out_ids,
               void *workspace, size_t ws_bytes, int flags, void *stream);
int ccr_search_finish(ccr_index *index);
int ccr_search_last_stats(const ccr_index *index, ccr_search_stats *stats );
int ccr_search_stream_wait_main_pass(const ccr_index *index, void *stream);

int ccr_scores(const ccr_index *index, const uint16_t *Q_bf16, int n_q, int mode, float *out, void *stream);

size_t ccr_search_blocked_workspace_bytes(const ccr_index *index, int n_q, int k, const int64_t *block_ptr_host);
int ccr_search_blocked(ccr_index *index, const uint16_t *Q_bf16, int n_q, int k, const int64_t *block_ptr_host,
                       const int64_t *block_idx, float *out_scores, int64_t *out_ids, void *workspace, size_t ws_bytes,
                       int flags, void *stream);

size_t ccr_search_sparse_prior_workspace_bytes(const ccr_index *index, int n_q, int k, const int64_t *prior_ptr_host);
int ccr_search_sparse_prior(ccr_index *index, const uint16_t *Q_bf16, int n_q, int k, const int64_t *prior_ptr_host,
                            const int64_t *prior_idx, const double *prior_val, double *out_scores, int64_t *out_ids,
                            void *workspace, size_t ws_bytes, int flags, void *stream);

int ccr_colsum_bf16(const uint16_t *X, int64_t rows, int dim, double *out , void *stream);

int ccr_merge_topk(const float *scores, const int64_t *ids, int R, int n_q, int k, float *out_scores,
                   int64_t *out_ids, void *stream);
int ccr_merge_topk_strided(const float *scores, const int64_t *ids, int64_t score_rank_stride, int64_t id_rank_stride,
                           int R, int n_q, int k, float *out_scores, int64_t *out_ids, void *stream);

#define CCR_SHARD_MAGIC 0x4d524343u
typedef struct ccr_shard_header {
    uint32_t magic;
    uint32_t n_flagged;
    uint32_t k_valid;
    uint32_t n_covered;
    int64_t row_offset;
    int64_t n_rows;
} ccr_shard_header;
size_t ccr_shard_message_bytes(int n_q, int k);
int ccr_search_shard(ccr_index *index, const uint16_t *Q_bf16, int n_q, int k, void *message, void *workspace, size_t ws_bytes,
                     int flags, void *stream);
int ccr_shard_message_fill(void *message, int n_q, int k, int k_valid, const float *scores, const int64_t *ids, int64_t row_offset,
                           int64_t n_rows, void *stream);
int ccr_merge_shard_messages(const void *messages, int64_t message_stride_bytes, int R, int n_q, int k, float *out_scores,
                             int64_t *out_ids, void *stream);
int ccr_merge_short_lists(const void *messages, int64_t message_stride_bytes, int R, int n_q, int k_list, int k_out, float *out_scores,
                          int64_t *out_ids, uint32_t *flags, uint32_t *n_flagged, void *stream);

int ccr_apply_block(const float *in_scores, const int64_t *in_ids, int n_q, int k_in, const int64_t *block_ptr,
                    const int64_t *block_idx, int64_t n_rows_total, float *out_scores, int64_t *out_ids, int k_out,
                    void *stream);

size_t ccr_inbatch_ce_workspace_bytes(int B, int dim);
int ccr_inbatch_pack3_bf16(const float *q, const float *p, const float *n, int B, int dim, uint16_t *out, void *stream);
int ccr_inbatch_ce_fwd_f32(const float *q, const float *p, const float *n, int B, int dim, float inv_temperature, uint16_t *packed,
                           float *loss, float *lse, void *workspace, size_t ws_bytes, void *stream);
int ccr_inbatch_ce_fwd(const uint16_t *Qe, const uint16_t *Pe, const uint16_t *Ne, int B, int dim,
                       float inv_temperature, float *loss, float *lse, void *workspace, size_t ws_bytes, void *stream);
int ccr_inbatch_ce_bwd(const uint16_t *Qe, const uint16_t *Pe, const uint16_t *Ne, const float *lse, int B, int dim,
                       float inv_temperature, float grad_out, float *dQ, float *dP, float *dN, void *workspace,
                       size_t ws_bytes, void *stream);
int ccr_inbatch_ce_bwd_dev(const uint16_t *Qe, const uint16_t *Pe, const uint16_t *Ne, const float *lse, int B, int dim,
                           float inv_temperature, const float *grad_out_dev, float *dQ, float *dP, float *dN,
                           void *workspace, size_t ws_bytes, void *stream);

size_t ccr_pool_ce_workspace_bytes(int n_q, int n_c, int dim);
int ccr_pool_ce_fwd(const uint16_t *Q, const uint16_t *C, const int32_t *label, const float *weight, int n_q, int n_c, int dim,
                    float inv_temperature, float *out3, float *lse, void *workspace, size_t ws_bytes, void *stream);
int ccr_pool_ce_fwd_f32(const float *q, const float *c, const int32_t *label, const float *weight, int n_q, int n_c, int dim,
                        float inv_temperature, uint16_t *packed, float *out3, float *lse, void *workspace, size_t ws_bytes,
                        void *stream);
int ccr_pool_ce_bwd_dev(const uint16_t *Q, const uint16_t *C, const int32_t *label, const float *weight, const float *lse, int n_q,
                        int n_c, int dim, float inv_temperature, const float *grad_out_dev, const float *W_dev, float *dQ, float *dC,
                        void *workspace, size_t ws_bytes, void *stream);

int ccr_bpr_sample(const int64_t *users, int B, int n_neg, int64_t n_users, const int64_t *prior_ptr, const int64_t *prior_idx,
                   const float *prior_t, float t0, const float *proposal, const double *proposal_cdf, int n_items,
                   const double *uniforms, int max_row_nnz, int64_t *out_nj, void *stream);
size_t ccr_bpr_frozen_workspace_bytes(int B, int n_neg, int dim);
int ccr_bpr_frozen_fwd(const float *table, int64_t n_rows, int dim, const float *gamma, const float *beta, float eps,
                       const int64_t *ptr_i, const int64_t *ptr_j, const int64_t *ptr_nj, const float *w, int B, int n_neg,
                       float *out3, void *workspace, size_t ws_bytes, void *stream);
int ccr_bpr_frozen_bwd_dev(const float *table, int64_t n_rows, int dim, const float *gamma, const float *beta, float eps,
                           const int64_t *ptr_i, const int64_t *ptr_j, const int64_t *ptr_nj, const float *w, int B, int n_neg,
                           const float *den_dev, const float *grad_out_dev, float *dgamma, float *dbeta, void *workspace,
                           size_t ws_bytes, void *stream);

int ccr_rank_metrics(const int64_t *ids, int n_q, int k, const int64_t *qrel_ptr, const int64_t *qrel_idx,
                     const int32_t *k_values, int n_k, float *out_rr, int32_t *out_hits, void *stream);

typedef struct ccr_bm25_index ccr_bm25_index;
int ccr_bm25_index_create(const int64_t *indptr_host, const int32_t *doc_ids, const float *tf, const double *doc_k,
                          int64_t n_terms, int64_t n_docs, double k1, ccr_bm25_index **out);
int ccr_bm25_index_destroy(ccr_bm25_index *index);
int ccr_bm25_index_set_idf(ccr_bm25_index *index, const double *idf_host, double *contrib, void *stream);
size_t ccr_bm25_search_workspace_bytes(const ccr_bm25_index *index, int n_q, int max_terms_per_query);
size_t ccr_bm25_search_workspace_bytes_k(const ccr_bm25_index *index, int n_q, int max_terms_per_query, int k);
int ccr_bm25_search_last_stats(const ccr_bm25_index *index, int64_t *out4);
int ccr_bm25_search(const ccr_bm25_index *index, const int64_t *q_ptr_host, const int32_t *q_terms_host,
                    const double *q_idf_host, int n_q, int k, float *out_scores, int64_t *out_ids, void *workspace,
                    size_t ws_bytes, void *stream);

#ifdef __cplusplus
}
#endif
#endif
```

Before: 255,100.

## Skip already-sampled tiles in main pass and rejoin their candidates at rescore

When the optimistic threshold path is chosen, the main filtering GEMM now skips the tiles already scored during the sampling pass, remapping virtual tile indices with a stride-aware function. Candidate groups from the sample whose upper bound beats the threshold are recorded in a per-query list by the threshold kernel and re-joined at select/rescore, which grows the rescore capacity to hold them. A cost model decides whether skipping pays off. This adds complexity and a larger rescore buffer, and it inserts an explicit lgkmcnt wait in the bitonic sort.

```diff
diff --git a/crowd-coachable-recommendations_amd/ccrec_amd/_lib.py b/crowd-coachable-recommendations_amd/ccrec_amd/_lib.py
--- a/crowd-coachable-recommendations_amd/ccrec_amd/_lib.py
+++ b/crowd-coachable-recommendations_amd/ccrec_amd/_lib.py
@@ -49,7 +49,7 @@
                 ("ms_main", ctypes.c_float), ("ms_select", ctypes.c_float), ("ms_fallback", ctypes.c_float),
                 ("ms_total", ctypes.c_float), ("n_retried", ctypes.c_int32), ("n_dense", ctypes.c_int32),
                 ("main_launches", ctypes.c_int32), ("opt_rank", ctypes.c_int32), ("main_tile_queries", ctypes.c_int32),
-                ("reserved0", ctypes.c_int32)]
+                ("skipped_tiles", ctypes.c_int32)]
 
 
 class CcrError(RuntimeError):
diff --git a/crowd-coachable-recommendations_amd/csrc/ccr_api.hip b/crowd-coachable-recommendations_amd/csrc/ccr_api.hip
--- a/crowd-coachable-recommendations_amd/csrc/ccr_api.hip
+++ b/crowd-coachable-recommendations_amd/csrc/ccr_api.hip
@@ -40,6 +40,8 @@
     kn.opt_rank = env_int("CCR_OPT_RANK", 0);
     kn.narrow = env_int("CCR_NARROW", -1);
     kn.wide = env_int("CCR_WIDE", -1);
+    kn.skip_sampled = env_int("CCR_SKIP_SAMPLED", -1);
+    kn.skip_list = env_int("CCR_SKIP_LIST", 1);
     kn.narrow_grid = env_int("CCR_NARROW_GRID", 0);
     kn.narrow_groups = env_int("CCR_NARROW_GROUPS", NARROW_MAX_GROUPS);
     return kn;
@@ -94,11 +96,18 @@
     int64_t sample, ranges;
     int item_a, item_b;
     int opt_rank;
+    int skip;
 };
 
-static int optimistic_rank(int k, int64_t sample, int64_t tiles, const Knobs &kn) {
+static bool may_skip_sampled(const Plan &p, int64_t sample, bool streaming, const Knobs &kn) {
+    if (kn.skip_sampled == 0 || streaming || sample < 1) return false;
+    const int64_t stride = std::max<int64_t>(1, p.full_tiles / sample);
+    return stride >= 2 && (sample - 1) * stride < p.full_tiles && sample < p.tiles;
+}
+
+static int optimistic_rank(int k, int64_t sample, int64_t tiles, const Knobs &kn, bool skip = false) {
     if (kn.opt_rank > 0) return kn.opt_rank;
-    const double need = (double)k * (double)sample / (double)tiles;
+    const double need = (double)k * (double)sample / (double)(skip ? tiles - sample : tiles);
     int r = 40;
     for (; r < 1 << 20; ++r) {
         const double a = 1.0 / (9.0 * r), t = 1.0 - a - 5.2 * sqrt(a);
@@ -108,7 +117,7 @@
 }
 
 static MainPassChoice choose_main_pass(const Plan &p, int k, int64_t sample_a, int64_t sample_b, int64_t sample_c, const Knobs &kn,
-                                       bool single_only = false) {
+                                       bool single_only = false, int64_t skip_only = 0) {
     const int nrc = NUM_XCD / p.main_qgroups, qb_per = p.main_qblocks / p.main_qgroups, per_x = p.grid / NUM_XCD;
     const double tile_cost = p.tile_q == WIDE_Q ? 1.37 : 1.0;
     int64_t max_lists = p.rescore_cap > 512 ? 2048 : 1024;
@@ -124,11 +133,12 @@
         return (double)((smp * p.qblocks + p.grid - 1) / p.grid) + 0.015 * (double)smp * std::max(1.0, qscale);
     };
 
-    MainPassChoice best_choice = {sample_a, target, 0, 0, 0};
+    MainPassChoice best_choice = {sample_a, target, 0, 0, 0, 0};
     double best = 1e300;
     for (int pass = 0; pass < 3; ++pass) {
         const int64_t smp = pass == 0 ? sample_a : (pass == 1 ? sample_b : sample_c);
         if ((pass >= 1 && smp == sample_a) || (pass == 2 && smp == sample_b)) continue;
+        if (skip_only && smp != skip_only) continue;
         const double fs = (double)smp / (double)p.tiles;
         const double smp_cost = sample_cost(smp);
         auto survivors = [&](double fa, double fb) -> double {
@@ -144,27 +154,29 @@
             auto rounds = [&](int64_t n) { return (double)((n + per_x - 1) / per_x); };
             const double common = smp_cost + select_per_range * (double)R + 1e-3 * std::abs((double)(R - target));
             const double single = rounds(items) * item_cost + hit_w * survivors(0.0, 0.0) + common;
-            if (single < best && kn.optimistic != 1) {
+            if (single < best && kn.optimistic != 1 && !skip_only) {
                 best = single;
-                best_choice = {smp, R, 0, 0, 0};
+                best_choice = {smp, R, 0, 0, 0, 0};
             }
             if (kn.optimistic != 0 && smp * GROUPS_PER_TILE >= 4 * 40) {
-                const int rank = optimistic_rank(k, smp, p.tiles, kn);
+                const bool skip = skip_only && may_skip_sampled(p, smp, single_only, kn);
+                const int rank = optimistic_rank(k, smp, p.tiles, kn, skip);
                 if ((int64_t)rank * 4 <= smp * GROUPS_PER_TILE) {
                     const double pass = std::max((double)rank / fs, (double)k);
-                    const double opt = rounds(items) * item_cost + hit_w * pass + common - (kn.optimistic == 1 ? 1e9 : 0.0);
+                    const double opt_item = skip ? ((double)((p.tiles - smp + R - 1) / R) + 0.15) * tile_cost : item_cost;
+                    const double opt = rounds(items) * opt_item + hit_w * pass + common - (kn.optimistic == 1 ? 1e9 : 0.0);
                     if (opt < best) {
                         best = opt;
-                        best_choice = {smp, R, 0, 0, rank};
+                        best_choice = {smp, R, 0, 0, rank, skip ? 1 : 0};
                     }
                 }
             }
-            if (!(prog_on && items > per_x && (double)p.tiles / (double)R >= 8.0)) continue;
+            if (skip_only || !(prog_on && items > per_x && (double)p.tiles / (double)R >= 8.0)) continue;
             const double fa = (double)per_x / (double)items;
             const double two = (1.0 + rounds(items - per_x)) * item_cost + phase_w + hit_w * survivors(fa, 0.0) + common;
             if (two < best) {
                 best = two;
-                best_choice = {smp, R, per_x, 0, 0};
+                best_choice = {smp, R, per_x, 0, 0, 0};
             }
             if (max_phases < 3) continue;
             for (int m = 1; m <= 3; ++m) {
@@ -174,7 +186,7 @@
                 const double three = (1.0 + m + rounds(items - ib)) * item_cost + 2.0 * phase_w + hit_w * survivors(fa, fb) + common;
                 if (three < best) {
                     best = three;
-                    best_choice = {smp, R, per_x, (int)ib, 0};
+                    best_choice = {smp, R, per_x, (int)ib, 0, 0};
                 }
             }
         }
@@ -206,7 +218,7 @@
         p.mfma16 = mfma16;
         p.sublists = p.mfma16 ? 8 : 4;
     }
-    p.rescore_cap = std::min(8192, std::max(256, 2 * pow2_ceil(k)));
+    p.rescore_cap = p.rescore_regular = std::min(8192, std::max(256, 2 * pow2_ceil(k)));
 
     const int64_t min_sample = (2 * (int64_t)k + GROUPS_PER_TILE - 1) / GROUPS_PER_TILE;
     int64_t sample_div = 32;
@@ -256,7 +268,11 @@
             }
         }
         p.main_qgroups = pick_qgroups(p.main_qblocks, dim, kn, p.tile_q);
-        const MainPassChoice choice = choose_main_pass(p, k, sample, sample_alt, sample_big, kn, narrow);
+        MainPassChoice choice = choose_main_pass(p, k, sample, sample_alt, sample_big, kn, narrow);
+        if (choice.opt_rank > 0 && may_skip_sampled(p, choice.sample, narrow, kn)) {
+            const MainPassChoice skipped = choose_main_pass(p, k, sample, sample_alt, sample_big, kn, narrow, choice.sample);
+            if (skipped.skip) choice = skipped;
+        }
         sample = choice.sample;
         const int64_t R = choice.ranges;
         p.sample_tiles = (int)sample;
@@ -266,6 +282,17 @@
         p.item_a = choice.item_a;
         p.item_b = choice.item_b;
         p.opt_rank = choice.opt_rank;
+        p.skip_sampled = (p.opt_rank > 0 && !p.narrow) ? choice.skip : 0;
+        if (p.skip_sampled) {
+            const double join_rows = 256.0 * (double)choice.sample * (1.0 - pow(1.0 - std::min(1.0, (double)k / (double)n_rows), 16.0));
+            const double need = (double)k + (double)(k / 4) + 1.5 * join_rows + TILE_DOCS + 16;
+            const double saved = 0.5 * (double)choice.sample * p.main_qblocks * (p.tile_q == WIDE_Q ? 1.37 : 1.0) / (double)p.grid;
+            const bool pays = 0.065 * join_rows * ((double)p.nq_pad / 3584.0) < saved;
+            if (need > 8192.0 || (kn.skip_sampled < 0 && !pays))
+                p.skip_sampled = 0;
+            else
+                p.rescore_cap = std::min(8192, std::max(p.rescore_cap, pow2_ceil((int)need)));
+        }
         const int nrc_p = NUM_XCD / p.main_qgroups, qb_per_p = p.main_qblocks / p.main_qgroups;
         const int64_t RA = p.item_a ? std::min<int64_t>(R, (int64_t)nrc_p * ((p.item_a + qb_per_p - 1) / qb_per_p)) : 0;
         const int64_t RB = p.item_b ? std::min<int64_t>(R, (int64_t)nrc_p * ((p.item_b + qb_per_p - 1) / qb_per_p)) : 0;
@@ -369,6 +396,7 @@
     w.top = (uint32_t *)take(p.item_b ? (nq_pad + (size_t)n_q * k) * 4 : 0);
     w.thr_safe = (float *)take(p.opt_rank ? nq_pad * 8 : 0);
     w.cq_safe = w.thr_safe + nq_pad;
+    w.glist = (uint32_t *)take(p.skip_sampled ? nq_pad * (size_t)(skip_list_cap(p.opt_rank) + 1) * 4 : 0);
     w.dense_bytes = (size_t)p.dense_rows_per_chunk * n_rows * 4;
     w.dense = (float *)take(w.dense_bytes);
     w.retry_bytes = nq_pad * dim * 2 + nq_pad * 8 + (size_t)n_q * 16 + 64 + 64 + (size_t)n_q * 4 + 256 * 10;
@@ -671,6 +699,11 @@
 
 static int run_main_pass(const ccr_index *ix, const Plan &p, const SearchWs &w, const uint16_t *Q, int n_q, int k, hipStream_t s) {
     GemmArgs gm = filter_args(ix, p, w, Q, n_q, p.nq_pad, p.main_qblocks, p.main_qgroups, w.thr, w.cq, p.cand);
+    if (p.skip_sampled) {
+        gm.n_vt = p.tiles - p.sample_tiles;
+        gm.skip_stride = (int)p.sample_stride;
+        gm.skip_count = p.sample_tiles;
+    }
     const int nrc = NUM_XCD / gm.qgroups, qb_per = gm.qblocks / gm.qgroups, items = p.ranges / nrc * qb_per;
     const int bounds[4] = {0, p.item_a, p.item_b, items};
     int done = 0, updates = 0, prev_full = 0, prev_part = 0, prev_blocks = 0;
@@ -747,6 +780,7 @@
     st.sublists = p.narrow ? p.first_sp : p.sublists;
     st.main_launches = 1 + (p.item_a ? 1 : 0) + (p.item_b ? 1 : 0);
     st.opt_rank = p.opt_rank;
+    st.skipped_tiles = p.skip_sampled ? p.sample_tiles : 0;
     st.main_tile_queries = p.narrow ? 0 : p.tile_q;
     st.n_candidates = (int64_t)ncand;
     return CCR_OK;
@@ -785,7 +819,7 @@
         if (rc != CCR_OK) return rc;
         rc = launch_select_rescore(w.cand, w.cnt, nsub_all, p.sublists, n_cur, pad2, lay2, pd.k, p.rescore_cap, p.select_compact, ix->n_rows,
                                    w.thr2, w.cq2, ix->tile_norm, ix->row_norm, ix->dmax_bits, w.Q2, ix->D, ix->dim, ix->id_out, pd.out_scores, pd.out_ids,
-                                   w.flag2, w.flag2 + 16, nullptr, cur, s);
+                                   w.flag2, w.flag2 + 16, nullptr, cur, s, nullptr, 0, 0, 0, nullptr, 0, p.rescore_regular);
         if (rc != CCR_OK) return rc;
         ix->stats.n_retried += n_cur;
         uint32_t again = 0;
@@ -958,7 +992,7 @@
     if (!p.fused) return search_dense(ix, w, Q_bf16, n_q, k, out_scores, out_ids, flags, s);
 
     CCR_HIP_CHECK(hipMemsetAsync(w.flag_count, 0, 64, s));
-    if ((int64_t)p.ranges > p.tiles) CCR_HIP_CHECK(hipMemsetAsync(w.cnt, 0, (size_t)p.ranges * p.nq_pad * p.sublists * 4, s));
+    if ((int64_t)p.ranges > p.tiles - (p.skip_sampled ? p.sample_tiles : 0)) CCR_HIP_CHECK(hipMemsetAsync(w.cnt, 0, (size_t)p.ranges * p.nq_pad * p.sublists * 4, s));
     int rc = launch_row_norms_bf16(Q_bf16, n_q, ix->dim, w.qnorm, nullptr, nullptr, s);
     if (rc != CCR_OK) return rc;
 
@@ -973,7 +1007,8 @@
     if (rc != CCR_OK) return rc;
     CCR_HIP_CHECK(hipEventRecord(ix->ev[EV_SAMPLE_END], s));
     rc = launch_threshold(w.gmax, (int64_t)p.sample_tiles * GROUPS_PER_TILE, n_q, p.nq_pad, p.opt_rank ? p.opt_rank : k, w.qnorm, ix->dmax_bits,
-                          ix->dim, ix->tile_norm, p.sample_stride, w.thr, w.cq, s, p.narrow ? w.cnt : nullptr, p.narrow ? NARROW_SUBLISTS : 0);
+                          ix->dim, ix->tile_norm, p.sample_stride, w.thr, w.cq, s, p.narrow ? w.cnt : nullptr, p.narrow ? NARROW_SUBLISTS : 0,
+                          p.skip_sampled && ix->knobs.skip_list ? w.glist : nullptr, skip_list_cap(p.opt_rank));
     if (rc != CCR_OK) return rc;
 
     CCR_HIP_CHECK(hipEventRecord(ix->ev[EV_MAIN_BEGIN], s));
@@ -983,7 +1018,9 @@
     ix->main_pass_recorded = true;
     rc = launch_select_rescore(w.cand, w.cnt, p.first_nsub, p.first_sp, n_q, p.nq_pad, p.first_lay, k, p.rescore_cap, p.select_compact, ix->n_rows, w.thr,
                                w.cq, ix->tile_norm, ix->row_norm, ix->dmax_bits, Q_bf16, ix->D, ix->dim, ix->id_out, out_scores, out_ids,
-                               w.flag_count, w.flag_list, w.stat_cand, nullptr, s);
+                               w.flag_count, w.flag_list, w.stat_cand, nullptr, s, p.skip_sampled ? w.gmax : nullptr, p.sample_tiles,
+                               (int)p.sample_stride, p.nq_pad, ix->knobs.skip_list ? w.glist : nullptr, skip_list_cap(p.opt_rank),
+                               p.rescore_regular);
     if (rc != CCR_OK) return rc;
     CCR_HIP_CHECK(hipEventRecord(ix->ev[EV_SELECT_END], s));
 
diff --git a/crowd-coachable-recommendations_amd/csrc/ccr_common.h b/crowd-coachable-recommendations_amd/csrc/ccr_common.h
--- a/crowd-coachable-recommendations_amd/csrc/ccr_common.h
+++ b/crowd-coachable-recommendations_amd/csrc/ccr_common.h
@@ -80,11 +80,13 @@
     int item_a;
     int item_b;
     int opt_rank;
+    int skip_sampled;
     int qgroups;
     int cap;
     CandLayout cand;
     int grid;
     int rescore_cap;
+    int rescore_regular;
     int select_compact;
     int mfma16;
     int sublists;
@@ -97,6 +99,12 @@
     size_t off_qnorm, off_thr, off_gmax, off_cnt, off_cand, off_flag, off_dense, off_retry, off_top, off_safe, total;
     int64_t dense_rows_per_chunk;
 };
+
+__host__ __device__ __forceinline__ int64_t unsampled_tile(int64_t v, int s, int n) {
+    if (s == 0) return v;
+    const uint32_t u = (uint32_t)v, d = (uint32_t)(s - 1);
+    return u < (uint32_t)n * d ? (int64_t)(u + u / d + 1u) : v + n;
+}
 
 enum { EPI_FILTER = 0, EPI_GMAX = 1, EPI_STORE = 2 };
 
@@ -111,6 +119,7 @@
     int64_t n_vt;
     int64_t tile_stride;
     int ranges;
+    int skip_stride, skip_count;
     int qgroups;
     int item_begin, item_end;
     const float *thr;
diff --git a/crowd-coachable-recommendations_amd/csrc/ccr_fused.hip b/crowd-coachable-recommendations_amd/csrc/ccr_fused.hip
--- a/crowd-coachable-recommendations_amd/csrc/ccr_fused.hip
+++ b/crowd-coachable-recommendations_amd/csrc/ccr_fused.hip
@@ -35,6 +35,10 @@
     float m;
     asm("v_max3_f32 %0, %1, %2, %3" : "=v"(m) : "v"(a), "v"(b), "v"(c));
     return m;
+}
+
+__device__ __forceinline__ int64_t real_tile(const GemmArgs &a, int64_t vt) {
+    return a.skip_stride ? unsampled_tile(vt, a.skip_stride, a.skip_count) : vt * a.tile_stride;
 }
 
 struct ItemWalk {
@@ -296,7 +300,7 @@
         int iks = 0;
         const uint16_t *dsrc[2];
         auto tile_ptrs = [&]() {
-            const int64_t row0 = (r + it * a.ranges) * a.tile_stride * TILE_DOCS;
+            const int64_t row0 = real_tile(a, r + it * a.ranges) * TILE_DOCS;
 #pragma unroll
             for (int i = 0; i < 2; ++i) {
                 int64_t drow = row0 + (i * 128 + srow);
@@ -330,8 +334,8 @@
             }
         };
 
-        auto epilogue = [&](int64_t vt, float nt) {
-            const int64_t row_base = vt * a.tile_stride * TILE_DOCS + wd * 128 + 4 * lh;
+        auto epilogue = [&](int64_t vt, int64_t rt, float nt) {
+            const int64_t row_base = rt * TILE_DOCS + wd * 128 + 4 * lh;
             if constexpr (EPI == EPI_GMAX) {
                 S::gmax(acc, a, vt, q0, wd, wq, lane);
             } else if constexpr (EPI == EPI_FILTER) {
@@ -373,11 +377,11 @@
         int cks = 0;
         int64_t ct = 0;
         bool pending = false;
-        int64_t pending_vt = 0;
+        int64_t pending_vt = 0, pending_rt = 0;
         float pending_nt = 0.f;
         for (int64_t u = 0; u < U; ++u) {
             if (pending) {
-                epilogue(pending_vt, pending_nt);
+                epilogue(pending_vt, pending_rt, pending_nt);
                 pending = false;
             }
             if (u + 1 < U) {
@@ -395,19 +399,21 @@
             if (++cks == KS2) {
                 cks = 0;
                 const int64_t vt_done = r + ct * a.ranges;
-                const float nt_done = EPI == EPI_FILTER ? load_uniform_f32(a.tile_norm + vt_done * a.tile_stride) : 0.f;
+                const int64_t rt_done = real_tile(a, vt_done);
+                const float nt_done = EPI == EPI_FILTER ? load_uniform_f32(a.tile_norm + rt_done) : 0.f;
                 if (g1) {
-                    epilogue(vt_done, nt_done);
+                    epilogue(vt_done, rt_done, nt_done);
                 } else {
                     pending = true;
                     pending_vt = vt_done;
+                    pending_rt = rt_done;
                     pending_nt = nt_done;
                 }
                 ++ct;
             }
             CCR_BARRIER();
         }
-        if (pending) epilogue(pending_vt, pending_nt);
+        if (pending) epilogue(pending_vt, pending_rt, pending_nt);
         if (!g1) CCR_BARRIER();
 
         if (EPI == EPI_FILTER) {
@@ -504,7 +510,7 @@
         const char *dtile = nullptr;
         int dlimit = 0;
         auto tile_base = [&]() __attribute__((always_inline)) {
-            const int64_t row0 = (r + it * a.ranges) * a.tile_stride * TILE_DOCS;
+            const int64_t row0 = real_tile(a, r + it * a.ranges) * TILE_DOCS;
             dlimit = (a.n_rows - 1 - row0 < TILE_DOCS - 1) ? (int)(a.n_rows - 1 - row0) : TILE_DOCS - 1;
             dtile = reinterpret_cast<const char *>(a.D) + row0 * pitch;
         };
@@ -553,14 +559,14 @@
             }
         };
 
-        auto epilogue = [&](int64_t vt, float nt) __attribute__((always_inline)) {
+        auto epilogue = [&](int64_t rt, float nt) __attribute__((always_inline)) {
             const int eln = fresh_lane();
             const int l15o = eln & 15, lqo = eln >> 4;
             char *const cbase = reinterpret_cast<char *>(a.cand + seg_base + ((int64_t)(r - seg_r0) * a.nq_pad + q0) * 8 * cap + wd * 4);
             const uint32_t row_lo = (uint32_t)(wd * 128 + 4 * lqo);
             const uint32_t tc_addr = lds_offset(s_tc) + (uint32_t)l15o * 8u;
             const uint32_t cnt_addr = lds_offset(s_cnt) + (uint32_t)(lqo * 16 + l15o) * 4u;
-            const int64_t tile_row0 = vt * a.tile_stride * TILE_DOCS;
+            const int64_t tile_row0 = rt * TILE_DOCS;
             const uint32_t rows_left = a.n_rows - tile_row0 < TILE_DOCS ? (uint32_t)(a.n_rows - tile_row0) : (uint32_t)TILE_DOCS;
 #pragma unroll
             for (int qt = 0; qt < WIDE_QT; ++qt) {
@@ -608,14 +614,14 @@
         int cks = 0;
         int64_t ct = 0;
         bool pending = false;
-        int64_t pending_vt = 0;
+        int64_t pending_rt = 0;
         float pending_nt = 0.f;
         int uslot = 0;
         for (int u = 0; u < U; ++u) {
             if (u + 2 < U) issue();
             __builtin_amdgcn_sched_barrier(0);
             if (pending) {
-                epilogue(pending_vt, pending_nt);
+                epilogue(pending_rt, pending_nt);
                 pending = false;
             }
             const char *abuf = smem + uslot * WIDE_SUB_BYTES;
@@ -661,13 +667,13 @@
             }
             if (++cks == KS2) {
                 cks = 0;
-                const int64_t vt_done = r + ct * a.ranges;
-                const float nt_done = load_uniform_f32(a.tile_norm + vt_done * a.tile_stride);
+                const int64_t rt_done = real_tile(a, r + ct * a.ranges);
+                const float nt_done = load_uniform_f32(a.tile_norm + rt_done);
                 if (g1) {
-                    epilogue(vt_done, nt_done);
+                    epilogue(rt_done, nt_done);
                 } else {
                     pending = true;
-                    pending_vt = vt_done;
+                    pending_rt = rt_done;
                     pending_nt = nt_done;
                 }
                 ++ct;
@@ -675,7 +681,7 @@
             CCR_WAIT_LGKM0();
             CCR_BARRIER();
         }
-        if (pending) epilogue(pending_vt, pending_nt);
+        if (pending) epilogue(pending_rt, pending_nt);
         if (!g1) CCR_BARRIER();
 
         {
@@ -765,25 +771,37 @@
     }
 }
 
+template <bool LIST>
 __global__ __launch_bounds__(256) void threshold_kernel(const float *__restrict__ gmax, int64_t n_groups, int n_q, int nq_pad,
                                                        int k, const float *__restrict__ qnorm,
                                                        const uint32_t *__restrict__ dmax_bits, float gamma,
                                                        const float *__restrict__ tile_norm, int64_t sample_stride,
-                                                       float *__restrict__ thr, float *__restrict__ cq) {
+                                                       float *__restrict__ thr, float *__restrict__ cq,
+                                                       uint32_t *__restrict__ glist, int list_cap) {
     __shared__ uint32_t s_hist[16][256];
-    __shared__ uint32_t s_prefix[16], s_remaining[16];
+    __shared__ uint32_t s_prefix[16], s_remaining[16], s_nlist[16];
     const int tid = threadIdx.x;
     const int ql = tid & 15, ph = tid >> 4;
     const int q = blockIdx.x * 16 + ql;
     if (tid < 16) {
         s_prefix[tid] = 0;
         s_remaining[tid] = (uint32_t)k;
-    }
+        s_nlist[tid] = 0;
+    }
+    uint32_t *const my_list = LIST ? glist + (int64_t)q * (list_cap + 1) : nullptr;
+
     const float dmax = __uint_as_float(*dmax_bits);
     const float c = (q < n_q) ? ((dmax < INFINITY) ? gamma * (qnorm[q] * 1.001f) * 1.001f : __builtin_nanf("")) : 0.f;
     auto tile_of = [&](int64_t g) { return tile_norm[(g / GROUPS_PER_TILE) * sample_stride]; };
+    auto emit = [&](int64_t g, float v, float tn, uint32_t prefix) {
+        if (f32_orderable(fmaf(c, tn, v)) >= prefix) {
+            const uint32_t p = atomicAdd(&s_nlist[ql], 1u);
+            if (p < (uint32_t)list_cap) my_list[1 + p] = (uint32_t)g;
+        }
+    };
     uint32_t mask = 0;
     for (int shift = 24; shift >= 0; shift -= 8) {
+        const bool listing = LIST && shift == 0;
         for (int b = tid; b < 16 * 256; b += 256) (&s_hist[0][0])[b] = 0;
         __syncthreads();
         const uint32_t prefix = s_prefix[ql];
@@ -799,11 +817,14 @@
             for (int j = 0; j < 16; ++j) {
                 const uint32_t o = f32_orderable(fmaf(-c, tn[j], v[j]));
                 if ((o & mask) == prefix) atomicAdd(&s_hist[ql][(o >> shift) & 255u], 1u);
+                if (listing) emit(i + 16 * j, v[j], tn[j], prefix);
             }
         }
         for (; i < n_groups; i += 16) {
-            const uint32_t o = f32_orderable(fmaf(-c, tile_of(i), gmax[i * nq_pad + q]));
+            const float v = gmax[i * nq_pad + q], tn = tile_of(i);
+            const uint32_t o = f32_orderable(fmaf(-c, tn, v));
             if ((o & mask) == prefix) atomicAdd(&s_hist[ql][(o >> shift) & 255u], 1u);
+            if (listing) emit(i, v, tn, prefix);
         }
         __syncthreads();
         {
@@ -852,6 +873,7 @@
             cq[qq] = c;
             thr[qq] = (c < INFINITY) ? tau : __builtin_nanf("");
         }
+        if (LIST) my_list[0] = s_nlist[tid];
     }
 }
 
@@ -1004,7 +1026,9 @@
                                                             int64_t *__restrict__ out_ids, uint32_t *__restrict__ flag_count,
                                                             uint32_t *__restrict__ flag_list,
                                                             unsigned long long *__restrict__ stat_cand,
-                                                            const uint32_t *__restrict__ out_rows) {
+                                                            const uint32_t *__restrict__ out_rows, const float *__restrict__ gmax,
+                                                            int sample_tiles, int sample_stride, int gmax_pitch,
+                                                            const uint32_t *__restrict__ glist, int list_cap, int regular_cap) {
     extern __shared__ __attribute__((aligned(16))) char sm[];
     const size_t cnt_bytes = ((size_t)(ranges + 1) * 4 + 15) & ~(size_t)15;
     uint16_t *s_q = reinterpret_cast<uint16_t *>(sm);
@@ -1195,7 +1219,29 @@
             }
         }
         __syncthreads();
-        if (s_ncoll > (uint32_t)coll_cap) bad = dense_only = true;
+        const uint32_t n_recorded = s_ncoll;
+        if (n_recorded > (uint32_t)regular_cap) bad = dense_only = true;
+        if (gmax && !bad) {
+            __syncthreads();
+            const int ngroups = sample_tiles * GROUPS_PER_TILE;
+            const uint32_t *const my_list = glist ? glist + (int64_t)q * (list_cap + 1) : nullptr;
+            const int nlist = my_list ? (int)min(my_list[0], (uint32_t)list_cap + 1u) : list_cap + 1;
+            const bool listed = nlist <= list_cap;
+            for (int x = tid; x < (listed ? nlist : ngroups); x += THREADS) {
+                const int g = listed ? (int)my_list[1 + x] : x;
+                const int64_t tile = (int64_t)(g / GROUPS_PER_TILE) * sample_stride;
+                if (fmaf(c, tile_norm[tile], gmax[(int64_t)g * gmax_pitch + q]) >= low) {
+                    const int gi = g % GROUPS_PER_TILE;
+                    const uint32_t row0 = (uint32_t)(tile * TILE_DOCS) + (uint32_t)((gi >> 3) * 128 + ((gi >> 1) & 3) * 32 + (gi & 1) * 4);
+                    for (int e = 0; e < 16; ++e) {
+                        const uint32_t p = atomicAdd(&s_ncoll, 1u);
+                        if (p < (uint32_t)coll_cap) s_keys[p] = (unsigned long long)(row0 + (uint32_t)((e & 3) + 8 * (e >> 2)));
+                    }
+                }
+            }
+            __syncthreads();
+            if (s_ncoll > (uint32_t)coll_cap) bad = dense_only = true;
+        }
     }
     if (bad) {
         if (tid == 0) {
@@ -1411,10 +1457,11 @@
                                                              const float *__restrict__ qnorm, const uint32_t *__restrict__ dmax_bits,
                                                              float gamma, const float *__restrict__ tile_norm, int64_t sample_stride,
                                                              float *__restrict__ thr, float *__restrict__ cq, uint32_t *__restrict__ zero_cnt,
-                                                             int zero_per_query) {
+                                                             int zero_per_query, uint32_t *__restrict__ glist, int list_cap) {
     extern __shared__ __attribute__((aligned(16))) uint32_t s_low[];
     __shared__ uint32_t s_hist[256];
     __shared__ uint32_t s_ctl[4];
+    __shared__ uint32_t s_nlist;
     const int tid = threadIdx.x, q = blockIdx.x;
     const float dmax = __uint_as_float(*dmax_bits);
     const float c = (dmax < INFINITY) ? gamma * (qnorm[q] * 1.001f) * 1.001f : __builtin_nanf("");
@@ -1434,24 +1481,38 @@
         cq[q] = c;
         thr[q] = (c < INFINITY) ? orderable_to_f32(kth) : __builtin_nanf("");
     }
+    if (glist) {
+        uint32_t *const my_list = glist + (int64_t)q * (list_cap + 1);
+        if (tid == 0) s_nlist = 0u;
+        __syncthreads();
+        for (int g = tid; g < n_groups; g += 256) {
+            const float up = fmaf(c, tile_norm[(int64_t)(g / GROUPS_PER_TILE) * sample_stride], gmax[(int64_t)g * nq_pad + q]);
+            if (f32_orderable(up) >= kth) {
+                const uint32_t p = atomicAdd(&s_nlist, 1u);
+                if (p < (uint32_t)list_cap) my_list[1 + p] = (uint32_t)g;
+            }
+        }
+        __syncthreads();
+        if (tid == 0) my_list[0] = s_nlist;
+    }
 }
 
 int launch_threshold(const float *gmax, int64_t n_groups, int n_q, int nq_pad, int k, const float *qnorm,
                      const uint32_t *dmax_bits, int dim, const float *tile_norm, int64_t sample_stride, float *thr, float *cq,
-                     hipStream_t s, uint32_t *zero_cnt, int zero_per_query) {
+                     hipStream_t s, uint32_t *zero_cnt, int zero_per_query, uint32_t *glist, int list_cap) {
     if (n_q <= 128 && n_groups >= k && n_groups <= 16384 && zero_per_query <= 256) {
         if (n_groups * 4 > 32 * 1024) {
             const int rc = ensure_dynamic_lds(reinterpret_cast<const void *>(&threshold_small_kernel), 72 * 1024);
             if (rc != CCR_OK) return rc;
         }
         hipLaunchKernelGGL(threshold_small_kernel, dim3(n_q), dim3(256), (size_t)n_groups * 4, s, gmax, (int)n_groups, nq_pad, k, qnorm, dmax_bits,
-                           mfma_gamma(dim), tile_norm, sample_stride, thr, cq, zero_cnt, zero_per_query);
+                           mfma_gamma(dim), tile_norm, sample_stride, thr, cq, zero_cnt, zero_per_query, glist, list_cap);
         CCR_LAUNCH_CHECK();
         return CCR_OK;
     }
     if (zero_cnt) CCR_HIP_CHECK(hipMemsetAsync(zero_cnt, 0, (size_t)n_q * zero_per_query * 4, s));
-    hipLaunchKernelGGL(threshold_kernel, dim3(nq_pad / 16), dim3(256), 0, s, gmax, n_groups, n_q, nq_pad, k, qnorm, dmax_bits,
-                       mfma_gamma(dim), tile_norm, sample_stride, thr, cq);
+    hipLaunchKernelGGL(glist ? threshold_kernel<true> : threshold_kernel<false>, dim3(nq_pad / 16), dim3(256), 0, s, gmax, n_groups, n_q, nq_pad, k, qnorm, dmax_bits,
+                       mfma_gamma(dim), tile_norm, sample_stride, thr, cq, glist, list_cap);
     CCR_LAUNCH_CHECK();
     return CCR_OK;
 }
@@ -1527,7 +1588,9 @@
                           const uint32_t *dmax_bits, const uint16_t *Q,
                           const uint16_t *D, int dim, int64_t id_offset, float *out_scores, int64_t *out_ids,
                           uint32_t *flag_count, uint32_t *flag_list, unsigned long long *stat_cand, const uint32_t *out_rows,
-                          hipStream_t s) {
+                          hipStream_t s, const float *gmax, int sample_tiles, int sample_stride, int gmax_pitch, const uint32_t *glist, int list_cap,
+                          int regular_cap) {
+    if (regular_cap <= 0 || regular_cap > rescore_cap) regular_cap = rescore_cap;
     const size_t lds = select_fixed_lds(dim, ranges, rescore_cap) + (size_t)compact * 8;
     const bool wide = rescore_cap > 512 || compact > 8192 || ranges > 1024;
     auto go = [&](auto kernel, int threads) -> int {
@@ -1537,7 +1600,7 @@
         }
         hipLaunchKernelGGL(kernel, dim3(n_q), dim3(threads), lds, s, cand, cnt, ranges, sp, nq_pad, lay, k, rescore_cap, compact,
                            n_rows, thr, cq, tile_norm, row_norm, dmax_bits, Q, D, dim, id_offset, out_scores, out_ids, flag_count, flag_list, stat_cand,
-                           out_rows);
+                           out_rows, gmax, sample_tiles, sample_stride, gmax_pitch, glist, list_cap, regular_cap);
         CCR_LAUNCH_CHECK();
         return CCR_OK;
     };
diff --git a/crowd-coachable-recommendations_amd/csrc/ccr_index.h b/crowd-coachable-recommendations_amd/csrc/ccr_index.h
--- a/crowd-coachable-recommendations_amd/csrc/ccr_index.h
+++ b/crowd-coachable-recommendations_amd/csrc/ccr_index.h
@@ -15,6 +15,8 @@
     int max_lists;
     int narrow;
     int narrow_grid;
+    int skip_sampled;
+    int skip_list;
     int wide;
     int narrow_groups;
 };
@@ -37,12 +39,14 @@
     unsigned long long *stat_cand;
     uint32_t *top;
     float *thr_safe, *cq_safe, *dense;
+    uint32_t *glist;
     uint16_t *Q2;
     float *thr2, *cq2;
     uint32_t *retry_list, *dense_list, *counts, *flag2, *list_b, *list_c;
     size_t cand_bytes, dense_bytes, retry_bytes, total;
 };
 SearchWs search_ws(const Plan &p, int64_t n_rows, int dim, int n_q, int k, char *base);
+inline int skip_list_cap(int opt_rank) { return 2 * opt_rank + 30; }
 
 enum MainKernel { MAIN_32X32, MAIN_16X16, MAIN_WIDE };
 int launch_gemm(const GemmArgs &a, MainKernel kind, int epi, int grid, hipStream_t s);
@@ -53,13 +57,15 @@
 int launch_tile_norms(const float *row_bounds, int64_t rows, uint32_t *tile_bits, uint32_t *max_bits, hipStream_t s);
 int launch_threshold(const float *gmax, int64_t n_groups, int n_q, int nq_pad, int k, const float *qnorm,
                      const uint32_t *dmax_bits, int dim, const float *tile_norm, int64_t sample_stride, float *thr, float *cq,
-                     hipStream_t s, uint32_t *zero_cnt = nullptr, int zero_per_query = 0);
+                     hipStream_t s, uint32_t *zero_cnt = nullptr, int zero_per_query = 0,
+                     uint32_t *glist = nullptr, int list_cap = 0);
 int select_compact_entries(int dim, int ranges, int rescore_cap, int64_t want);
 int launch_select_rescore(const uint2 *cand, const uint32_t *cnt, int ranges, int sp, int n_q, int nq_pad, const CandLayout &lay, int k,
                           int rescore_cap, int compact, int64_t n_rows, float *thr, const float *cq, const float *tile_norm, const float *row_norm,
                           const uint32_t *dmax_bits, const uint16_t *Q, const uint16_t *D, int dim, int64_t id_offset, float *out_scores, int64_t *out_ids,
                           uint32_t *flag_count, uint32_t *flag_list, unsigned long long *stat_cand, const uint32_t *out_rows,
-                          hipStream_t s);
+                          hipStream_t s, const float *gmax = nullptr, int sample_tiles = 0, int sample_stride = 0, int gmax_pitch = 0,
+                          const uint32_t *glist = nullptr, int list_cap = 0, int regular_cap = 0);
 int launch_partition_flags(const uint32_t *flags, int begin, int n, uint32_t *retry_list, uint32_t *dense_list, uint32_t *counts,
                            hipStream_t s);
 int launch_underfilled_to_retry(uint32_t *flags, int begin, int n, const float *thr_safe, float *thr, hipStream_t s);
diff --git a/crowd-coachable-recommendations_amd/csrc/ccr_topk_device.h b/crowd-coachable-recommendations_amd/csrc/ccr_topk_device.h
--- a/crowd-coachable-recommendations_amd/csrc/ccr_topk_device.h
+++ b/crowd-coachable-recommendations_amd/csrc/ccr_topk_device.h
@@ -94,6 +94,7 @@
     const int nt = blockDim.x;
     for (int size = 2; size <= n; size <<= 1) {
         for (int stride = size >> 1; stride > 0; stride >>= 1) {
+            asm volatile("s_waitcnt lgkmcnt(0)" ::: "memory");
             __syncthreads();
             for (int i = tid; i < (n >> 1); i += nt) {
                 const int pos = 2 * i - (i & (stride - 1));
diff --git a/include/ccr_retrieval.h b/include/ccr_retrieval.h
--- a/include/ccr_retrieval.h
+++ b/include/ccr_retrieval.h
@@ -47,7 +47,7 @@
     int32_t main_launches;
     int32_t opt_rank;
     int32_t main_tile_queries;
-    int32_t reserved0;
+    int32_t skipped_tiles;
 } ccr_search_stats;
 
 const char *ccr_last_error(void);
```

After: 259,500 (median of 6 runs). 1.7% higher.
